# trnKhanh/medical-image-analysis

Measured on AMD Instinct MI355X. Metric: training images/sec (whole node), UNet 512x512 1ch bs=32/GPU, higher is better.
Workload: dtype bf16; 1 GPU; UNet-2D channels [64, 128, 256, 512, 1024] 512x512 1ch, batch 32/GPU, instance norm, dropout 0.1, Dice+CE, Adam(wd 5e-4), clip 10 (cfg3); global_batch=32, parallelism=dp1

## Files before the change

include/mia_hip.h:

```cpp
#ifndef MIA_HIP_H
#define MIA_HIP_H
#include <stdint.h>
#ifdef __cplusplus
extern "C" {
#endif

#define MIA_F32 0
#define MIA_BF16 1

int mia_version(void);
const char* mia_last_error(void);

int mia_pack_weight(const float* src, void* dst, int dtype, int d0, int d1, int taps, int npad, int kpad,
                    int n_from_d0, void* stream);
int mia_pack_desc_bytes(void);
int mia_pack_weight_batch(const void* descs_dev, int count, int total_bricks, int max_taps, int dtype, void* stream);
int mia_relayout(const void* src, int src_dtype, void* dst, int dst_dtype, int n, int c, int64_t hw,
                 int64_t ssn, int64_t ssc, int64_t ssp, int64_t dsn, int64_t dsc, int64_t dsp, void* stream);
int mia_add(const void* a, const void* b, void* out, int dtype, int64_t n, void* stream);
int mia_dropout_mask(float* out, int64_t n, float keep, uint64_t seed, uint64_t offset, void* stream);
int mia_dropout_mask_dyn(float* out, int64_t n, float keep, const uint64_t* seed_base, uint64_t rel_offset, void* stream);
int mia_zero(void* p, int64_t bytes, void* stream);
int mia_gather_f32(const float* src, int64_t stride, float* dst, int n, void* stream);
int mia_colsum_workspace(int64_t p, int c);
int mia_colsum(const void* x, int dtype, int64_t p, int c, float* workspace, float* out, int accumulate, void* stream);

#define MIA_CONV_G3S1 0
#define MIA_CONV_G3S2 1
#define MIA_CONV_G2S2 2
#define MIA_CONV_T3S2 3
#define MIA_CONV_T2S2 4
#define MIA_CONV_G1 5
int mia_set_option(const char* name, int value);
int mia_get_option(const char* name, int* value);
int mia_conv_mma_tiles(int mode, int hout, int wout, int* tiles_y, int* tiles_x, int* tile_h);
int mia_conv_mma(int mode, int dtype, const void* in1, int c1, const void* in2, int c2, const void* wpack, int npad,
                 int kpad, int flip_taps, const float* bias, void* out1, int o1, void* out2, int o2,
                 float* stat_partials, int n, int hin, int win, int hout, int wout, const void* amax_in1, const void* amax_in2,
                 const void* amax_w, const void* wpack_split, void* amax_out1, void* amax_out2, void* stream);
int mia_split_desc_bytes(void);
int mia_split_f16_batch(const void* descs_dev, int count, void* stream);
int mia_amax(const float* x, int64_t n, void* slot, int reset, void* stream);
int mia_widen_u8_i64(const void* src, void* dst, int64_t n, void* stream);
int mia_host_narrow_labels(const int64_t* src, uint8_t* dst, int64_t n, int threads);
int mia_host_copy(void* dst, const void* src, int64_t bytes, int threads);
int mia_amax_desc_bytes(void);
int mia_amax_batch(const void* descs_dev, int count, void* slots, void* stream);

int mia_conv_nl_supported(int mode, int dtype, int c1, int nout, int hout, int wout);
int mia_conv_mma_nl(int mode, int dtype, const void* y_in, int c1, const float* in_scale, const float* in_shift, float slope,
                    const void* wpack, int npad, int kpad, const float* bias, void* out, int nout, float* stat_partials,
                    int n, int hin, int win, int hout, int wout, void* stream);

int mia_conv_acc_supported(int mode, int dtype, int c1, int nout);
int mia_conv_mma_acc(int mode, int dtype, const void* in1, int c1, const void* wpack, int npad, int kpad, int flip_taps,
                     void* out_inout, int nout, int n, int hin, int win, int hout, int wout, const void* amax_in, const void* amax_w,
                     const void* wpack_split, void* stream);


int mia_stem_slabs(void);
int mia_stem_wgrad_workspace(int c0);
int mia_stem_fwd(const void* x, int x_dtype, const float* w, const float* bias, void* y, int dtype, float* stat_partials, int n,
                 int h, int wd, int c0, void* stream);
int mia_stem_wgrad(const void* x, int x_dtype, const void* dy, int dtype, float* workspace, float* grad, int n, int h, int wd,
                   int c0, int accumulate, void* stream);
int mia_stem_wgrad_fused(const void* x, int x_dtype, const void* dz, const void* y, int dtype, const float* scale,
                         const float* shift, const float* xa, const float* xb, const float* c1, const float* c2, float slope,
                         float* workspace, float* grad, int n, int h, int wd, int c0, int accumulate, void* stream);

#define MIA_WGRAD_3S1 0
#define MIA_WGRAD_3S2 1
#define MIA_WGRAD_2S2 2
int mia_wgrad_target_blocks(int mode, int dtype);
int mia_wgrad_geometry(int mode, int dtype, int hy, int wy, int* tiles_y, int* tiles_x);
int mia_wgrad_plan(int mode, int dtype, int c1, int c2, int cdy, int npad, int hy, int* column_blocks, int* target_blocks, int* tile_h);
int mia_conv_wgrad(int mode, int dtype, const void* x1, int c1, const void* x2, int c2, const void* dy, int cdy,
                   float* slabs, int ksplit, int npad, int kpad, int n, int hx, int wx, int hy, int wy, const void* amax_x1,
                   const void* amax_x2, const void* amax_dy, void* stream);
int mia_wgrad_nl_supported(int mode, int dtype, int c1, int cdy);
int mia_conv_wgrad_nl(int mode, int dtype, const void* y_in, int c1, const float* in_scale, const float* in_shift, float slope,
                      const void* dy, int cdy, float* slabs, int ksplit, int npad, int kpad, int n, int hx, int wx, int hy,
                      int wy, void* stream);
int mia_wgrad_reduce(const float* slabs, int ksplit, int taps, int npad, int kpad, float* grad, int nn, int kk,
                     int accumulate, void* stream);

#define MIA_NORM_INSTANCE 0
#define MIA_NORM_BATCH 1
int mia_norm_finalize(const float* partials, int n, int tiles, int c, int64_t hw, int mode, int training,
                      const float* drop_scale, const float* gamma, const float* beta, float eps, float momentum,
                      float* running_mean, float* running_var, long long* num_batches, float* xa, float* xb,
                      float* scale, float* shift, float* ysum, void* stream);
int mia_norm_stats(const void* y, int dtype, int n, int64_t hw, int c, int slabs, float* partials, void* stream);
int mia_norm_act_fwd(const void* y, void* z, int dtype, const float* scale, const float* shift, int n, int64_t hw, int c,
                     float slope, void* amax_out, void* stream);
int mia_norm_two_piece_ok(int dtype, int c);
int mia_norm_act_bwd(const void* dz, const void* dz2, const void* y, void* dy, int dtype, const float* scale, const float* shift,
                     const float* xa, const float* xb, const float* ysum, int n, int64_t hw, int c, int mode,
                     int fixed_stats, float slope, int slabs, float* partials, float* c1, float* c2, float* dgamma,
                     float* dbeta, float* dbias, int accumulate, void* amax_out, void* stream);
int mia_norm_bwd_sums(const void* dz, const void* dz2, const void* y, int dtype, const float* scale, const float* shift,
                      const float* xa, const float* xb, const float* ysum, int n, int64_t hw, int c, int mode,
                      int fixed_stats, float slope, int slabs, float* partials, float* c1, float* c2, float* dgamma,
                      float* dbeta, float* dbias, int accumulate, void* stream);

int mia_bn_sync_local_stats(const float* partials, int n, int tiles, int c, int64_t hw, const float* drop_scale, float* xa,
                            float* xb, float* local, void* stream);
int mia_norm_finalize_sync(const float* gathered, int world, int n, int c, int64_t hw, const float* drop_scale,
                           const float* gamma, const float* beta, float eps, float momentum, float* running_mean,
                           float* running_var, long long* num_batches, float* xa, float* xb, float* scale, float* shift,
                           float* ysum, void* stream);
int mia_norm_act_bwd_reduce(const void* dz, const void* dz2, const void* y, int dtype, const float* scale, const float* shift, const float* xa,
                            const float* xb, int n, int64_t hw, int c, float slope, int slabs, float* partials, float* c1,
                            float* c2, float* tot, void* stream);
int mia_norm_act_bwd_apply_sync(const void* dz, const void* dz2, const void* y, void* dy, int dtype, const float* scale, const float* shift,
                                const float* xa, const float* xb, const float* ysum, int n, int64_t hw, int c, float slope,
                                float* c1, float* c2, const float* group_tot, float* dgamma, float* dbeta, float* dbias,
                                int accumulate, void* amax_out, void* stream);

int mia_head_fwd(const void* x, int dtype, const float* w, const float* b, float* logits, int n, int64_t hw, int c0, int k1,
                 int64_t osn, int64_t osk, int64_t osp, void* stream);
int mia_head_bwd_workspace(int c0, int k1);
int mia_head_bwd(const float* dlogits, const void* x, int dtype, const float* w, void* dx, float* dw, float* db,
                 float* workspace, int n, int64_t hw, int c0, int k1, int64_t gsn, int64_t gsk, int64_t gsp, int accumulate,
                 void* stream);
#define MIA_LOSS_SOFTMAX 1
#define MIA_LOSS_DO_BG 2
#define MIA_LOSS_BATCH 4
#define MIA_LOSS_SQUARED 8
#define MIA_LOSS_DENSE 16
int mia_dice_ce_workspace(int nb, int k1, int slabs);
int mia_dice_ce_fwd(const float* logits, const long long* labels, int nb, int64_t hw, int k1, int64_t sn, int64_t sk,
                    int64_t sp, int flags, float smooth, float dice_w, float ce_w, int slabs, float* workspace, float* sums,
                    float* coef, float* out, int* bad_label, void* stream);
int mia_dice_ce_bwd(const float* logits, const long long* labels, const float* coef, const float* grad_out, float* dlogits,
                    int nb, int64_t hw, int k1, int64_t sn, int64_t sk, int64_t sp, int64_t gsn, int64_t gsk, int64_t gsp,
                    int flags, float dice_w, float ce_w, void* stream);

int mia_ds_loss_workspace(int nb, int k1, int slabs);
int mia_ds_loss_fwd(const float* z, const long long* labels, int nb, int h, int w, int factor, int k1, int64_t sn, int64_t sk,
                    int64_t sp, int flags, float smooth, float dice_w, float ce_w, int slabs, float* workspace, float* sums,
                    float* coef, float* out, int* bad_label, void* stream);
int mia_ds_loss_bwd(const float* z, const long long* labels, const float* coef, const float* grad_out, float* dz, int nb, int h,
                    int w, int factor, int k1, int64_t sn, int64_t sk, int64_t sp, int64_t gsn, int64_t gsk, int64_t gsp, int flags,
                    float dice_w, float ce_w, void* stream);

int mia_head_norm_eligible(int dtype, int n, int64_t hw, int c0, int k1);
int mia_head_norm_fwd(const void* y, int dtype, const float* scale, const float* shift, float slope, const float* w,
                      const float* b, float* logits, int n, int64_t hw, int c0, int k1, int64_t osn, int64_t osk, int64_t osp,
                      void* stream);
int mia_head_norm_wgrad(const float* dlogits, const void* y, int dtype, const float* scale, const float* shift, float slope,
                        float* dw, float* db, float* workspace, int n, int64_t hw, int c0, int k1, int64_t gsn, int64_t gsk,
                        int64_t gsp, int accumulate, void* stream);
int mia_norm_act_bwd_head(const float* dlogits, const float* w, int k1, int64_t gsn, int64_t gsk, int64_t gsp, const void* y,
                          void* dy, int dtype, const float* scale, const float* shift, const float* xa, const float* xb,
                          const float* ysum, int n, int64_t hw, int c, int mode, int fixed_stats, float slope, int slabs,
                          float* partials, float* c1, float* c2, float* dgamma, float* dbeta, float* dbias, int accumulate,
                          void* amax_out, void* stream);
int mia_head_w_supported(int dtype, int c, int k1);
int mia_norm_act_bwd_head_w(const float* dlogits, const float* w, int k1, int64_t gsn, int64_t gsk, int64_t gsp,
                            const void* y, void* dy, int dtype, const float* scale, const float* shift, const float* xa,
                            const float* xb, const float* ysum, int n, int64_t hw, int c, int mode, int fixed_stats,
                            float slope, int slabs, float* partials, float* c1, float* c2, float* dgamma, float* dbeta,
                            float* dbias, int accumulate, float* head_workspace, float* dw_head, float* db_head,
                            int accumulate_head, void* amax_out, void* stream);

#define MIA_SEGLOSS_SOFTMAX 1
#define MIA_SEGLOSS_DO_BG 2
#define MIA_SEGLOSS_BATCH 4
#define MIA_SEGLOSS_LABEL_U8 8
#define MIA_SEGLOSS_IGNORE 16
int mia_seg_loss_workspace(int nb, int k1, int slabs);
int mia_seg_loss_fwd(const float* logits, const void* labels, const float* class_w, int nb, int64_t hw, int k1, int64_t sn,
                     int64_t sk, int64_t sp, int flags, int64_t ignore_label, float smooth, float dice_w, float ce_w, int slabs,
                     float* workspace, float* coef, float* out, int64_t* counts, int* bad_label, void* stream);
int mia_seg_loss_bwd(const float* logits, const void* labels, const float* class_w, const float* coef, const float* grad_out,
                     float* dlogits, int nb, int64_t hw, int k1, int64_t sn, int64_t sk, int64_t sp, int64_t gsn, int64_t gsk,
                     int64_t gsp, int flags, int64_t ignore_label, void* stream);
int mia_topk_ce_workspace(int64_t n_pixels);
int mia_topk_ce_fwd(const float* logits, const void* labels, const float* class_w, int nb, int64_t hw, int k1, int64_t sn,
                    int64_t sk, int64_t sp, int flags, int64_t ignore_label, int64_t n_top, float* workspace, float* out,
                    int* bad_label, void* stream);
int mia_topk_ce_bwd(const float* logits, const void* labels, const float* class_w, const float* workspace, const float* grad_out,
                    float* dlogits, int nb, int64_t hw, int k1, int64_t sn, int64_t sk, int64_t sp, int64_t gsn, int64_t gsk,
                    int64_t gsp, int flags, int64_t ignore_label, void* stream);
#define MIA_REGLOSS_DO_BG 1
#define MIA_REGLOSS_BATCH 2
#define MIA_REGLOSS_IGNORE 4
#define MIA_REGLOSS_INDEX 8
#define MIA_REGLOSS_TARGET_U8 16
int mia_region_loss_workspace(int nb, int c, int slabs);
int mia_region_loss_fwd(const float* logits, const void* target, const unsigned* region_bits, int n_labels, const float* pos_weight,
                        int nb, int64_t hw, int c, int64_t sn, int64_t sk, int64_t sp, int flags, int64_t ignore_label, float smooth,
                        float dice_w, float ce_w, int slabs, float* workspace, float* coef, float* out, int64_t* counts,
                        int* bad_label, void* stream);
int mia_region_loss_bwd(const float* logits, const void* target, const unsigned* region_bits, int n_labels, const float* pos_weight,
                        const float* coef, const float* grad_out, float* dlogits, int nb, int64_t hw, int c, int64_t sn, int64_t sk,
                        int64_t sp, int64_t gsn, int64_t gsk, int64_t gsp, int flags, int64_t ignore_label, void* stream);

#define MIA_OPT_ADAM 0
#define MIA_OPT_ADAMW 1
#define MIA_OPT_SGD 2
int mia_grad_norm_workspace(void);
int mia_grad_norm(const float* grad, int64_t n, float max_norm, float grad_scale, float* workspace, float* out, void* stream);
int mia_scale_by_clip(float* x, int64_t n, const float* clip, void* stream);
int mia_optim_step(float* param, const float* grad, float* m, float* v, int64_t n, int kind, float lr, float beta1,
                   float beta2, float eps, float weight_decay, float bias_corr1, float bias_corr2, int first_step,
                   const float* clip, float grad_scale, void* stream);
int mia_step_dyn_set(void* dyn32, float lr, float bias_corr1, float bias_corr2, int first_step, uint64_t seed, uint64_t offset, void* stream);
int mia_optim_step_dyn(float* param, const float* grad, float* m, float* v, int64_t n, int kind, float beta1, float beta2, float eps,
                       float weight_decay, const float* dyn, const float* clip, float grad_scale, void* stream);

int mia_affine_nearest(const float* img_in, float* img_out, const long long* lab_in, long long* lab_out, int nb, int c, int h,
                       int w, const float* mats, const int* apply, void* stream);
int mia_elastic_warp(const float* img_in, float* img_out, const long long* lab_in, long long* lab_out, int nb, int c, int h,
                     int w, const float* disp, int gh, int gw, const int* apply, void* stream);
int mia_rot90_flip(const void* in, void* out, int elem_bytes, int nb, int c, int h, int w, int k, int flip_h, int flip_w,
                   void* stream);
int mia_crop(const void* in, void* out, int elem_bytes, int nb, int c, int h, int w, int oh, int ow, const int* top,
             const int* left, void* stream);
int mia_gaussian_blur(const float* in, float* out, int nb, int c, int h, int w, const float* sigma, const int* ksize,
                      int max_ksize, const int* apply, void* stream);
int mia_sample_stats_workspace(int nb);
int mia_sample_stats(const float* in, int nb, int c, int64_t hw, int gray, float* workspace, float* mean_std, void* stream);
int mia_sample_stats_sel(const float* in, int nb, int c, int64_t hw, int gray, float* workspace, float* mean_std,
                         const int* apply, void* stream);
int mia_copy_selected(const void* in, void* out, int64_t bytes_per_sample, int nb, const int* apply, void* stream);
#define MIA_EW_GAMMA 0
#define MIA_EW_CONTRAST 1
#define MIA_EW_NOISE 2
#define MIA_EW_ZSCORE 3
int mia_elementwise(const float* in, float* out, int64_t per_sample, int nb, int op, const float* p0, const float* mean_std,
                    const float* aux, const int* apply, void* stream);
int mia_noise_clip(const float* in, float* out, int64_t per_sample, int nb, const float* sigma, uint64_t seed, uint64_t offset,
                   const int* apply, void* stream);
int mia_resize_bilinear(const float* in, float* out, int nb, int c, int h, int w, int oh, int ow, const int* lowres_hw,
                        const int* apply, void* stream);
int mia_resize_bilinear_bwd(const float* dout, float* din_zeroed, int nb, int c, int h, int w, int oh, int ow, void* stream);
int mia_resize_bilinear_aa(const float* in, float* tmp, float* out, int nb, int c, int h, int w, int oh, int ow, void* stream);
int mia_resize_nearest(const void* in, void* out, int elem_bytes, int64_t planes, int h, int w, int oh, int ow, void* stream);

int mia_argmax_dice_workspace(int nb, int k1, int slabs);
int mia_argmax_dice(const float* logits, const long long* labels, long long* pred, int nb, int64_t hw, int k1, int64_t sn, int64_t sk,
                    int64_t sp, int slabs, float* workspace, float* counts, float* dice, void* stream);
int mia_selector_scores_workspace(int nb, int slabs);
int mia_selector_scores(const float* logits, int nb, int64_t hw, int k1, int64_t sn, int64_t sk, int64_t sp, float smooth, int slabs,
                        float* workspace, float* scores, void* stream);
int mia_badge_embed_workspace(int nb, int64_t hw, int k1, int c0, int dtype, int* slabs);
int mia_badge_embed(const float* logits, const void* feat, int dtype, int nb, int64_t hw, int k1, int c0, int64_t sn, int64_t sk,
                    int64_t sp, float smooth, int do_bg, int squared, float* workspace, float* embed, float* loss, void* stream);
int mia_surface_distance_workspace(int nvol, int d, int h, int w, int k1);
int mia_surface_distance(const long long* pred, const long long* labels, int nvol, int ndim, int d, int h, int w, int k1,
                         float sd, float sh, float sw, float* workspace, float* hd, float* asd, void* stream);
int mia_surface_metrics_workspace(int nvol, int d, int h, int w, int k1);
int mia_surface_metrics(const long long* pred, const long long* labels, int nvol, int ndim, int d, int h, int w, int k1,
                        float sd, float sh, float sw, double percentile, const float* tolerance, float* workspace, float* hd,
                        float* asd, float* hd_pct, float* assd, float* nsd, void* stream);
int mia_sdm_workspace(int nb, int h, int w, int k1, int class_mask);
int mia_signed_distance_map(const void* labels, int label_u8, int nb, int h, int w, int k1, int class_mask, float sh, float sw,
                            float* workspace, float* phi, void* stream);
int mia_boundary_loss_workspace(int nb, int slabs);
int mia_boundary_loss_fwd(const float* logits, const void* labels, int label_u8, const float* phi, const float* weight_dev, int nb,
                          int64_t hw, int k1, int class_mask, int64_t sn, int64_t sk, int64_t sp, int slabs, float* workspace,
                          float* coef, float* out, int* bad_label, void* stream);
int mia_boundary_loss_bwd(const float* logits, const float* phi, const float* coef, const float* weight_dev, const float* grad_out,
                          float* dlogits, int nb, int64_t hw, int k1, int class_mask, int64_t sn, int64_t sk, int64_t sp,
                          int64_t gsn, int64_t gsk, int64_t gsp, void* stream);
int mia_consistency_workspace(int nb, int slabs);
int mia_consistency_fwd(const float* zs, const float* zt, const float* prob_mean, const float* dyn_dev, int nb, int64_t hw, int k1,
                        int64_t sn, int64_t sk, int64_t sp, int64_t tsn, int64_t tsk, int64_t tsp, float den_scale, int slabs,
                        float* workspace, unsigned char* keep, float* coef, float* out, long long* n_keep, void* stream);
int mia_consistency_bwd(const float* zs, const float* zt, const unsigned char* keep, const float* coef, const float* dyn_dev,
                        const float* grad_out, float* dzs, int nb, int64_t hw, int k1, int64_t sn, int64_t sk, int64_t sp,
                        int64_t tsn, int64_t tsk, int64_t tsp, int64_t gsn, int64_t gsk, int64_t gsp, void* stream);
int mia_ema_update(float* teacher, const float* student, int64_t n, float alpha, const float* alpha_dev, void* stream);
int mia_urpc_workspace(int nb, int ns, int slabs);
int mia_urpc_fwd(const float* const* z, const int* factors, const int64_t* strides, int ns, int nb, int H, int W, int k1,
                 const float* dyn_dev, int slabs, float* workspace, float* sums, float* terms, float* out, void* stream);
int mia_urpc_bwd(const float* const* z, const int* factors, const int64_t* strides, float* const* dz, const int64_t* gstrides, int ns,
                 int nb, int H, int W, int k1, const float* sums, const float* dyn_dev, const float* grad_out, void* stream);
int mia_cps_workspace(int nb, int slabs);
int mia_cps_fwd(const float* za, const float* zb, const float* dyn_dev, int nb, int64_t hw, int k1, int64_t asn, int64_t ask,
                int64_t asp, int64_t bsn, int64_t bsk, int64_t bsp, int slabs, float* workspace, unsigned char* code, float* out,
                long long* counts, void* stream);
int mia_cps_bwd(const float* za, const float* zb, const unsigned char* code, const float* dyn_dev, const float* grad_out, float* dza,
                float* dzb, int nb, int64_t hw, int k1, int64_t asn, int64_t ask, int64_t asp, int64_t bsn, int64_t bsk, int64_t bsp,
                int64_t gasn, int64_t gask, int64_t gasp, int64_t gbsn, int64_t gbsk, int64_t gbsp, void* stream);

int mia_softmax_accum(const float* logits, float* prob_sum, long long* pred, int nb, int64_t hw, int k1, int64_t sn, int64_t sk,
                      int64_t sp, float weight, int first, void* stream);
int mia_sigmoid_accum(const float* logits, float* prob_sum, long long* pred, const long long* class_order, int nb, int64_t hw, int c,
                      int64_t sn, int64_t sk, int64_t sp, float weight, float threshold, int first, void* stream);
int mia_window_accum(const float* logits, float* canvas, const float* gy, const float* gx, int nb, int k1, int ph, int pw, int h,
                     int w, int y0, int x0, int64_t sn, int64_t sk, int64_t sp, float weight, int flip_h, int flip_w, void* stream);
int mia_window_finalize(float* canvas, long long* pred, const float* ry, const float* rx, int nb, int k1, int h, int w, float scale,
                        int normalise, void* stream);
int mia_mask_denoise_supported(int h, int w, int dilate, int erode, int smooth_k);
int mia_mask_denoise(const long long* in, long long* out, int nb, int h, int w, int dilate, int erode, int smooth_k, void* stream);
int mia_cc_label(const long long* labels, int* roots, int nvol, int ndim, int d, int h, int w, int connectivity, int n_classes,
                 int foreground, int* status, void* stream);
int mia_cc_workspace(int nvol, int ndim, int d, int h, int w, int n_classes);
int mia_cc_filter(const long long* labels, long long* out, int nvol, int ndim, int d, int h, int w, int connectivity, int n_classes,
                  int foreground, int keep_largest, int min_size, const unsigned char* class_mask, int64_t fill, float* workspace,
                  int* status, void* stream);

#ifdef __cplusplus
}
#endif
#endif
```

include/mia_hip_experiments.h:

```cpp
#pragma once
#include <stdint.h>
#ifdef __cplusplus
extern "C" {
#endif
int mia_conv_cr_supported(int mode, int dtype, int c1, int nout, int hout, int wout);
int mia_conv_mma_cr(int mode, int dtype, const void* in1, int c1, const void* wpack, int npad, int kpad, int flip_taps,
                    void* out, int nout, const void* y_prod, const float* scale, const float* shift, const float* xa,
                    const float* xb, float slope, float* partials, int n, int hin, int win, int hout, int wout, void* stream);
int mia_norm_act_bwd_pre(const void* dz, const void* y, void* dy, int dtype, const float* scale, const float* shift,
                         const float* xa, const float* xb, const float* ysum, int n, int64_t hw, int c, int mode,
                         int fixed_stats, float slope, int parts, const float* partials, float* c1, float* c2,
                         float* dgamma, float* dbeta, float* dbias, int accumulate, void* amax_out, void* stream);
#ifdef __cplusplus
}
#endif
```

medical-image-analysis_amd/csrc/common.h:

```cpp
#pragma once
#include <hip/hip_runtime.h>
#include <stdint.h>
#include <stdio.h>
#include <string.h>

#define MIA_F32 0
#define MIA_BF16 1

#define MIA_OK 0
#define MIA_EARG (-1)
#define MIA_EUNSUPPORTED (-2)

extern "C" const char* mia_last_error(void);
void mia_set_error(const char* fmt, ...);

#define MIA_CHECK_ARG(cond, ...)            \
  do {                                      \
    if (!(cond)) {                          \
      mia_set_error(__VA_ARGS__);           \
      return MIA_EARG;                      \
    }                                       \
  } while (0)

#define MIA_LAUNCH_CHECK()                                                  \
  do {                                                                      \
    hipError_t _e = hipGetLastError();                                      \
    if (_e != hipSuccess) {                                                 \
      mia_set_error("%s:%d: %s", __FILE__, __LINE__, hipGetErrorString(_e)); \
      return (int)_e;                                                       \
    }                                                                       \
  } while (0)

typedef unsigned short bf16_t;

typedef __attribute__((ext_vector_type(4))) float f32x4;
typedef __attribute__((ext_vector_type(8))) __bf16 bf16x8;
typedef __attribute__((ext_vector_type(4))) short s16x4;
typedef __attribute__((ext_vector_type(4))) unsigned int u32x4;
typedef __attribute__((ext_vector_type(2))) unsigned int u32x2;
typedef __attribute__((ext_vector_type(16))) float f32x16;

__device__ __forceinline__ float bf2f(bf16_t v) { return __builtin_bit_cast(float, ((unsigned)v) << 16); }
__device__ __forceinline__ bf16_t f2bf(float f) {
  __bf16 b = (__bf16)f;
  return __builtin_bit_cast(bf16_t, b);
}

typedef float f32x2_t __attribute__((ext_vector_type(2)));
typedef __bf16 bf16x2_t __attribute__((ext_vector_type(2)));
__device__ __forceinline__ unsigned pack_bf16x2(float a, float b) {
  return __builtin_bit_cast(unsigned, __builtin_convertvector(f32x2_t{a, b}, bf16x2_t));
}

__device__ __forceinline__ float row16_sum(float v) {
  int iv;
  iv = __builtin_bit_cast(int, v); v += __builtin_bit_cast(float, __builtin_amdgcn_update_dpp(iv, iv, 0xB1, 0xF, 0xF, false));
  iv = __builtin_bit_cast(int, v); v += __builtin_bit_cast(float, __builtin_amdgcn_update_dpp(iv, iv, 0x4E, 0xF, 0xF, false));
  iv = __builtin_bit_cast(int, v); v += __builtin_bit_cast(float, __builtin_amdgcn_update_dpp(iv, iv, 0x141, 0xF, 0xF, false));
  iv = __builtin_bit_cast(int, v); v += __builtin_bit_cast(float, __builtin_amdgcn_update_dpp(iv, iv, 0x140, 0xF, 0xF, false));
  return v;
}

template <typename T> struct Elem;
template <> struct Elem<float> {
  static constexpr int EPU = 4;
  static constexpr int DT = MIA_F32;
  __device__ static __forceinline__ float ld(const float* p) { return *p; }
  __device__ static __forceinline__ void st(float* p, float v) { *p = v; }
  __device__ static __forceinline__ float cvt(float v) { return v; }
};
template <> struct Elem<bf16_t> {
  static constexpr int EPU = 8;
  static constexpr int DT = MIA_BF16;
  __device__ static __forceinline__ float ld(const bf16_t* p) { return bf2f(*p); }
  __device__ static __forceinline__ void st(bf16_t* p, float v) { *p = f2bf(v); }
  __device__ static __forceinline__ bf16_t cvt(float v) { return f2bf(v); }
};

struct SplitF16 {
  typedef __attribute__((ext_vector_type(2))) float f2;
  typedef __attribute__((ext_vector_type(2))) _Float16 h2;
  typedef __attribute__((ext_vector_type(8))) _Float16 f16x8;
  static __device__ __forceinline__ int exp_of(unsigned amax_bits) {
    const int e = 141 - (int)((amax_bits >> 23) & 0xFFu);
    return e > 120 ? 120 : e;
  }
  static __device__ __forceinline__ float pow2(int e) { return __builtin_bit_cast(float, (unsigned)(127 + e) << 23); }
  static __device__ __forceinline__ u32x4 unit(const u32x4& raw, float s) {
    const f32x4 x = __builtin_bit_cast(f32x4, raw) * s;
    u32x4 o;
#pragma unroll
    for (int p = 0; p < 2; ++p) {
      const f2 v = {x[2 * p], x[2 * p + 1]};
      const h2 hh = __builtin_convertvector(v, h2);
      const h2 ll = __builtin_convertvector(v - __builtin_convertvector(hh, f2), h2);
      const unsigned hp = __builtin_bit_cast(unsigned, hh), lp = __builtin_bit_cast(unsigned, ll);
      o[2 * p] = __builtin_amdgcn_perm(lp, hp, 0x05040100u);
      o[2 * p + 1] = __builtin_amdgcn_perm(lp, hp, 0x07060302u);
    }
    return o;
  }
  static __device__ __forceinline__ void unit_planar(const u32x4& raw, float s, u32x2& hp, u32x2& lp) {
    const f32x4 x = __builtin_bit_cast(f32x4, raw) * s;
#pragma unroll
    for (int p = 0; p < 2; ++p) {
      const f2 v = {x[2 * p], x[2 * p + 1]};
      const h2 hh = __builtin_convertvector(v, h2);
      const h2 ll = __builtin_convertvector(v - __builtin_convertvector(hh, f2), h2);
      hp[p] = __builtin_bit_cast(unsigned, hh); lp[p] = __builtin_bit_cast(unsigned, ll);
    }
  }
  static __device__ __forceinline__ void planes_of(const u32x4& w, u32x2& hp, u32x2& lp) {
#pragma unroll
    for (int p = 0; p < 2; ++p) {
      hp[p] = __builtin_amdgcn_perm(w[2 * p + 1], w[2 * p], 0x05040100u);
      lp[p] = __builtin_amdgcn_perm(w[2 * p + 1], w[2 * p], 0x07060302u);
    }
  }
  static __device__ __forceinline__ f32x16 mfma32(const u32x4& a, const u32x4& b, f32x16 c) {
    return __builtin_amdgcn_mfma_f32_32x32x16_f16(__builtin_bit_cast(f16x8, a), __builtin_bit_cast(f16x8, b), c, 0, 0, 0);
  }
  static __device__ __forceinline__ u32x4 dup_hi(const u32x4& w) {
    u32x4 o;
#pragma unroll
    for (int d = 0; d < 4; ++d) o[d] = __builtin_amdgcn_perm(w[d], w[d], 0x01000100u);
    return o;
  }
  static __device__ __forceinline__ u32x4 dup_lo(const u32x4& w) {
    u32x4 o;
#pragma unroll
    for (int d = 0; d < 4; ++d) o[d] = __builtin_amdgcn_perm(w[d], w[d], 0x03020302u);
    return o;
  }
  static __device__ __forceinline__ u32x4 swap_hl(const u32x4& w) {
    u32x4 o;
#pragma unroll
    for (int d = 0; d < 4; ++d) o[d] = __builtin_amdgcn_alignbit(w[d], w[d], 16);
    return o;
  }
  static __device__ __forceinline__ f32x4 mfma(const u32x4& a, const u32x4& b, f32x4 c) {
    return __builtin_amdgcn_mfma_f32_16x16x32_f16(__builtin_bit_cast(f16x8, a), __builtin_bit_cast(f16x8, b), c, 0, 0, 0);
  }
  static __device__ __forceinline__ f32x4 mma(const u32x4& a, const u32x4& bh, const u32x4& bl, f32x4 c) { return mfma(a, bl, mfma(a, bh, c)); }
  static __device__ __forceinline__ f32x4 mma_a(const u32x4& ah, const u32x4& al, const u32x4& b, f32x4 c) { return mfma(al, b, mfma(ah, b, c)); }
  static __device__ __forceinline__ float unscale(float acc, int eo) { return __builtin_ldexpf(acc, eo); }
};

__device__ __forceinline__ float norm_bwd_dy(float g, float yv, float sc, float sf, float ka, float kb, float slope) {
  if (!(__builtin_fmaf(sc, yv, sf) > 0.f)) g *= slope;
  return __builtin_fmaf(sc, g, __builtin_fmaf(ka, yv, kb));
}

__device__ __forceinline__ void store_data_fence() { __builtin_amdgcn_sched_barrier(0x3AC); }
__device__ __forceinline__ void store_data_pad() {
  __builtin_amdgcn_sched_barrier(0x3AC);
  asm volatile("s_nop 1" ::: "memory");
  __builtin_amdgcn_sched_barrier(0x3AC);
}

__device__ __forceinline__ float wave_sum(float v) {
#pragma unroll
  for (int o = 32; o > 0; o >>= 1) v += __shfl_xor(v, o, 64);
  return v;
}

__device__ __forceinline__ double wave_sum_d(double v) {
#pragma unroll
  for (int o = 32; o > 0; o >>= 1) v += __shfl_xor(v, o, 64);
  return v;
}

__device__ __forceinline__ int wave_sum_i(int v) {
#pragma unroll
  for (int o = 32; o > 0; o >>= 1) v += __shfl_xor(v, o, 64);
  return v;
}

__device__ __forceinline__ float block_sum(float v, float* red ) {
  v = wave_sum(v);
  const int w = threadIdx.x >> 6, l = threadIdx.x & 63, nw = (blockDim.x + 63) >> 6;
  __syncthreads();
  if (l == 0) red[w] = v;
  __syncthreads();
  float r = 0.f;
  if (threadIdx.x < 64) {
    r = (l < nw) ? red[l] : 0.f;
    r = wave_sum(r);
  }
  return r;
}

static inline int ceil_div(int a, int b) { return (a + b - 1) / b; }
static inline int64_t ceil_div64(int64_t a, int64_t b) { return (a + b - 1) / b; }
```

medical-image-analysis_amd/csrc/conv64.hip:

```cpp
#include "conv_common.h"
#include "lds_dma.h"
#include <stdlib.h>
#include <type_traits>

namespace {

constexpr int C = 64;
constexpr int TH = 16, TW = 16;
constexpr int IH = TH + 2, IW = TW + 2, PITCH = IW;
constexpr int A_IT = (IH * IW + 63) / 64;
constexpr int NPA = ((A_IT * 64 + 13) / 16) * 16 + 2;
constexpr int LDS_BYTES = 8 * NPA * 16;

struct Tile { int img, ty, tx; };

__device__ __forceinline__ void stat_acc(float& s1, float& s2, float v) {
  asm volatile("v_add_f32 %0, %2, %0\n\tv_fmac_f32 %1, %2, %2" : "+v"(s1), "+v"(s2) : "v"(v));
}

}

#ifdef CONV64_STAMPS
__device__ unsigned long long conv64_dbg[512 * 4 * 8];
#define STAMP(var)                                                                          \
  do {                                                                                      \
    __builtin_amdgcn_sched_barrier(0);                                                      \
    asm volatile("s_memtime %0\n\ts_waitcnt lgkmcnt(0)" : "=s"(var)::"memory");             \
    __builtin_amdgcn_sched_barrier(0);                                                      \
  } while (0)
extern "C" int mia_conv64_debug_read(unsigned long long* host_out) {
  return (int)hipMemcpyFromSymbol(host_out, HIP_SYMBOL(conv64_dbg), sizeof(conv64_dbg));
}
#else
#define STAMP(var) do { } while (0)
#endif

template <bool NL, bool CR>
__global__ __launch_bounds__(256, 2) void conv64_persist_kernel(const ConvArgs a, int total_tiles, int tiles_per_img, int run, int n_base) {
  __shared__ __attribute__((aligned(16))) unsigned char smem[LDS_BYTES + (NL ? 2 * C * 4 : 0)];
  u32x4* ldsA = reinterpret_cast<u32x4*>(smem);
  float* cf = reinterpret_cast<float*>(smem + LDS_BYTES);

  const int tid = threadIdx.x, lane = tid & 63;
  const int wave = __builtin_amdgcn_readfirstlane(tid >> 6);
  const int q = lane >> 4, c16 = lane & 15;
  const int pr = pi16(c16);
  const int g = tid & 3, p4 = tid >> 2;

  const rsrc_t rsw = make_rsrc(a.wp, (unsigned)(9 * a.npad * C * 2));
  u32x4 wf[2][3][3];
#pragma unroll
  for (int c = 0; c < 2; ++c)
#pragma unroll
    for (int ta = 0; ta < 3; ++ta)
#pragma unroll
      for (int tb = 0; tb < 3; ++tb) {
        const int t = ta * 3 + tb;
        const int tw = a.flip ? 8 - t : t;
        wf[c][ta][tb] = __builtin_amdgcn_raw_buffer_load_b128(rsw, ((n_base + 16 * wave + c16) * C + 32 * c + 8 * q) * 2, tw * a.npad * C * 2, 0);
      }
  f32x4 bv;
#pragma unroll
  for (int r = 0; r < 4; ++r) bv[r] = a.bias ? a.bias[n_base + 16 * wave + 4 * q + r] : 0.f;

  const int nblk = gridDim.x, b = blockIdx.x;
  const int first = (b & 7) * run + (b >> 3);
  const int stride = 8 * run;
  auto decode = [&](int t) -> Tile {
    Tile r;
    r.img = t / tiles_per_img;
    const int rem = t - r.img * tiles_per_img;
    r.ty = rem / a.tiles_x;
    r.tx = rem - r.ty * a.tiles_x;
    return r;
  };
  const Tile dstep = decode(stride);
  auto advance = [&](Tile r) -> Tile {
    r.tx += dstep.tx;
    if (r.tx >= a.tiles_x) { r.tx -= a.tiles_x; r.ty += 1; }
    r.ty += dstep.ty;
    if (r.ty >= a.tiles_y) { r.ty -= a.tiles_y; r.img += 1; }
    r.img += dstep.img;
    return r;
  };

  const size_t ipix = (size_t)a.Hin * a.Win;
  const unsigned img_bytes = (unsigned)(ipix * C * 2);
  const bf16_t* in = static_cast<const bf16_t*>(a.in1);
  bf16_t* out = static_cast<bf16_t*>(n_base ? a.out2 : a.out1);

  u32x4 pf[2 * A_IT];
  float cpf = 0.f;
  auto fetch = [&](const Tile& t) {
    const rsrc_t rs = make_rsrc(in + (size_t)t.img * ipix * C, img_bytes);
    const int iy0 = t.ty * TH - 1, ix0 = t.tx * TW - 1;
    int p4v = p4;
    asm volatile("" : "+v"(p4v));
    const bool interior = iy0 >= 0 && ix0 >= 0 && iy0 + IH <= a.Hin && ix0 + IW <= a.Win;
    const int tile_off = (iy0 * a.Win + ix0) * (C * 2) + g * 16;
    if constexpr (NL) {
      if (wave < 2) cpf = (wave == 0 ? a.nl_scale : a.nl_shift)[(size_t)t.img * C + lane];
    }
#pragma unroll
    for (int i = 0; i < A_IT; ++i) {
      const int pix = p4v + 64 * i, iy = pix / IW, ix = pix - iy * IW;
      unsigned voff;
      if (interior) {
        voff = (unsigned)(tile_off + (iy * a.Win + ix) * (C * 2));
        if (i == A_IT - 1) voff = (pix < IH * IW) ? voff : SENT;
      } else {
        const int gy = iy0 + iy, gx = ix0 + ix;
        const int okm = -(int)(((unsigned)gy < (unsigned)a.Hin) & ((unsigned)gx < (unsigned)a.Win) & (pix < IH * IW));
        const unsigned off = (unsigned)((gy * a.Win + gx) * (C * 2) + g * 16);
        voff = (off & (unsigned)okm) | (SENT & ~(unsigned)okm);
      }
      pf[2 * i] = __builtin_amdgcn_raw_buffer_load_b128(rs, (int)voff, 0, 0);
      pf[2 * i + 1] = __builtin_amdgcn_raw_buffer_load_b128(rs, (int)voff, 64, 0);
    }
  };
  auto xform = [&](const u32x4& raw, const f32x4& sa, const f32x4& sb, const f32x4& ha, const f32x4& hb, auto mask_tag, unsigned keep) -> u32x4 {
    constexpr bool MASK = decltype(mask_tag)::value;
    u32x4 o;
    const f32x2_t sl2 = {a.nl_slope, a.nl_slope};
#pragma unroll
    for (int d = 0; d < 4; ++d) {
      const unsigned w = raw[d];
      const f32x2_t sc = d == 0 ? f32x2_t{sa[0], sa[1]} : d == 1 ? f32x2_t{sa[2], sa[3]} : d == 2 ? f32x2_t{sb[0], sb[1]} : f32x2_t{sb[2], sb[3]};
      const f32x2_t sh = d == 0 ? f32x2_t{ha[0], ha[1]} : d == 1 ? f32x2_t{ha[2], ha[3]} : d == 2 ? f32x2_t{hb[0], hb[1]} : f32x2_t{hb[2], hb[3]};
      const f32x2_t x = {__builtin_bit_cast(float, w << 16), __builtin_bit_cast(float, w & 0xFFFF0000u)};
      const f32x2_t v = __builtin_elementwise_fma(sc, x, sh);
      const f32x2_t m = v * sl2;
      const unsigned r = pack_bf16x2(__builtin_fmaxf(v[0], m[0]), __builtin_fmaxf(v[1], m[1]));
      o[d] = MASK ? (r & keep) : r;
    }
    return o;
  };
  auto commit = [&](const Tile& t) {
    if constexpr (NL) {
      const f32x4* cf4 = reinterpret_cast<const f32x4*>(cf);
      const int iy0 = t.ty * TH - 1, ix0 = t.tx * TW - 1;
      const bool interior = iy0 >= 0 && ix0 >= 0 && iy0 + IH <= a.Hin && ix0 + IW <= a.Win;
#pragma unroll
      for (int h = 0; h < 2; ++h) {
        const f32x4 sa = cf4[8 * h + 2 * g], sb = cf4[8 * h + 2 * g + 1], ha = cf4[16 + 8 * h + 2 * g], hb = cf4[17 + 8 * h + 2 * g];
#pragma unroll
        for (int i = 0; i < A_IT; ++i) pf[2 * i + h] = xform(pf[2 * i + h], sa, sb, ha, hb, std::false_type{}, 0u);
        __builtin_amdgcn_sched_barrier(0);
      }
      if (!interior) {
        int p4v = p4;
        asm volatile("" : "+v"(p4v));
#pragma unroll
        for (int i = 0; i < A_IT; ++i) {
          const int pix = p4v + 64 * i, iy = pix / IW, ix = pix - iy * IW;
          const unsigned keep = 0u - (unsigned)(((unsigned)(iy0 + iy) < (unsigned)a.Hin) & ((unsigned)(ix0 + ix) < (unsigned)a.Win));
#pragma unroll
          for (int d = 0; d < 4; ++d) { pf[2 * i][d] &= keep; pf[2 * i + 1][d] &= keep; }
        }
      }
    }
#pragma unroll
    for (int i = 0; i < A_IT; ++i) {
      ldsA[g * NPA + p4 + 64 * i] = pf[2 * i];
      ldsA[(4 + g) * NPA + p4 + 64 * i] = pf[2 * i + 1];
    }
  };

  int t = first;
  if (t >= total_tiles) return;
  Tile cur = decode(t);
  fetch(cur);
  if constexpr (NL) {
    if (tid < 2 * C) cf[tid] = cpf;
    __syncthreads();
  }
  commit(cur);
  __syncthreads();

#ifdef CONV64_STAMPS
  unsigned long long ts0 = 0, ts1 = 0, ts2 = 0, ts3 = 0, ts4 = 0, ts5 = 0, acc_f = 0, acc_m = 0, acc_e = 0, acc_b = 0, acc_c = 0, ntl = 0;
#endif
  while (true) {
    STAMP(ts0);
    const int tn = t + stride;
    const bool more = tn < total_tiles;
    Tile nxt = cur;
    if (more) { nxt = advance(cur); fetch(nxt); }

    STAMP(ts1);
    f32x4 acc[TH];
    constexpr int GROUPS = 6, RPG = 3;
    u32x4 fr[2][RPG];
    auto load_group = [&](int gi, u32x4* f) {
      const int ph = gi / GROUPS, c = ph / 3, tb = ph % 3, r0 = (gi % GROUPS) * RPG;
#pragma unroll
      for (int j = 0; j < RPG; ++j) f[j] = ldsA[(4 * c + q) * NPA + (r0 + j) * PITCH + tb + pr];
    };
    load_group(0, fr[0]);
#pragma unroll
    for (int gi = 0; gi < 6 * GROUPS; ++gi) {
      const int ph = gi / GROUPS, c = ph / 3, tb = ph % 3, r0 = (gi % GROUPS) * RPG;
      if (gi + 1 < 6 * GROUPS) load_group(gi + 1, fr[(gi + 1) & 1]);
      __builtin_amdgcn_sched_barrier(0);
#pragma unroll
      for (int j = 0; j < RPG; ++j) {
        const int r = r0 + j;
#pragma unroll
        for (int ta = 0; ta < 3; ++ta) {
          const int m = r - ta;
          if (m >= 0 && m < TH) {
            const bool first_touch = (ph == 0 && ta == 0);
            acc[m] = __builtin_amdgcn_mfma_f32_16x16x32_bf16(__builtin_bit_cast(bf16x8, wf[c][ta][tb]),
                                                             __builtin_bit_cast(bf16x8, fr[gi & 1][j]), first_touch ? bv : acc[m], 0, 0, 0);
          }
        }
      }
    }

    STAMP(ts2);
    const int oy0 = cur.ty * TH, ox0 = cur.tx * TW;
    const bool full = (oy0 + TH <= a.Hout) && (ox0 + TW <= a.Wout);
    const bool colok = ox0 + pr < a.Wout;
    const rsrc_t rso = make_rsrc(out + (size_t)cur.img * ipix * C, img_bytes);
    const int qodd = q & 1;
    const unsigned obase = (unsigned)((((oy0 + qodd) * a.Wout) + ox0 + pr) * (C * 2) + (16 * wave + 8 * (q >> 1)) * 2);
    const int row_bytes = a.Wout * (C * 2);
    const bool want_stats = a.stats != nullptr;
    float s1[4] = {0.f, 0.f, 0.f, 0.f}, s2[4] = {0.f, 0.f, 0.f, 0.f};
    f32x4 csc, csf, cxa, cxb;
    u32x2 yv[TH];
    const unsigned ybase = (unsigned)(((oy0 * a.Wout) + ox0 + pr) * (C * 2) + (16 * wave + 4 * q) * 2);
    rsrc_t rsy;
    constexpr int YB = 2;
    auto load_y = [&](int m0, bool full_t) {
#pragma unroll
      for (int mm = m0; mm < m0 + YB; ++mm) {
        const bool ok = full_t || (colok && oy0 + mm < a.Hout);
        yv[mm] = __builtin_bit_cast(u32x2, __builtin_amdgcn_raw_buffer_load_b64(rsy, (int)(ok ? ybase + (unsigned)(mm * row_bytes) : SENT), 0, 0));
      }
    };
    if constexpr (CR) {
      const unsigned cbytes = (unsigned)(a.N * C * 4);
      const int co = (cur.img * C + 16 * wave + 4 * q) * 4;
      csc = __builtin_bit_cast(f32x4, __builtin_amdgcn_raw_buffer_load_b128(make_rsrc(a.cr_scale, cbytes), co, 0, 0));
      csf = __builtin_bit_cast(f32x4, __builtin_amdgcn_raw_buffer_load_b128(make_rsrc(a.cr_shift, cbytes), co, 0, 0));
      cxa = __builtin_bit_cast(f32x4, __builtin_amdgcn_raw_buffer_load_b128(make_rsrc(a.cr_xa, cbytes), co, 0, 0));
      cxb = __builtin_bit_cast(f32x4, __builtin_amdgcn_raw_buffer_load_b128(make_rsrc(a.cr_xb, cbytes), co, 0, 0));
      rsy = make_rsrc(static_cast<const bf16_t*>(a.cr_y) + (size_t)cur.img * ipix * C, img_bytes);
      load_y(0, full);
      load_y(YB, full);
    }
    auto cr_row = [&](unsigned p01, unsigned p23, const u32x2& yr, float wgt) {
      const unsigned dzw[2] = {p01, p23}, yw[2] = {yr[0], yr[1]};
#pragma unroll
      for (int h = 0; h < 2; ++h) {
#pragma unroll
        for (int e = 0; e < 2; ++e) {
          const int r = 2 * h + e;
          const float dzv = __builtin_bit_cast(float, e ? (dzw[h] & 0xFFFF0000u) : (dzw[h] << 16));
          const float y = __builtin_bit_cast(float, e ? (yw[h] & 0xFFFF0000u) : (yw[h] << 16));
          float g = dzv * wgt;
          if (!(__builtin_fmaf(csc[r], y, csf[r]) > 0.f)) g *= a.cr_slope;
          s1[r] += g;
          s2[r] = __builtin_fmaf(g, __builtin_fmaf(cxa[r], y, cxb[r]), s2[r]);
        }
      }
    };
    auto store_rows = [&](auto full_tag) {
      constexpr bool FULL = decltype(full_tag)::value;
      if constexpr (FULL) asm volatile("s_nop 7\n\ts_nop 7" ::: "memory");
#pragma unroll
      for (int m = 0; m < TH; m += 2) {
        if constexpr (CR) {
          if (m % YB == 0 && m + 2 * YB < TH) load_y(m + 2 * YB, FULL);
        }
        if (want_stats && !CR) {
#pragma unroll
          for (int mm = m; mm < m + 2; ++mm) {
            const float w = (FULL || (colok && oy0 + mm < a.Hout)) ? 1.f : 0.f;
#pragma unroll
            for (int r = 0; r < 4; ++r) {
              const float v = acc[mm][r];
              if constexpr (FULL) stat_acc(s1[r], s2[r], v);
              else { const float vm = v * w; s1[r] += vm; s2[r] += vm * v; }
            }
          }
        }
        const unsigned x0 = pack_bf16x2(acc[m][0], acc[m][1]), x1 = pack_bf16x2(acc[m][2], acc[m][3]);
        const unsigned y0 = pack_bf16x2(acc[m + 1][0], acc[m + 1][1]), y1 = pack_bf16x2(acc[m + 1][2], acc[m + 1][3]);
        if constexpr (CR) {
          cr_row(x0, x1, yv[m], (FULL || (colok && oy0 + m < a.Hout)) ? 1.f : 0.f);
          cr_row(y0, y1, yv[m + 1], (FULL || (colok && oy0 + m + 1 < a.Hout)) ? 1.f : 0.f);
        }
        const auto r0 = __builtin_amdgcn_permlane16_swap(x0, y0, false, false);
        const auto r1 = __builtin_amdgcn_permlane16_swap(x1, y1, false, false);
        const u32x4 d = {r0[0], r1[0], r0[1], r1[1]};
        if constexpr (FULL) {
          __builtin_amdgcn_raw_buffer_store_b128(d, rso, (int)obase, m * row_bytes, 0);
        } else {
          const bool ok = colok && (oy0 + m + qodd < a.Hout);
          const unsigned voff = ok ? obase + (unsigned)(m * row_bytes) : SENT;
          __builtin_amdgcn_raw_buffer_store_b128(d, rso, (int)voff, 0, 0);
        }
        if constexpr (CR) {
          __builtin_amdgcn_sched_barrier(0);
#ifndef CR_PAD
#define CR_PAD 16
#endif
#if CR_PAD >= 16
          asm volatile("s_nop 7\n\ts_nop 7" ::: "memory");
#elif CR_PAD >= 8
          asm volatile("s_nop 7" ::: "memory");
#elif CR_PAD >= 4
          asm volatile("s_nop 3" ::: "memory");
#elif CR_PAD >= 2
          asm volatile("s_nop 1" ::: "memory");
#endif
          __builtin_amdgcn_sched_barrier(0);
        }
      }
    };
    if (full) store_rows(std::true_type{});
    else store_rows(std::false_type{});
    if (want_stats) {
#pragma unroll
      for (int r = 0; r < 4; ++r) { s1[r] = row16_sum(s1[r]); s2[r] = row16_sum(s2[r]); }
      if (c16 == 0) {
        const size_t tile = (size_t)cur.img * tiles_per_img + (size_t)cur.ty * a.tiles_x + cur.tx;
        typedef __attribute__((address_space(1))) f32x4 gf32x4;
        gf32x4* dst = (gf32x4*)(a.stats + (tile * (size_t)(a.o1 + a.o2) + n_base + 16 * wave + 4 * q) * 2);
        dst[0] = f32x4{s1[0], s2[0], s1[1], s2[1]};
        __builtin_amdgcn_sched_barrier(0);
        asm volatile("s_nop 1" ::: "memory");
        __builtin_amdgcn_sched_barrier(0);
        dst[1] = f32x4{s1[2], s2[2], s1[3], s2[3]};
        __builtin_amdgcn_sched_barrier(0);
        asm volatile("s_nop 1" ::: "memory");
        __builtin_amdgcn_sched_barrier(0);
      }
    }
    STAMP(ts3);
#ifdef CONV64_STAMPS
    acc_f += ts1 - ts0; acc_m += ts2 - ts1; acc_e += ts3 - ts2; ntl += 1;
#endif
    if (!more) break;
    if constexpr (NL) {
      if (tid < 2 * C) cf[tid] = cpf;
    }
    __syncthreads();
    STAMP(ts4);
    commit(nxt);
    __syncthreads();
    STAMP(ts5);
#ifdef CONV64_STAMPS
    acc_b += ts4 - ts3; acc_c += ts5 - ts4;
#endif
    t = tn;
    cur = nxt;
  }
#ifdef CONV64_STAMPS
  if (lane == 0) {
    unsigned long long* d = conv64_dbg + ((size_t)blockIdx.x * 4 + wave) * 8;
    d[0] = acc_f; d[1] = acc_m; d[2] = acc_e; d[3] = acc_b; d[4] = acc_c; d[5] = ntl;
  }
#endif
}

bool conv64_eligible(int mode, int dtype, const ConvArgs& a) {
  if (mode != MODE_G3S1 || dtype != MIA_BF16) return false;
  if (a.nl_scale != nullptr && (a.o2 != 0 || a.nl_shift == nullptr || !(a.nl_slope >= 0.f && a.nl_slope <= 1.f))) return false;
  if (a.cr_y != nullptr && (a.o2 != 0 || a.nl_scale != nullptr || a.stats == nullptr || !a.cr_scale || !a.cr_shift || !a.cr_xa || !a.cr_xb)) return false;
  if (a.c1 != C || a.c2 != 0 || a.o1 != C || (a.o2 != 0 && a.o2 != C) || a.npad != a.o1 + a.o2 || a.kpad != C) return false;
  if (!a.vec_in || !a.vec_out) return false;
  if ((size_t)a.Hin * a.Win * C * 2 >= ((size_t)1 << 31)) return false;
  if (a.Hout <= 8) return false;
  return true;
}

int conv64_launch(const ConvArgs& a, int blocks_override, int reserve, hipStream_t st) {
  const int tiles_per_img = a.tiles_x * a.tiles_y;
  const int total = a.N * tiles_per_img;
  const int cap = 2 * persistent_cus(256, reserve);
  int nblk = total < cap ? ((total + 7) / 8) * 8 : cap;
  if (blocks_override >= 8 && blocks_override % 8 == 0 && blocks_override <= nblk) nblk = blocks_override;
  const int run = nblk / 8;
  if (a.nl_scale != nullptr) {
    hipLaunchKernelGGL((conv64_persist_kernel<true, false>), dim3(nblk), dim3(256), 0, st, a, total, tiles_per_img, run, 0);
    return MIA_OK;
  }
#ifdef MIA_EXPERIMENTS
  if (a.cr_y != nullptr) {
    hipLaunchKernelGGL((conv64_persist_kernel<false, true>), dim3(nblk), dim3(256), 0, st, a, total, tiles_per_img, run, 0);
    return MIA_OK;
  }
#else
  if (a.cr_y != nullptr) { mia_set_error("column-reduce epilogue: experiment build only (-DMIA_EXPERIMENTS)"); return MIA_EUNSUPPORTED; }
#endif
  hipLaunchKernelGGL((conv64_persist_kernel<false, false>), dim3(nblk), dim3(256), 0, st, a, total, tiles_per_img, run, 0);
  if (a.o2 == C)
    hipLaunchKernelGGL((conv64_persist_kernel<false, false>), dim3(nblk), dim3(256), 0, st, a, total, tiles_per_img, run, C);
  return MIA_OK;
}
```

medical-image-analysis_amd/csrc/conv_mma.hip:

```cpp
#include <stdlib.h>

#include "conv_common.h"
#include "options.h"

template <typename T, int MODE, int MT, int NT>
__global__ __launch_bounds__(256, 2) void conv_mma_kernel(const ConvArgs a) {
  using G = Geo<MODE, MT>;
  constexpr int TH = G::TH, BN = 16 * NT, EPU = Elem<T>::EPU, KB = 4 * EPU;
  constexpr int NPA = G::NPA, NPB = BN + 2, PITCH = G::PITCH, S = G::S, IW = G::IW, IH = G::IH;
  constexpr int OSTR = BN + EPU;
  constexpr int A_UNITS = 4 * NPA, B_UNITS = G::MAXTAPS * 4 * NPB;
  constexpr int STAGE_BYTES = (A_UNITS + B_UNITS) * 16;
  constexpr int OUT_BYTES = TH * 16 * OSTR * (int)sizeof(T);
  constexpr int LDS_BYTES = STAGE_BYTES > OUT_BYTES ? STAGE_BYTES : OUT_BYTES;
  __shared__ __attribute__((aligned(16))) unsigned char smem[LDS_BYTES + 2 * 4 * BN * 4];
  u32x4* ldsA = reinterpret_cast<u32x4*>(smem);
  u32x4* ldsB = ldsA + A_UNITS;
  T* ldsO = reinterpret_cast<T*>(smem);
  float* ldsR = reinterpret_cast<float*>(smem + LDS_BYTES);

  const int tid = threadIdx.x, lane = tid & 63, wave = tid >> 6;
  const int q = lane >> 4, r16 = lane & 15;
  const int pr = pi16(r16);

// ... 20 lines not shown
    return 0;
  };
  auto tap_off = [&](int ta, int tb) -> int {
    if (MODE == MODE_G3S1) return ta * PITCH + tb;
    if (MODE == MODE_G3S2 || MODE == MODE_G2S2) return ta * PITCH + (tb & 1) * G::IWH + (tb >> 1);
    if (MODE == MODE_T3S2) { const int dh = ph ? (ta == 0 ? 1 : 0) : 0; const int dw = pw ? (tb == 0 ? 1 : 0) : 0; return dh * PITCH + dw; }
    return 0;
  };

  const int ctot = a.c1 + a.c2;
  f32x4 acc[MT][NT];
#pragma unroll
  for (int m = 0; m < MT; ++m)
#pragma unroll
    for (int n = 0; n < NT; ++n) acc[m][n] = f32x4{0.f, 0.f, 0.f, 0.f};

  const T* in1 = static_cast<const T*>(a.in1);
  const T* in2 = static_cast<const T*>(a.in2);
  const T* wp = static_cast<const T*>(a.wp);

  constexpr int A_N = IH * IW * 4, A_IT = (A_N + 255) / 256;
  constexpr int B_NMAX = G::MAXTAPS * 4 * BN, B_IT = (B_NMAX + 255) / 256;
  const int ntaps = nth * ntw;
  const int b_n = ntaps * 4 * BN;
  constexpr unsigned OOB = 0xFFFFFFFFu;
  unsigned a_pix[A_IT];
#pragma unroll
  for (int i = 0; i < A_IT; ++i) {
    const int u = tid + i * 256;
    a_pix[i] = OOB;
    if (u < A_N) {
      const int pix = u >> 2;
      const int iy = pix / IW, ix = pix - iy * IW;
      const int gy = iy0 + iy, gx = ix0 + ix;
      if (gy >= 0 && gy < a.Hin && gx >= 0 && gx < a.Win) a_pix[i] = (unsigned)(((int64_t)img * a.Hin + gy) * a.Win + gx);
    }
  }
  auto b_src = [&](int u) -> size_t {
    const int g = u & 3, n = (u >> 2) % BN, tl = u / (4 * BN);
    const int ta = tl / ntw, tb = tl - ta * ntw;
    return ((size_t)tap_w(ta, tb) * a.npad + n0 + n) * a.kpad + g * EPU;
  };
  u32x4 pa[A_IT], pb[B_IT];
  auto fetch = [&](int c0) {
#pragma unroll
    for (int i = 0; i < A_IT; ++i) {
      const int g = (tid + i * 256) & 3;
      const int c = c0 + g * EPU;
      u32x4 v = u32x4{0u, 0u, 0u, 0u};
      if (a_pix[i] != OOB && c < ctot) {
        const size_t p = a_pix[i];
        if (a.vec_in) {
          const T* src = (c < a.c1) ? in1 + p * a.c1 + c : in2 + p * a.c2 + (c - a.c1);
          v = *reinterpret_cast<const u32x4*>(src);
        } else {
          alignas(16) T tmp[EPU];
#pragma unroll
          for (int e = 0; e < EPU; ++e) {
            const int ce = c + e;
            T val = (T)0;
            if (ce < a.c1) val = in1[p * a.c1 + ce];
            else if (ce < ctot) val = in2[p * a.c2 + (ce - a.c1)];
            tmp[e] = val;
          }
          v = *reinterpret_cast<const u32x4*>(tmp);
        }
      }
      pa[i] = v;
    }
#pragma unroll
    for (int i = 0; i < B_IT; ++i)
      if (tid + i * 256 < b_n) pb[i] = *reinterpret_cast<const u32x4*>(wp + b_src(tid + i * 256) + c0);
  };
  auto commit = [&]() {
#pragma unroll
    for (int i = 0; i < A_IT; ++i) {
      const int u = tid + i * 256;
      if (u < A_N) {
        const int pix = u >> 2;
        const int iy = pix / IW, ix = pix - iy * IW;
        const int lidx = (S == 2) ? iy * PITCH + (ix & 1) * G::IWH + (ix >> 1) : iy * PITCH + ix;
        ldsA[(u & 3) * NPA + lidx] = pa[i];
      }
    }
#pragma unroll
    for (int i = 0; i < B_IT; ++i) {
      const int u = tid + i * 256;
      if (u < b_n) ldsB[((u / (4 * BN)) * 4 + (u & 3)) * NPB + ((u >> 2) % BN)] = pb[i];
    }
  };

  fetch(0);
  for (int c0 = 0; c0 < ctot; c0 += KB) {
    commit();
    __syncthreads();
    if (c0 + KB < ctot) fetch(c0 + KB);

    for (int ta = 0; ta < nth; ++ta) {
      for (int tb = 0; tb < ntw; ++tb) {
        const int tl = ta * ntw + tb;
        const int toff = tap_off(ta, tb);
        u32x4 bf[NT], af[MT];
#pragma unroll
        for (int n = 0; n < NT; ++n) bf[n] = ldsB[(tl * 4 + q) * NPB + n * 16 + pr];
#pragma unroll
        for (int m = 0; m < MT; ++m) af[m] = ldsA[q * NPA + S * (wave * MT + m) * PITCH + toff + pr];
#pragma unroll
        for (int m = 0; m < MT; ++m)
#pragma unroll
          for (int n = 0; n < NT; ++n) acc[m][n] = Mma<T>::run(af[m], bf[n], acc[m][n]);
      }
    }
    __syncthreads();
  }

  const bool tmode = (MODE == MODE_T3S2 || MODE == MODE_T2S2);
  const int hd = tmode ? (a.Hout - ph + 1) / 2 : a.Hout;
  const int wd = tmode ? (a.Wout - pw + 1) / 2 : a.Wout;
  const int nout = a.o1 + a.o2;
  float s1[NT], s2[NT];
#pragma unroll
  for (int n = 0; n < NT; ++n) { s1[n] = 0.f; s2[n] = 0.f; }
#pragma unroll
  for (int n = 0; n < NT; ++n) {
    const int nn = n * 16 + pr;
    const float b = (a.bias != nullptr && n0 + nn < nout) ? a.bias[n0 + nn] : 0.f;
#pragma unroll
    for (int m = 0; m < MT; ++m) {
      const int y = wave * MT + m;
#pragma unroll
      for (int r = 0; r < 4; ++r) {
        const int px = pi16(4 * q + r);
        const float v = acc[m][n][r] + b;
        if (oy0 + y < hd && ox0 + px < wd) { s1[n] += v; s2[n] += v * v; }
        ldsO[(y * 16 + px) * OSTR + nn] = Elem<T>::cvt(v);
      }
    }
  }
  if (a.stats != nullptr) {
#pragma unroll
    for (int n = 0; n < NT; ++n) {
      float t1 = s1[n], t2 = s2[n];
      t1 += __shfl_xor(t1, 16, 64); t1 += __shfl_xor(t1, 32, 64);
      t2 += __shfl_xor(t2, 16, 64); t2 += __shfl_xor(t2, 32, 64);
      if (q == 0) { ldsR[(0 * 4 + wave) * BN + n * 16 + pr] = t1; ldsR[(1 * 4 + wave) * BN + n * 16 + pr] = t2; }
    }
  }
  __syncthreads();
  if (a.stats != nullptr && tid < BN && n0 + tid < nout) {
    const float t1 = ldsR[0 * BN + tid] + ldsR[1 * BN + tid] + ldsR[2 * BN + tid] + ldsR[3 * BN + tid];
    const float t2 = ldsR[4 * BN + tid] + ldsR[5 * BN + tid] + ldsR[6 * BN + tid] + ldsR[7 * BN + tid];
    const size_t tile = (size_t)img * (a.tiles_x * a.tiles_y) + ty * a.tiles_x + tx;
    float* dst = a.stats + (tile * nout + n0 + tid) * 2;
    dst[0] = t1; dst[1] = t2;
  }
  T* out1 = static_cast<T*>(a.out1);
  T* out2 = static_cast<T*>(a.out2);
  constexpr int UPP = BN / EPU;
  for (int u = tid; u < TH * 16 * UPP; u += 256) {
    const int cu = u % UPP, pl = u / UPP;
    const int y = pl >> 4, px = pl & 15;
    if (oy0 + y >= hd || ox0 + px >= wd) continue;
    const int oy = tmode ? 2 * (oy0 + y) + ph : oy0 + y;
    const int ox = tmode ? 2 * (ox0 + px) + pw : ox0 + px;
    const size_t p = ((size_t)img * a.Hout + oy) * a.Wout + ox;
    const int n = n0 + cu * EPU;
    if (n >= nout) continue;
    const T* srow = ldsO + pl * OSTR + cu * EPU;
    if (a.vec_out) {
      T* dst = (n < a.o1) ? out1 + p * a.o1 + n : out2 + p * a.o2 + (n - a.o1);
      *reinterpret_cast<u32x4*>(dst) = *reinterpret_cast<const u32x4*>(srow);
    } else {
#pragma unroll
      for (int e = 0; e < EPU; ++e) {
        const int ne = n + e;
        if (ne < a.o1) out1[p * a.o1 + ne] = srow[e];
        else if (ne < nout) out2[p * a.o2 + (ne - a.o1)] = srow[e];
      }
    }
  }
}

template <typename T, int MODE, int MT, int NT>
static void launch(const ConvArgs& a, int grid_y, hipStream_t st) {
  const int grid_x = a.N * a.tiles_x * a.tiles_y * a.nblk_n;
  hipLaunchKernelGGL((conv_mma_kernel<T, MODE, MT, NT>), dim3(grid_x, grid_y), dim3(256), 0, st, a);
}

template <typename T, int MODE, int MT>
static void launch_nt(const ConvArgs& a, int nt, int grid_y, hipStream_t st) {
  if (nt == 4) launch<T, MODE, MT, 4>(a, grid_y, st);
  else if (nt == 2) launch<T, MODE, MT, 2>(a, grid_y, st);
  else launch<T, MODE, MT, 1>(a, grid_y, st);
}

template <typename T, int MODE>
static void launch_mt(const ConvArgs& a, int mt, int nt, int grid_y, hipStream_t st) {
  if constexpr (MODE == MODE_G3S2 || MODE == MODE_G2S2) {
    launch_nt<T, MODE, 2>(a, nt, grid_y, st);
  } else {
    if (mt >= 4) launch_nt<T, MODE, 4>(a, nt, grid_y, st);
    else launch_nt<T, MODE, 2>(a, nt, grid_y, st);
  }
}

template <typename T>
static int dispatch(int mode, const ConvArgs& a, int mt, int nt, int grid_y, hipStream_t st) {
  switch (mode) {
    case MODE_G3S1: launch_mt<T, MODE_G3S1>(a, mt, nt, grid_y, st); break;
    case MODE_G3S2: launch_mt<T, MODE_G3S2>(a, mt, nt, grid_y, st); break;
    case MODE_G2S2: launch_mt<T, MODE_G2S2>(a, mt, nt, grid_y, st); break;
    case MODE_T3S2: launch_mt<T, MODE_T3S2>(a, mt, nt, grid_y, st); break;
    case MODE_T2S2: launch_mt<T, MODE_T2S2>(a, mt, nt, grid_y, st); break;
    case MODE_G1: launch_mt<T, MODE_G1>(a, mt, nt, grid_y, st); break;
    default: return MIA_EARG;
  }
  return MIA_OK;
}

extern "C" int mia_amax(const float* x, int64_t n, void* slot, int reset, void* stream);

static void conv_tiles(const MiaOptions& opt, int mode, int hout, int wout, int* tiles_y, int* tiles_x, int* tile_h) {
  const bool tmode = (mode == MODE_T3S2 || mode == MODE_T2S2);
  const int hd = tmode ? (hout + 1) / 2 : hout, wd = tmode ? (wout + 1) / 2 : wout;
  int mt = (mode == MODE_G3S2 || mode == MODE_G2S2) ? 2 : (hd > 8 ? 4 : 2);
  const int th = 4 * mt;
  if (tiles_y) *tiles_y = ceil_div(hd, th);
  if (tiles_x) *tiles_x = ceil_div(wd, 16);
  if (tile_h) *tile_h = th;
}

extern "C" int mia_conv_mma_tiles(int mode, int hout, int wout, int* tiles_y, int* tiles_x, int* tile_h) {
  const MiaOptions opt = mia_options();
  conv_tiles(opt, mode, hout, wout, tiles_y, tiles_x, tile_h);
  return MIA_OK;
}

static int conv_mma_run(int mode, int dtype, const void* in1, int c1, const void* in2, int c2, const void* wpack,
                        int npad, int kpad, int flip_taps, const float* bias, void* out1, int o1, void* out2,
                        int o2, float* stat_partials, int n, int hin, int win, int hout, int wout, void* stream,
                        const float* nl_scale, const float* nl_shift, float nl_slope, const void* cr_y = nullptr,
                        const float* const* cr_coef = nullptr, float cr_slope = 0.f, int acc_out = 0, const void* amax_in1 = nullptr,
                        const void* amax_in2 = nullptr, const void* amax_w = nullptr, void* amax_out1 = nullptr, void* amax_out2 = nullptr,
                        const void* wpack_split = nullptr) {
  MIA_CHECK_ARG(mode >= 0 && mode <= MODE_G1, "mia_conv_mma: bad mode %d", mode);
  MIA_CHECK_ARG(dtype == MIA_F32 || dtype == MIA_BF16, "mia_conv_mma: bad dtype %d", dtype);
  MIA_CHECK_ARG(in1 && wpack && out1 && c1 > 0 && o1 > 0 && c2 >= 0 && o2 >= 0, "mia_conv_mma: null/empty operand");
  MIA_CHECK_ARG((c2 == 0) == (in2 == nullptr) && (o2 == 0) == (out2 == nullptr), "mia_conv_mma: split operand mismatch");
  MIA_CHECK_ARG(n > 0 && hin > 0 && win > 0 && hout > 0 && wout > 0, "mia_conv_mma: bad shape");
  const int epu = dtype == MIA_BF16 ? 8 : 4, kb = 4 * epu;
  MIA_CHECK_ARG(npad % 64 == 0 && npad >= o1 + o2, "mia_conv_mma: npad=%d must be a multiple of 64 >= %d", npad, o1 + o2);
  MIA_CHECK_ARG(kpad % kb == 0 && kpad >= c1 + c2, "mia_conv_mma: kpad=%d must be a multiple of %d >= %d", kpad, kb, c1 + c2);
  bool ok = true;
  switch (mode) {
    case MODE_G3S1: case MODE_G1: ok = (hout == hin && wout == win); break;
    case MODE_G3S2: ok = (hout == (hin + 1) / 2 && wout == (win + 1) / 2); break;
    case MODE_G2S2: ok = (hin == 2 * hout && win == 2 * wout); break;
    case MODE_T3S2: ok = (hin == (hout + 1) / 2 && win == (wout + 1) / 2); break;
    case MODE_T2S2: ok = (hout == 2 * hin && wout == 2 * win); break;
  }
  MIA_CHECK_ARG(ok, "mia_conv_mma: mode %d shape mismatch in %dx%d out %dx%d", mode, hin, win, hout, wout);
  const MiaOptions opt = mia_options();
  ConvArgs a;
  a.in1 = in1; a.in2 = in2; a.c1 = c1; a.c2 = c2; a.wp = wpack; a.bias = bias;
  a.out1 = out1; a.out2 = out2; a.o1 = o1; a.o2 = o2; a.stats = stat_partials;
  a.N = n; a.Hin = hin; a.Win = win; a.Hout = hout; a.Wout = wout;
  a.npad = npad; a.kpad = kpad; a.flip = flip_taps;
  a.nl_scale = nl_scale; a.nl_shift = nl_shift; a.nl_slope = nl_slope;
  a.acc_out = acc_out;
  a.split = (dtype == MIA_F32 && opt.f32_split && amax_in1 != nullptr && amax_w != nullptr && (c2 == 0 || amax_in2 != nullptr)) ? opt.f32_split : 0;
  a.amax_in1 = static_cast<const unsigned*>(amax_in1); a.amax_in2 = static_cast<const unsigned*>(amax_in2);
  a.amax_w = static_cast<const unsigned*>(amax_w);
  if (dtype != MIA_F32) amax_out1 = amax_out2 = nullptr;
  if (cr_y != nullptr) {
    a.cr_y = cr_y; a.cr_scale = cr_coef[0]; a.cr_shift = cr_coef[1]; a.cr_xa = cr_coef[2]; a.cr_xb = cr_coef[3]; a.cr_slope = cr_slope;
  }
  int th;
  conv_tiles(opt, mode, hout, wout, &a.tiles_y, &a.tiles_x, &th);
  int mt = th / 4;
  const int nout = o1 + o2;
  const int nt = nout > 32 ? 4 : (nout > 16 ? 2 : 1);
  a.nblk_n = ceil_div(nout, 16 * nt);
  a.st_tiles_y = a.tiles_y;
  auto al16 = [](const void* p) { return (reinterpret_cast<uintptr_t>(p) & 15) == 0; };
  a.vec_in = (c1 % epu == 0) && (c2 % epu == 0) && al16(in1) && (in2 == nullptr || al16(in2));
  a.vec_out = (o1 % epu == 0) && (o2 % epu == 0) && al16(out1) && (out2 == nullptr || al16(out2));
  const bool tmode = (mode == MODE_T3S2 || mode == MODE_T2S2);
  a.xcd = opt.conv_xcd;
  const int grid_y = tmode ? 4 : 1;
  hipStream_t st = static_cast<hipStream_t>(stream);
  int rc;
  const bool fast = conv_mma_fast_eligible(dtype, a, nt);
  if (opt.conv_s2_wide && fast && mode == MODE_G3S2 && dtype == MIA_BF16 && nout % 128 == 0 && o1 % 128 == 0 && hout > 8 &&
      (c1 + c2 >= 128 || opt.conv_s2_wide >= 2)) {
    mt = 4;
    a.tiles_y = ceil_div(hout, 16);
    a.nblk_n = nout / 128;
  }
  if (acc_out) {
    if (!fast) { mia_set_error("mia_conv_mma_acc: shape outside the accumulating kernel's contract"); return MIA_EUNSUPPORTED; }
    if (a.split && wpack_split != nullptr) { a.wp = wpack_split; a.wsplit = 1; }
    rc = conv_mma_fast_launch(mode, dtype, a, mt, nt, grid_y, st);
  }
#ifdef MIA_EXPERIMENTS
  else if (cr_y != nullptr) {
    if (!(mt == 4 && conv64_eligible(mode, dtype, a))) {
      mia_set_error("mia_conv_mma_cr: shape outside the column-reduce kernel's contract (ask mia_conv_cr_supported first)");
      return MIA_EUNSUPPORTED;
    }
    rc = conv64_launch(a, 0, opt.reserve_cus, st);
  }
#endif
  else if (nl_scale != nullptr) {
    if (!(mt == 4 && conv64_eligible(mode, dtype, a))) {
      mia_set_error("mia_conv_mma_nl: shape outside the normalise-on-load kernel's contract (ask mia_conv_nl_supported first)");
      return MIA_EUNSUPPORTED;
    }
    rc = conv64_launch(a, 0, opt.reserve_cus, st);
  }
  else if (opt.conv64 && opt.conv64_dma && (opt.conv64_dma >= 2 || a.o2 != 0) && mt == 4 && conv64_dma_eligible(mode, dtype, a)) rc = conv64_dma_launch(a, opt.reserve_cus, st);
  else if (opt.conv64 && mt == 4 && conv64_eligible(mode, dtype, a)) rc = conv64_launch(a, 0, opt.reserve_cus, st);
  else if (opt.conv_bt && mt == 4 && conv_bt_eligible(mode, dtype, a)) rc = conv_bt_launch(a, opt.conv_bt_order, opt.reserve_cus, st);
  else if (opt.conv_pw && (mode != MODE_G3S2 || opt.conv_pw_s2 >= 2 || (opt.conv_pw_s2 == 1 && c1 <= 256)) && conv_pw_eligible(mode, dtype, a))
    rc = conv_pw_launch(mode, a, opt.reserve_cus, st);
  else if (fast) {
    if (a.split && wpack_split != nullptr) { a.wp = wpack_split; a.wsplit = 1; }
    if (dtype == MIA_F32) { a.amax_out1 = static_cast<unsigned*>(amax_out1); a.amax_out2 = static_cast<unsigned*>(amax_out2); amax_out1 = amax_out2 = nullptr; }
    rc = conv_mma_fast_launch(mode, dtype, a, mt, nt, grid_y, st);
  }
  else rc = dtype == MIA_BF16 ? dispatch<bf16_t>(mode, a, mt, nt, grid_y, st) : dispatch<float>(mode, a, mt, nt, grid_y, st);
  if (rc != MIA_OK) return rc;
  MIA_LAUNCH_CHECK();
  if (amax_out1 != nullptr) { rc = mia_amax(static_cast<const float*>(out1), (int64_t)n * hout * wout * o1, amax_out1, 0, stream); if (rc) return rc; }
  if (amax_out2 != nullptr && out2 != nullptr) { rc = mia_amax(static_cast<const float*>(out2), (int64_t)n * hout * wout * o2, amax_out2, 0, stream); if (rc) return rc; }
  return MIA_OK;
}

extern "C" int mia_conv_mma(int mode, int dtype, const void* in1, int c1, const void* in2, int c2, const void* wpack,
                            int npad, int kpad, int flip_taps, const float* bias, void* out1, int o1, void* out2,
                            int o2, float* stat_partials, int n, int hin, int win, int hout, int wout, const void* amax_in1,
                            const void* amax_in2, const void* amax_w, const void* wpack_split, void* amax_out1, void* amax_out2,
                            void* stream) {
  return conv_mma_run(mode, dtype, in1, c1, in2, c2, wpack, npad, kpad, flip_taps, bias, out1, o1, out2, o2, stat_partials, n, hin,
                      win, hout, wout, stream, nullptr, nullptr, 0.f, nullptr, nullptr, 0.f, 0, amax_in1, amax_in2, amax_w, amax_out1,
                      amax_out2, wpack_split);
}

extern "C" int mia_conv_nl_supported(int mode, int dtype, int c1, int nout, int hout, int wout) {
  if (mode != MODE_G3S1) return 0;
  return (dtype == MIA_BF16 && c1 == 64 && nout == 64 && hout > 8) ? 1 : 0;
}

extern "C" int mia_conv_mma_nl(int mode, int dtype, const void* y_in, int c1, const float* in_scale, const float* in_shift,
                               float slope, const void* wpack, int npad, int kpad, const float* bias, void* out, int nout,
                               float* stat_partials, int n, int hin, int win, int hout, int wout, void* stream) {
  MIA_CHECK_ARG(in_scale != nullptr && in_shift != nullptr, "mia_conv_mma_nl: null coefficient arrays");
  MIA_CHECK_ARG(slope >= 0.f && slope <= 1.f, "mia_conv_mma_nl: slope %g outside [0, 1]", (double)slope);
  MIA_CHECK_ARG(mia_conv_nl_supported(mode, dtype, c1, nout, hout, wout), "mia_conv_mma_nl: unsupported shape (mode %d dtype %d %d -> %d)",
                mode, dtype, c1, nout);
  return conv_mma_run(mode, dtype, y_in, c1, nullptr, 0, wpack, npad, kpad, 0, bias, out, nout, nullptr, 0, stat_partials, n, hin, win,
                      hout, wout, stream, in_scale, in_shift, slope);
}

#ifdef MIA_EXPERIMENTS
extern "C" int mia_conv_cr_supported(int mode, int dtype, int c1, int nout, int hout, int wout) {
  (void)wout;
  return (mode == MODE_G3S1 && dtype == MIA_BF16 && c1 == 64 && nout == 64 && hout > 8) ? 1 : 0;
}

extern "C" int mia_conv_mma_cr(int mode, int dtype, const void* in1, int c1, const void* wpack, int npad, int kpad, int flip_taps,
                               void* out, int nout, const void* y_prod, const float* scale, const float* shift, const float* xa,
                               const float* xb, float slope, float* partials, int n, int hin, int win, int hout, int wout,
                               void* stream) {
  MIA_CHECK_ARG(y_prod && scale && shift && xa && xb && partials, "mia_conv_mma_cr: null pointer");
  MIA_CHECK_ARG(mia_conv_cr_supported(mode, dtype, c1, nout, hout, wout), "mia_conv_mma_cr: unsupported shape (mode %d dtype %d %d -> %d)",
                mode, dtype, c1, nout);
  MIA_CHECK_ARG((reinterpret_cast<uintptr_t>(y_prod) & 15) == 0 && (reinterpret_cast<uintptr_t>(scale) & 15) == 0 &&
                (reinterpret_cast<uintptr_t>(shift) & 15) == 0 && (reinterpret_cast<uintptr_t>(xa) & 15) == 0 &&
                (reinterpret_cast<uintptr_t>(xb) & 15) == 0, "mia_conv_mma_cr: 16-byte aligned tensors / coefficient rows required");
  const float* coef[4] = {scale, shift, xa, xb};
  return conv_mma_run(mode, dtype, in1, c1, nullptr, 0, wpack, npad, kpad, flip_taps, nullptr, out, nout, nullptr, 0, partials, n, hin,
                      win, hout, wout, stream, nullptr, nullptr, 0.f, y_prod, coef, slope);
}

#endif

extern "C" int mia_conv_acc_supported(int mode, int dtype, int c1, int nout) {
  const int epu = dtype == MIA_BF16 ? 8 : 4;
  return ((mode == MODE_T3S2 || mode == MODE_G3S1) && (dtype == MIA_BF16 || dtype == MIA_F32) && c1 % (4 * epu) == 0 && nout % epu == 0) ? 1 : 0;
}

extern "C" int mia_conv_mma_acc(int mode, int dtype, const void* in1, int c1, const void* wpack, int npad, int kpad, int flip_taps,
                                void* out_inout, int nout, int n, int hin, int win, int hout, int wout, const void* amax_in,
                                const void* amax_w, const void* wpack_split, void* stream) {
  MIA_CHECK_ARG(mode == MODE_T3S2 || mode == MODE_G3S1, "mia_conv_mma_acc: mode %d not served", mode);
  return conv_mma_run(mode, dtype, in1, c1, nullptr, 0, wpack, npad, kpad, flip_taps, nullptr, out_inout, nout, nullptr, 0, nullptr, n, hin,
                      win, hout, wout, stream, nullptr, nullptr, 0.f, nullptr, nullptr, 0.f, 1, amax_in, nullptr, amax_w, nullptr, nullptr, wpack_split);
}
```

medical-image-analysis_amd/csrc/lds_dma.h:

```cpp
#pragma once
#include "common.h"

typedef int i32x4 __attribute__((ext_vector_type(4)));
typedef __amdgpu_buffer_rsrc_t rsrc_t;
constexpr unsigned SENT = 0xFFFFFFF0u;

__device__ __forceinline__ rsrc_t make_rsrc(const void* p, unsigned bytes) {
  return __builtin_amdgcn_make_buffer_rsrc(const_cast<void*>(p), 0, (int)bytes, 0x00020000);
}
__device__ __forceinline__ i32x4 rsrc_words(const void* p, unsigned bytes) {
  const unsigned long long addr = (unsigned long long)p;
  i32x4 r;
  r.x = __builtin_amdgcn_readfirstlane((int)(unsigned)addr);
  r.y = __builtin_amdgcn_readfirstlane((int)(unsigned)(addr >> 32));
  r.z = __builtin_amdgcn_readfirstlane((int)bytes);
  r.w = 0x00020000;
  return r;
}

template <int NOP>
__device__ __forceinline__ void dma16(i32x4 rsrc, unsigned voff, unsigned soff, unsigned lds_dst) {
  asm volatile("s_mov_b32 m0, %3\n\ts_nop %4\n\tbuffer_load_dwordx4 %0, %1, %2 offen lds" : : "v"(voff), "s"(rsrc), "s"(soff), "s"(lds_dst), "n"(NOP) : "memory", "m0");
}
template <int NOP>
__device__ __forceinline__ void dma16(i32x4 rsrc, unsigned voff, unsigned lds_dst) {
  asm volatile("s_mov_b32 m0, %2\n\ts_nop %3\n\tbuffer_load_dwordx4 %0, %1, 0 offen lds" : : "v"(voff), "s"(rsrc), "s"(lds_dst), "n"(NOP) : "memory", "m0");
}

template <int N> __device__ __forceinline__ void wait_vm() { asm volatile("s_waitcnt vmcnt(%0)" ::"n"(N) : "memory"); }
```

medical-image-analysis_amd/csrc/norm.hip:

```cpp
#include "common.h"
#include "options.h"
#include <stdlib.h>

#define NORM_INSTANCE 0
#define NORM_BATCH 1

template <bool INST>
__global__ __launch_bounds__(1024) void norm_fwd_sum_kernel(const float* __restrict__ part, int tiles, int c, float* __restrict__ xa, float* __restrict__ xb,
                                    int64_t hw, const float* __restrict__ drop, const float* __restrict__ gamma,
                                    const float* __restrict__ beta, float eps, float* __restrict__ scale, float* __restrict__ shift,
                                    float* __restrict__ ysum) {
  __shared__ double sh1[16][17], sh2[16][17];
  const int cl = threadIdx.x & 15, tl = threadIdx.x >> 4;
  const int n = blockIdx.x, ch = blockIdx.y * 16 + cl;
  double s1 = 0.0, s2 = 0.0;
  if (ch < c) {
    typedef float f2_t __attribute__((ext_vector_type(2)));
    const f2_t* p = reinterpret_cast<const f2_t*>(part) + (size_t)n * tiles * c + ch;
    int t = tl;
    for (; t + 192 < tiles; t += 256) {
      const f2_t v0 = p[(size_t)t * c], v1 = p[(size_t)(t + 64) * c], v2 = p[(size_t)(t + 128) * c], v3 = p[(size_t)(t + 192) * c];
      s1 += (double)v0.x + (double)v1.x + (double)v2.x + (double)v3.x;
      s2 += (double)v0.y + (double)v1.y + (double)v2.y + (double)v3.y;
    }
// ... 441 lines not shown
template <typename T, bool VEC>
__global__ void norm_act_fwd_kernel(const T* __restrict__ y, T* __restrict__ z, const float* __restrict__ scale,
                                    const float* __restrict__ shift, int64_t hw, int c, int64_t total_units, float slope) {
  constexpr int EPU = VEC ? Elem<T>::EPU : 1;
  const int upp = c / EPU;
  for (int64_t u = (int64_t)blockIdx.x * blockDim.x + threadIdx.x; u < total_units; u += (int64_t)gridDim.x * blockDim.x) {
    const int64_t pix = u / upp;
    const int ch = (int)(u - pix * upp) * EPU;
    const int n = (int)(pix / hw);
    const float* sc = scale + (size_t)n * c + ch;
    const float* sf = shift + (size_t)n * c + ch;
    if constexpr (VEC) {
      const u32x4 raw = *reinterpret_cast<const u32x4*>(y + u * EPU);
      alignas(16) T in[EPU]; alignas(16) T out[EPU];
      *reinterpret_cast<u32x4*>(in) = raw;
#pragma unroll
      for (int e = 0; e < EPU; ++e) {
        const float v = sc[e] * Elem<T>::ld(in + e) + sf[e];
        out[e] = Elem<T>::cvt(v > 0.f ? v : v * slope);
      }
      *reinterpret_cast<u32x4*>(z + u * EPU) = *reinterpret_cast<const u32x4*>(out);
    } else {
      const float v = sc[0] * Elem<T>::ld(y + u) + sf[0];
      Elem<T>::st(z + u, v > 0.f ? v : v * slope);
    }
  }
}

extern "C" int mia_norm_act_fwd(const void* y, void* z, int dtype, const float* scale, const float* shift, int n, int64_t hw,
                                int c, float slope, void* amax_out, void* stream) {
  MIA_CHECK_ARG(y && z && scale && shift && n > 0 && hw > 0 && c > 0, "mia_norm_act_fwd: bad arguments");
  if (dtype != MIA_F32) amax_out = nullptr;
  const int epu = dtype == MIA_BF16 ? 8 : 4;
  const bool vec = (c % epu == 0) && ((reinterpret_cast<uintptr_t>(y) | reinterpret_cast<uintptr_t>(z)) & 15) == 0;
  const int64_t units = (int64_t)n * hw * (vec ? c / epu : c);
  const int blocks = (int)((units + 255) / 256 < 16384 ? (units + 255) / 256 : 16384);
  hipStream_t st = static_cast<hipStream_t>(stream);
  if (vec && (dtype == MIA_BF16 || dtype == MIA_F32)) {
    int sl, upb, gy;
    stream_geometry(n, hw, c, epu, &sl, &upb, &gy);
    if (dtype == MIA_BF16)
      hipLaunchKernelGGL(norm_act_fwd_stream_kernel<bf16_t>, dim3(n * sl, gy), dim3(256), 0, st, static_cast<const bf16_t*>(y), static_cast<bf16_t*>(z), scale, shift, hw, c, sl, upb, slope, (unsigned*)nullptr);
    else
      hipLaunchKernelGGL(norm_act_fwd_stream_kernel<float>, dim3(n * sl, gy), dim3(256), 0, st, static_cast<const float*>(y), static_cast<float*>(z), scale, shift, hw, c, sl, upb, slope, static_cast<unsigned*>(amax_out));
    MIA_LAUNCH_CHECK();
    return MIA_OK;
  }
#define NA(T, V) hipLaunchKernelGGL((norm_act_fwd_kernel<T, V>), dim3(blocks), dim3(256), 0, st, static_cast<const T*>(y), \
                                    static_cast<T*>(z), scale, shift, hw, c, units, slope)
  if (dtype == MIA_BF16) { if (vec) NA(bf16_t, true); else NA(bf16_t, false); }
  else if (dtype == MIA_F32) { if (vec) NA(float, true); else NA(float, false); }
  else { mia_set_error("mia_norm_act_fwd: bad dtype"); return MIA_EARG; }
#undef NA
  MIA_LAUNCH_CHECK();
  if (amax_out) return mia_amax(static_cast<const float*>(z), (int64_t)n * hw * c, amax_out, 0, stream);
  return MIA_OK;
}

template <typename T>
__global__ void norm_act_bwd_reduce_kernel(const T* __restrict__ dz, const T* __restrict__ y, const float* __restrict__ scale,
                                           const float* __restrict__ shift, const float* __restrict__ xa,
                                           const float* __restrict__ xb, int64_t hw, int c, int slabs, float slope,
                                           float* __restrict__ part) {
  extern __shared__ float sh[];
  const int n = blockIdx.x / slabs, s = blockIdx.x % slabs;
  const int cw = blockDim.x >= c ? c : blockDim.x, rows_par = blockDim.x / cw;
  const int tc = threadIdx.x % cw, tr = threadIdx.x / cw;
  const int64_t per = (hw + slabs - 1) / slabs, r0 = s * per, r1 = r0 + per < hw ? r0 + per : hw;
  const size_t base = (size_t)n * hw * c;
  for (int cb = blockIdx.y * cw; cb < c; cb += gridDim.y * cw) {
    const int ch = cb + tc;
    float s1 = 0.f, s2 = 0.f;
    if (ch < c && tr < rows_par) {
      const float sc = scale[(size_t)n * c + ch], sf = shift[(size_t)n * c + ch];
      const float a = xa[(size_t)n * c + ch], b = xb[(size_t)n * c + ch];
      for (int64_t r = r0 + tr; r < r1; r += rows_par) {
        const float yv = Elem<T>::ld(y + base + r * c + ch);
        float g = Elem<T>::ld(dz + base + r * c + ch);
        if (!(sc * yv + sf > 0.f)) g *= slope;
        s1 += g; s2 += g * (a * yv + b);
      }
    }
    sh[threadIdx.x] = s1; sh[blockDim.x + threadIdx.x] = s2;
    __syncthreads();
    if (tr == 0 && ch < c) {
      float t1 = 0.f, t2 = 0.f;
      for (int j = 0; j < rows_par; ++j) { t1 += sh[j * cw + tc]; t2 += sh[blockDim.x + j * cw + tc]; }
      float* dst = part + (((size_t)n * slabs + s) * c + ch) * 2;
      dst[0] = t1; dst[1] = t2;
    }
    __syncthreads();
  }
}

__global__ void norm_bwd_sum_kernel(const float* __restrict__ part, int slabs, int c, float* __restrict__ c1,
                                    float* __restrict__ c2) {
  __shared__ double sh1[16][17], sh2[16][17];
  const int cl = threadIdx.x & 15, tl = threadIdx.x >> 4;
  const int n = blockIdx.x, ch = blockIdx.y * 16 + cl;
  double s1 = 0.0, s2 = 0.0;
  if (ch < c)
    for (int s = tl; s < slabs; s += 16) {
      const float* p = part + (((size_t)n * slabs + s) * c + ch) * 2;
      s1 += p[0]; s2 += p[1];
    }
  sh1[tl][cl] = s1; sh2[tl][cl] = s2;
  __syncthreads();
  if (tl == 0 && ch < c) {
    s1 = 0.0; s2 = 0.0;
    for (int j = 0; j < 16; ++j) { s1 += sh1[j][cl]; s2 += sh2[j][cl]; }
    c1[(size_t)n * c + ch] = (float)s1; c2[(size_t)n * c + ch] = (float)s2;
  }
}

__global__ void norm_bwd_finalize_kernel(int n_img, int c, int64_t hw, int mode, int fixed_stats, const float* __restrict__ scale,
                                         const float* __restrict__ xa, const float* __restrict__ xb, const float* __restrict__ ysum,
                                         float* __restrict__ c1, float* __restrict__ c2, float* __restrict__ dgamma,
                                         float* __restrict__ dbeta, float* __restrict__ dbias, int accumulate,
                                         const float* __restrict__ group_tot, const float* __restrict__ part, int slabs) {
  __shared__ double sh1[16][17], sh2[16][17], sh3[16][17];
  const int cl = threadIdx.x & 15, tl = threadIdx.x >> 4;
  const int ch = blockIdx.x * 16 + cl;
  const double M = (double)hw;
  if (part != nullptr && ch < c) {
    for (int n = tl; n < n_img; n += 16) {
      double s1 = 0.0, s2 = 0.0;
      for (int t = 0; t < slabs; ++t) {
        const float* p = part + (((size_t)n * slabs + t) * c + ch) * 2;
        s1 += p[0]; s2 += p[1];
      }
      c1[(size_t)n * c + ch] = (float)s1; c2[(size_t)n * c + ch] = (float)s2;
    }
  }
  double tg = 0.0, tgx = 0.0;
  if (ch < c)
    for (int n = tl; n < n_img; n += 16) { tg += c1[(size_t)n * c + ch]; tgx += c2[(size_t)n * c + ch]; }
  sh1[tl][cl] = tg; sh2[tl][cl] = tgx;
  __syncthreads();
  tg = 0.0; tgx = 0.0;
  for (int j = 0; j < 16; ++j) { tg += sh1[j][cl]; tgx += sh2[j][cl]; }
  __syncthreads();
  const double cnt = (double)n_img * M;
  double tb = 0.0;
  if (ch < c)
    for (int n = tl; n < n_img; n += 16) {
      const size_t idx = (size_t)n * c + ch;
      const double sg = c1[idx], sgx = c2[idx];
      double m1 = 0.0, m2 = 0.0;
      if (!fixed_stats) {
        if (mode == NORM_INSTANCE) { m1 = sg / M; m2 = sgx / M; }
        else if (group_tot) { const double gc = group_tot[2 * c + ch]; m1 = (double)group_tot[ch] / gc; m2 = (double)group_tot[c + ch] / gc; }
        else { m1 = tg / cnt; m2 = tgx / cnt; }
      }
      c1[idx] = (float)m1; c2[idx] = (float)m2;
      if (dbias) {
        const double sxh = ysum ? (double)xa[idx] * ysum[idx] + M * xb[idx] : 0.0;
        tb += (double)scale[idx] * (sg - M * m1 - m2 * sxh);
      }
    }
  sh3[tl][cl] = tb;
  __syncthreads();
  if (tl == 0 && ch < c) {
    tb = 0.0;
    for (int j = 0; j < 16; ++j) tb += sh3[j][cl];
    dgamma[ch] = accumulate ? dgamma[ch] + (float)tgx : (float)tgx;
    dbeta[ch] = accumulate ? dbeta[ch] + (float)tg : (float)tg;
    if (dbias) dbias[ch] = accumulate ? dbias[ch] + (float)tb : (float)tb;
  }
}

template <typename T, bool VEC>
__global__ void norm_act_bwd_apply_kernel(const T* __restrict__ dz, const T* __restrict__ y, T* __restrict__ dy,
                                          const float* __restrict__ scale, const float* __restrict__ shift,
                                          const float* __restrict__ xa, const float* __restrict__ xb,
                                          const float* __restrict__ c1, const float* __restrict__ c2, int64_t hw, int c,
                                          int64_t total_units, float slope) {
  constexpr int EPU = VEC ? Elem<T>::EPU : 1;
  const int upp = c / EPU;
  for (int64_t u = (int64_t)blockIdx.x * blockDim.x + threadIdx.x; u < total_units; u += (int64_t)gridDim.x * blockDim.x) {
    const int64_t pix = u / upp;
    const int ch = (int)(u - pix * upp) * EPU;
    const size_t o = (size_t)(pix / hw) * c + ch;
    alignas(16) T gin[EPU]; alignas(16) T yin[EPU]; alignas(16) T out[EPU];
    if constexpr (VEC) {
      *reinterpret_cast<u32x4*>(gin) = *reinterpret_cast<const u32x4*>(dz + u * EPU);
      *reinterpret_cast<u32x4*>(yin) = *reinterpret_cast<const u32x4*>(y + u * EPU);
    } else { gin[0] = dz[u]; yin[0] = y[u]; }
#pragma unroll
    for (int e = 0; e < EPU; ++e) {
      const float yv = Elem<T>::ld(yin + e);
      float g = Elem<T>::ld(gin + e);
      if (!(scale[o + e] * yv + shift[o + e] > 0.f)) g *= slope;
      const float xh = xa[o + e] * yv + xb[o + e];
      out[e] = Elem<T>::cvt(scale[o + e] * (g - c1[o + e] - xh * c2[o + e]));
    }
    if constexpr (VEC) *reinterpret_cast<u32x4*>(dy + u * EPU) = *reinterpret_cast<const u32x4*>(out);
    else dy[u] = out[0];
  }
}

static bool bwd_vec_ok(const void* dz, const void* y, const void* dy, int dtype, int c) {
  const int epu = dtype == MIA_BF16 ? 8 : 4;
  return (c % epu == 0) &&
         ((reinterpret_cast<uintptr_t>(y) | reinterpret_cast<uintptr_t>(dz) | reinterpret_cast<uintptr_t>(dy)) & 15) == 0;
}

struct NormBwd {
  const void *dz, *dz2, *y; void* dy; int dtype;
  const float *scale, *shift, *xa, *xb, *ysum;
  int n; int64_t hw; int c, mode, fixed_stats; float slope; int slabs;
  float *partials, *c1, *c2, *dgamma, *dbeta, *dbias; int accumulate;
  void* amax_out; hipStream_t st;
};

extern "C" int mia_norm_two_piece_ok(int dtype, int c) { return (dtype == MIA_BF16 || dtype == MIA_F32) && c % 32 == 0; }

static int bwd_check(const char* who, const NormBwd& p, bool tensors, bool need_partials, bool need_grads) {
  MIA_CHECK_ARG(tensors && p.scale && p.shift && p.xa && p.xb && p.c1 && p.c2 && (!need_partials || p.partials) &&
                (!need_grads || (p.dgamma && p.dbeta)), "%s: null pointer", who);
  MIA_CHECK_ARG(p.n > 0 && p.hw > 0 && p.c > 0 && (!need_partials || p.slabs > 0), "%s: bad shape", who);
  MIA_CHECK_ARG(p.dtype == MIA_BF16 || p.dtype == MIA_F32, "%s: bad dtype", who);
  MIA_CHECK_ARG(p.dz2 == nullptr || (p.c % 32 == 0 && bwd_vec_ok(p.dz, p.y, p.dy, p.dtype, p.c) && (reinterpret_cast<uintptr_t>(p.dz2) & 15) == 0),
                "%s: two-piece gradient needs c %% 32 == 0 and aligned tensors", who);
  return MIA_OK;
}

static void bwd_reduce_launch(const NormBwd& p) {
  const int n = p.n, c = p.c, slabs = p.slabs;
  const int64_t hw = p.hw; float* partials = p.partials; hipStream_t st = p.st;
  const bool vec = bwd_vec_ok(p.dz, p.y, nullptr, p.dtype, c);
#define RD(T) hipLaunchKernelGGL(norm_act_bwd_reduce_kernel<T>, dim3(n * slabs, ceil_div(c, 256)), dim3(256), 512 * sizeof(float), st,   \
                                 static_cast<const T*>(p.dz), static_cast<const T*>(p.y), p.scale, p.shift, p.xa, p.xb, hw, c, slabs, \
                                 p.slope, partials)
#define RDV(T) CRV(T, true, static_cast<const T*>(p.dz), static_cast<const T*>(p.y), static_cast<const T*>(p.dz2), p.scale, p.shift, p.xa, p.xb, p.slope)
  if (vec && c % 32 == 0) { if (p.dtype == MIA_BF16) RDV(bf16_t); else RDV(float); }
  else if (p.dtype == MIA_BF16) RD(bf16_t); else RD(float);
#undef RDV
#undef RD
}

static void bwd_finalize_launch(const NormBwd& p, bool producer_parts = false, const float* group_tot = nullptr) {
  const bool own = !producer_parts && group_tot == nullptr;
  const bool inline_sums = own && (int64_t)p.n * p.slabs <= 1024;
  if (group_tot == nullptr && !inline_sums)
    hipLaunchKernelGGL(norm_bwd_sum_kernel, dim3(p.n, ceil_div(p.c, 16)), dim3(256), 0, p.st, p.partials, p.slabs, p.c, p.c1, p.c2);
  hipLaunchKernelGGL(norm_bwd_finalize_kernel, dim3(ceil_div(p.c, 16)), dim3(256), 0, p.st, p.n, p.c, p.hw, p.mode, p.fixed_stats,
                     p.scale, p.xa, p.xb, p.ysum, p.c1, p.c2, p.dgamma, p.dbeta, p.dbias, p.accumulate, group_tot,
                     inline_sums ? p.partials : nullptr, own ? p.slabs : 0);
}

static void bwd_apply_launch(const NormBwd& p) {
  void* amax_out = p.dtype == MIA_F32 ? p.amax_out : nullptr;
  const int epu = p.dtype == MIA_BF16 ? 8 : 4;
  const bool vec = bwd_vec_ok(p.dz, p.y, p.dy, p.dtype, p.c);
  const int64_t units = (int64_t)p.n * p.hw * (vec ? p.c / epu : p.c);
  const int blocks = (int)((units + 255) / 256 < 16384 ? (units + 255) / 256 : 16384);
#define AP(T, V) hipLaunchKernelGGL((norm_act_bwd_apply_kernel<T, V>), dim3(blocks), dim3(256), 0, p.st,                   \
                                    static_cast<const T*>(p.dz), static_cast<const T*>(p.y), static_cast<T*>(p.dy), p.scale, p.shift, \
                                    p.xa, p.xb, p.c1, p.c2, p.hw, p.c, units, p.slope)
  if (vec) {
    int sl, upb, gy;
    stream_geometry(p.n, p.hw, p.c, epu, &sl, &upb, &gy);
#define BS(T, TWOF) hipLaunchKernelGGL((norm_act_bwd_stream_kernel<T, TWOF>), dim3(p.n * sl, gy), dim3(256), 0, p.st, static_cast<const T*>(p.dz), \
                                       static_cast<const T*>(p.dz2), static_cast<const T*>(p.y), static_cast<T*>(p.dy), p.scale, p.shift, p.xa, p.xb, \
                                       p.c1, p.c2, p.hw, p.c, sl, upb, p.slope, static_cast<unsigned*>(amax_out))
    if (p.dtype == MIA_BF16) { if (p.dz2) BS(bf16_t, true); else BS(bf16_t, false); }
    else { if (p.dz2) BS(float, true); else BS(float, false); }
#undef BS
  } else {
    if (p.dtype == MIA_BF16) AP(bf16_t, false);
    else AP(float, false);
    if (amax_out) (void)mia_amax(static_cast<const float*>(p.dy), (int64_t)p.n * p.hw * p.c, amax_out, 0, p.st);
  }
#undef AP
}

extern "C" int mia_norm_act_bwd(const void* dz, const void* dz2, const void* y, void* dy, int dtype, const float* scale, const float* shift,
                                const float* xa, const float* xb, const float* ysum, int n, int64_t hw, int c, int mode,
                                int fixed_stats, float slope, int slabs, float* partials, float* c1, float* c2, float* dgamma,
                                float* dbeta, float* dbias, int accumulate, void* amax_out, void* stream) {
  const NormBwd p{dz, dz2, y, dy, dtype, scale, shift, xa, xb, ysum, n, hw, c, mode, fixed_stats, slope, slabs, partials, c1, c2,
                  dgamma, dbeta, dbias, accumulate, amax_out, static_cast<hipStream_t>(stream)};
  if (int e = bwd_check("mia_norm_act_bwd", p, dz && y && dy, true, true)) return e;
  bwd_reduce_launch(p);
  bwd_finalize_launch(p);
  bwd_apply_launch(p);
  MIA_LAUNCH_CHECK();
  return MIA_OK;
}

extern "C" int mia_norm_bwd_sums(const void* dz, const void* dz2, const void* y, int dtype, const float* scale, const float* shift,
                                 const float* xa, const float* xb, const float* ysum, int n, int64_t hw, int c, int mode,
                                 int fixed_stats, float slope, int slabs, float* partials, float* c1, float* c2, float* dgamma,
                                 float* dbeta, float* dbias, int accumulate, void* stream) {
  const NormBwd p{dz, dz2, y, nullptr, dtype, scale, shift, xa, xb, ysum, n, hw, c, mode, fixed_stats, slope, slabs, partials, c1, c2,
                  dgamma, dbeta, dbias, accumulate, nullptr, static_cast<hipStream_t>(stream)};
  if (int e = bwd_check("mia_norm_bwd_sums", p, dz && y, true, true)) return e;
  bwd_reduce_launch(p);
  bwd_finalize_launch(p);
  MIA_LAUNCH_CHECK();
  return MIA_OK;
}

#ifdef MIA_EXPERIMENTS
extern "C" int mia_norm_act_bwd_pre(const void* dz, const void* y, void* dy, int dtype, const float* scale, const float* shift,
                                    const float* xa, const float* xb, const float* ysum, int n, int64_t hw, int c, int mode,
                                    int fixed_stats, float slope, int parts, const float* partials, float* c1, float* c2,
                                    float* dgamma, float* dbeta, float* dbias, int accumulate, void* amax_out, void* stream) {
  const NormBwd p{dz, nullptr, y, dy, dtype, scale, shift, xa, xb, ysum, n, hw, c, mode, fixed_stats, slope, parts,
                  const_cast<float*>(partials), c1, c2, dgamma, dbeta, dbias, accumulate, amax_out, static_cast<hipStream_t>(stream)};
  if (int e = bwd_check("mia_norm_act_bwd_pre", p, true, true, true)) return e;
  MIA_CHECK_ARG(dy == nullptr || (dz && y), "mia_norm_act_bwd_pre: the apply pass needs dz and y");
  bwd_finalize_launch(p, true);
  if (dy != nullptr) bwd_apply_launch(p);
  MIA_LAUNCH_CHECK();
  return MIA_OK;
}

#endif

__global__ void bn_bwd_local_tot_kernel(int n_img, int c, int64_t hw, const float* __restrict__ c1, const float* __restrict__ c2,
                                        float* __restrict__ tot) {
  __shared__ double sh1[16][17], sh2[16][17];
  const int cl = threadIdx.x & 15, tl = threadIdx.x >> 4;
  const int ch = blockIdx.x * 16 + cl;
  double tg = 0.0, tgx = 0.0;
  if (ch < c)
    for (int n = tl; n < n_img; n += 16) { tg += c1[(size_t)n * c + ch]; tgx += c2[(size_t)n * c + ch]; }
  sh1[tl][cl] = tg; sh2[tl][cl] = tgx;
  __syncthreads();
  if (tl == 0 && ch < c) {
    tg = 0.0; tgx = 0.0;
    for (int j = 0; j < 16; ++j) { tg += sh1[j][cl]; tgx += sh2[j][cl]; }
    tot[ch] = (float)tg; tot[c + ch] = (float)tgx; tot[2 * c + ch] = (float)((double)n_img * (double)hw);
  }
}

extern "C" int mia_norm_act_bwd_reduce(const void* dz, const void* dz2, const void* y, int dtype, const float* scale, const float* shift,
                                       const float* xa, const float* xb, int n, int64_t hw, int c, float slope, int slabs,
                                       float* partials, float* c1, float* c2, float* tot, void* stream) {
  const NormBwd p{dz, dz2, y, nullptr, dtype, scale, shift, xa, xb, nullptr, n, hw, c, NORM_BATCH, 0, slope, slabs, partials, c1, c2,
                  nullptr, nullptr, nullptr, 0, nullptr, static_cast<hipStream_t>(stream)};
  if (int e = bwd_check("mia_norm_act_bwd_reduce", p, dz && y && tot, true, false)) return e;
  bwd_reduce_launch(p);
  hipLaunchKernelGGL(norm_bwd_sum_kernel, dim3(n, ceil_div(c, 16)), dim3(256), 0, p.st, partials, slabs, c, c1, c2);
  hipLaunchKernelGGL(bn_bwd_local_tot_kernel, dim3(ceil_div(c, 16)), dim3(256), 0, p.st, n, c, hw, c1, c2, tot);
  MIA_LAUNCH_CHECK();
  return MIA_OK;
}

extern "C" int mia_norm_act_bwd_apply_sync(const void* dz, const void* dz2, const void* y, void* dy, int dtype, const float* scale,
                                           const float* shift, const float* xa, const float* xb, const float* ysum, int n,
                                           int64_t hw, int c, float slope, float* c1, float* c2, const float* group_tot,
                                           float* dgamma, float* dbeta, float* dbias, int accumulate, void* amax_out, void* stream) {
  const NormBwd p{dz, dz2, y, dy, dtype, scale, shift, xa, xb, ysum, n, hw, c, NORM_BATCH, 0, slope, 0, nullptr, c1, c2,
                  dgamma, dbeta, dbias, accumulate, amax_out, static_cast<hipStream_t>(stream)};
  if (int e = bwd_check("mia_norm_act_bwd_apply_sync", p, dz && y && dy && group_tot, false, true)) return e;
  bwd_finalize_launch(p, false, group_tot);
  bwd_apply_launch(p);
  MIA_LAUNCH_CHECK();
  return MIA_OK;
}

template <typename T, int K1, int CG, bool HWG = false>
__global__ __launch_bounds__(256) void colreduce_head_kernel(const float* __restrict__ dl, const float* __restrict__ w,
                                                             const T* __restrict__ y, const float* __restrict__ scale,
                                                             const float* __restrict__ shift, const float* __restrict__ xa,
                                                             const float* __restrict__ xb, int hw, int c, int slabs, float slope,
                                                             int64_t gsn, int64_t gsp, int64_t gsk, float* __restrict__ part, float* __restrict__ wpart) {
  constexpr int EPU = Elem<T>::EPU, UPB = CG / EPU, LANES = 256 / UPB;
  __shared__ float sh[2][LANES][CG + 1];
  const int n = blockIdx.x / slabs, s = blockIdx.x % slabs;
  const int u = threadIdx.x % UPB, pl = threadIdx.x / UPB;
  const int ch0 = blockIdx.y * CG + u * EPU;
  const int per = (hw + slabs - 1) / slabs, r0 = s * per, r1 = r0 + per < hw ? r0 + per : hw;
  float s1[EPU], s2[EPU], sc[EPU], sf[EPU], ka[EPU], kb[EPU], wr[K1][EPU];
  float wacc[HWG ? K1 : 1][EPU], bacc[HWG ? K1 : 1];
#pragma unroll
  for (int k = 0; k < (HWG ? K1 : 1); ++k) {
    bacc[k] = 0.f;
#pragma unroll
    for (int e = 0; e < EPU; ++e) wacc[k][e] = 0.f;
  }
#pragma unroll
  for (int e = 0; e < EPU; ++e) {
    s1[e] = 0.f; s2[e] = 0.f;
    const size_t o = (size_t)n * c + ch0 + e;
    sc[e] = scale[o]; sf[e] = shift[o]; ka[e] = xa[o]; kb[e] = xb[o];
#pragma unroll
    for (int k = 0; k < K1; ++k) wr[k][e] = w[k * c + ch0 + e];
  }
  const T* yb = y + (size_t)n * hw * c + ch0;
  const float* gb = dl + (int64_t)n * gsn;
  auto body = [&](const u32x4& raw, const float (&gv)[K1]) {
    alignas(16) T v[EPU];
    *reinterpret_cast<u32x4*>(v) = raw;
    if constexpr (HWG) {
#pragma unroll
      for (int k = 0; k < K1; ++k) bacc[k] += gv[k];
    }
#pragma unroll
    for (int e = 0; e < EPU; ++e) {
      const float yv = Elem<T>::ld(v + e);
      float g = 0.f;
#pragma unroll
      for (int k = 0; k < K1; ++k) g += gv[k] * wr[k][e];
      const float uv = sc[e] * yv + sf[e];
      if (!(uv > 0.f)) g *= slope;
      s1[e] += g; s2[e] += g * (ka[e] * yv + kb[e]);
      if constexpr (HWG) {
        const float xv = uv > 0.f ? uv : uv * slope;
#pragma unroll
        for (int k = 0; k < K1; ++k) wacc[k][e] += gv[k] * xv;
      }
    }
  };
  int r = r0 + pl;
  for (; r + 3 * LANES < r1; r += 4 * LANES) {
    u32x4 raw[4];
    float gv[4][K1];
#pragma unroll
    for (int j = 0; j < 4; ++j) raw[j] = *reinterpret_cast<const u32x4*>(yb + (size_t)(r + j * LANES) * c);
#pragma unroll
    for (int j = 0; j < 4; ++j)
#pragma unroll
      for (int k = 0; k < K1; ++k) gv[j][k] = gb[(int64_t)(r + j * LANES) * gsp + k * gsk];
#pragma unroll
    for (int j = 0; j < 4; ++j) body(raw[j], gv[j]);
  }
  for (; r < r1; r += LANES) {
    float gv[K1];
#pragma unroll
    for (int k = 0; k < K1; ++k) gv[k] = gb[(int64_t)r * gsp + k * gsk];
    body(*reinterpret_cast<const u32x4*>(yb + (size_t)r * c), gv);
  }
#pragma unroll
  for (int e = 0; e < EPU; ++e) { sh[0][pl][u * EPU + e] = s1[e]; sh[1][pl][u * EPU + e] = s2[e]; }
  __syncthreads();
  if (threadIdx.x < 2 * CG) {
    const int k = threadIdx.x / CG, chl = threadIdx.x % CG;
    float t = 0.f;
#pragma unroll 8
    for (int j = 0; j < LANES; ++j) t += sh[k][j][chl];
    part[(((size_t)n * slabs + s) * c + blockIdx.y * CG + chl) * 2 + k] = t;
  }
  if constexpr (HWG) {
#pragma unroll
    for (int k = 0; k < K1; ++k) {
      __syncthreads();
#pragma unroll
      for (int e = 0; e < EPU; ++e) sh[0][pl][u * EPU + e] = wacc[k][e];
      if (u == 0) sh[0][pl][CG] = bacc[k];
      __syncthreads();
      if (threadIdx.x <= CG) {
        float t = 0.f;
#pragma unroll 8
        for (int j = 0; j < LANES; ++j) t += sh[0][j][threadIdx.x];
        wpart[((size_t)blockIdx.x * K1 + k) * (CG + 1) + threadIdx.x] = t;
      }
    }
  }
}

__global__ void head_w_final_kernel(const float* __restrict__ part, int nblk, int k1, int c0, float* __restrict__ dw, float* __restrict__ db,
                                    int accumulate) {
  __shared__ float sh[16][17];
  const int cl = threadIdx.x & 15, tl = threadIdx.x >> 4;
  const int i = blockIdx.x * 16 + cl, tot = k1 * (c0 + 1);
  float sm = 0.f;
  if (i < tot)
    for (int b = tl; b < nblk; b += 16) sm += part[(size_t)b * tot + i];
  sh[tl][cl] = sm;
  __syncthreads();
  if (tl == 0 && i < tot) {
    float t = 0.f;
    for (int j = 0; j < 16; ++j) t += sh[j][cl];
    const int kk = i / (c0 + 1), ch = i % (c0 + 1);
    if (ch < c0) dw[kk * c0 + ch] = accumulate ? dw[kk * c0 + ch] + t : t;
    else db[kk] = accumulate ? db[kk] + t : t;
  }
}



template <typename T, int K1>
__global__ __launch_bounds__(256) void norm_act_bwd_stream_head_kernel(const float* __restrict__ dl, const float* __restrict__ w,
                                                                       const T* __restrict__ y, T* __restrict__ dy,
                                                                       const float* __restrict__ scale, const float* __restrict__ shift,
                                                                       const float* __restrict__ xa, const float* __restrict__ xb,
                                                                       const float* __restrict__ c1, const float* __restrict__ c2,
                                                                       int hw, int c, int slabs, int upb, float slope, int64_t gsn,
                                                                       int64_t gsp, int64_t gsk, unsigned* __restrict__ amax) {
  constexpr int EPU = Elem<T>::EPU;
  const int n = blockIdx.x / slabs, s = blockIdx.x % slabs;
  const int lanes = 256 / upb;
  const int u = blockIdx.y * upb + threadIdx.x % upb, pl = threadIdx.x / upb;
  const bool live = u * EPU < c;
  if (!live && (sizeof(T) != 4 || amax == nullptr)) return;
  const int per = (hw + slabs - 1) / slabs, r0 = s * per, r1 = live ? (r0 + per < hw ? r0 + per : hw) : r0;
  float sc[EPU], sf[EPU], ka[EPU], kb[EPU], wr[K1][EPU];
  unsigned am = 0;
#pragma unroll
  for (int e = 0; e < EPU; ++e) {
    const size_t o = live ? (size_t)n * c + u * EPU + e : 0;
    sc[e] = scale[o]; sf[e] = shift[o];
    ka[e] = -sc[e] * c2[o] * xa[o];
    kb[e] = -sc[e] * (c1[o] + c2[o] * xb[o]);
#pragma unroll
    for (int k = 0; k < K1; ++k) wr[k][e] = live ? w[k * c + u * EPU + e] : 0.f;
  }
  const size_t base = (size_t)n * hw * c + (size_t)u * EPU;
  const float* gb = dl + (int64_t)n * gsn;
  auto body = [&](const u32x4& raw, const float (&gv)[K1], int r) {
    alignas(16) T yin[EPU]; alignas(16) T out[EPU];
    *reinterpret_cast<u32x4*>(yin) = raw;
#pragma unroll
    for (int e = 0; e < EPU; ++e) {
      const float yv = Elem<T>::ld(yin + e);
      float g = 0.f;
#pragma unroll
      for (int k = 0; k < K1; ++k) g += gv[k] * wr[k][e];
      if (!(sc[e] * yv + sf[e] > 0.f)) g *= slope;
      out[e] = Elem<T>::cvt(sc[e] * g + ka[e] * yv + kb[e]);
    }
    amax_fold<T>(am, out);
    store_data_fence();
    *reinterpret_cast<u32x4*>(dy + base + (size_t)r * c) = *reinterpret_cast<const u32x4*>(out);
    store_data_pad();
  };
  int r = r0 + pl;
  for (; r + 3 * lanes < r1; r += 4 * lanes) {
    u32x4 raw[4];
    float gv[4][K1];
#pragma unroll
    for (int j = 0; j < 4; ++j) raw[j] = *reinterpret_cast<const u32x4*>(y + base + (size_t)(r + j * lanes) * c);
#pragma unroll
    for (int j = 0; j < 4; ++j)
#pragma unroll
      for (int k = 0; k < K1; ++k) gv[j][k] = gb[(int64_t)(r + j * lanes) * gsp + k * gsk];
#pragma unroll
    for (int j = 0; j < 4; ++j) body(raw[j], gv[j], r + j * lanes);
  }
  for (; r < r1; r += lanes) {
    float gv[K1];
#pragma unroll
    for (int k = 0; k < K1; ++k) gv[k] = gb[(int64_t)r * gsp + k * gsk];
    body(*reinterpret_cast<const u32x4*>(y + base + (size_t)r * c), gv, r);
  }
  if constexpr (sizeof(T) == 4) { if (amax != nullptr) amax_publish(am, amax); }
}

static int norm_act_bwd_head_run(const char* who, const float* dlogits, const float* w, int k1, int64_t gsn, int64_t gsk, int64_t gsp,
                                 const NormBwd& p, float* wpart, float* dwh, float* dbh, int acc_head) {
  if (int e = bwd_check(who, p, dlogits && w && p.y && p.dy, true, true)) return e;
  MIA_CHECK_ARG(p.hw < ((int64_t)1 << 31) && k1 >= 2 && k1 <= 4 && p.c % 32 == 0, "%s: bad shape (c=%d k1=%d)", who, p.c, k1);
  MIA_CHECK_ARG(((reinterpret_cast<uintptr_t>(p.y) | reinterpret_cast<uintptr_t>(p.dy)) & 15) == 0, "%s: unaligned", who);
  const int n = p.n, c = p.c, slabs = p.slabs, dtype = p.dtype, epu = dtype == MIA_BF16 ? 8 : 4;
  const int64_t hw = p.hw; hipStream_t st = p.st;
#define CRH(T, K, CGW, HG) hipLaunchKernelGGL((colreduce_head_kernel<T, K, CGW, HG>), dim3(n * slabs, c / CGW), dim3(256), 0, st, dlogits, w, \
                                              static_cast<const T*>(p.y), p.scale, p.shift, p.xa, p.xb, (int)hw, c, slabs, p.slope, gsn, gsp, gsk, p.partials, wpart)
#define CRHK(T, CGW, HG) do { if (k1 == 2) CRH(T, 2, CGW, HG); else if (k1 == 3) CRH(T, 3, CGW, HG); else CRH(T, 4, CGW, HG); } while (0)
  if (wpart != nullptr) {
    if (dtype == MIA_BF16) CRHK(bf16_t, 64, true); else CRHK(float, 64, true);
    hipLaunchKernelGGL(head_w_final_kernel, dim3(ceil_div(k1 * (c + 1), 16)), dim3(256), 0, st, wpart, n * slabs, k1, c, dwh, dbh, acc_head);
  }
  else if (c % 64 == 0) { if (dtype == MIA_BF16) CRHK(bf16_t, 64, false); else CRHK(float, 64, false); }
  else { if (dtype == MIA_BF16) CRHK(bf16_t, 32, false); else CRHK(float, 32, false); }
#undef CRHK
#undef CRH
  bwd_finalize_launch(p);
  int sl, upb, gy;
  stream_geometry(n, hw, c, epu, &sl, &upb, &gy);
  void* amax_out = dtype == MIA_F32 ? p.amax_out : nullptr;
#define BSH(T, K) hipLaunchKernelGGL((norm_act_bwd_stream_head_kernel<T, K>), dim3(n * sl, gy), dim3(256), 0, st, dlogits, w, \
                                     static_cast<const T*>(p.y), static_cast<T*>(p.dy), p.scale, p.shift, p.xa, p.xb, p.c1, p.c2, (int)hw, c, sl, upb, \
                                     p.slope, gsn, gsp, gsk, static_cast<unsigned*>(amax_out))
#define BSHK(T) do { if (k1 == 2) BSH(T, 2); else if (k1 == 3) BSH(T, 3); else BSH(T, 4); } while (0)
  if (dtype == MIA_BF16) BSHK(bf16_t); else BSHK(float);
#undef BSHK
#undef BSH
  MIA_LAUNCH_CHECK();
  return MIA_OK;
}

extern "C" int mia_norm_act_bwd_head(const float* dlogits, const float* w, int k1, int64_t gsn, int64_t gsk, int64_t gsp,
                                     const void* y, void* dy, int dtype, const float* scale, const float* shift, const float* xa,
                                     const float* xb, const float* ysum, int n, int64_t hw, int c, int mode, int fixed_stats,
                                     float slope, int slabs, float* partials, float* c1, float* c2, float* dgamma, float* dbeta,
                                     float* dbias, int accumulate, void* amax_out, void* stream) {
  const NormBwd p{nullptr, nullptr, y, dy, dtype, scale, shift, xa, xb, ysum, n, hw, c, mode, fixed_stats, slope, slabs, partials, c1, c2,
                  dgamma, dbeta, dbias, accumulate, amax_out, static_cast<hipStream_t>(stream)};
  return norm_act_bwd_head_run("mia_norm_act_bwd_head", dlogits, w, k1, gsn, gsk, gsp, p, nullptr, nullptr, nullptr, 0);
}

extern "C" int mia_head_w_supported(int dtype, int c, int k1) {
  return ((dtype == MIA_BF16 || dtype == MIA_F32) && c == 64 && k1 >= 2 && k1 <= 4) ? 1 : 0;
}
extern "C" int mia_norm_act_bwd_head_w(const float* dlogits, const float* w, int k1, int64_t gsn, int64_t gsk, int64_t gsp,
                                       const void* y, void* dy, int dtype, const float* scale, const float* shift, const float* xa,
                                       const float* xb, const float* ysum, int n, int64_t hw, int c, int mode, int fixed_stats,
                                       float slope, int slabs, float* partials, float* c1, float* c2, float* dgamma, float* dbeta,
                                       float* dbias, int accumulate, float* head_workspace, float* dw_head, float* db_head,
                                       int accumulate_head, void* amax_out, void* stream) {
  MIA_CHECK_ARG(head_workspace && dw_head && db_head, "mia_norm_act_bwd_head_w: null head-gradient pointer");
  MIA_CHECK_ARG(mia_head_w_supported(dtype, c, k1), "mia_norm_act_bwd_head_w: unsupported shape (c=%d k1=%d)", c, k1);
  const NormBwd p{nullptr, nullptr, y, dy, dtype, scale, shift, xa, xb, ysum, n, hw, c, mode, fixed_stats, slope, slabs, partials, c1, c2,
                  dgamma, dbeta, dbias, accumulate, amax_out, static_cast<hipStream_t>(stream)};
  return norm_act_bwd_head_run("mia_norm_act_bwd_head_w", dlogits, w, k1, gsn, gsk, gsp, p, head_workspace, dw_head, db_head,
                               accumulate_head);
}
```

medical-image-analysis_amd/mia_hip/__init__.py:

```python
from __future__ import annotations

import ctypes
import os
import re
from typing import Dict, List, Tuple

HERE = os.path.dirname(os.path.abspath(__file__))
ROOT = os.path.dirname(os.path.dirname(HERE))
HEADER = os.path.join(ROOT, "include", "mia_hip.h")
LIB_PATH = os.environ.get("MIA_HIP_LIB") or os.path.join(HERE, "libmia_hip.so")

F32, BF16 = 0, 1
CONV_G3S1, CONV_G3S2, CONV_G2S2, CONV_T3S2, CONV_T2S2, CONV_G1 = range(6)
WGRAD_3S1, WGRAD_3S2, WGRAD_2S2 = range(3)
NORM_INSTANCE, NORM_BATCH = 0, 1
LOSS_SOFTMAX, LOSS_DO_BG, LOSS_BATCH, LOSS_SQUARED, LOSS_DENSE = 1, 2, 4, 8, 16
SEGLOSS_SOFTMAX, SEGLOSS_DO_BG, SEGLOSS_BATCH, SEGLOSS_LABEL_U8, SEGLOSS_IGNORE = 1, 2, 4, 8, 16
REGLOSS_DO_BG, REGLOSS_BATCH, REGLOSS_IGNORE, REGLOSS_INDEX, REGLOSS_TARGET_U8 = 1, 2, 4, 8, 16
OPT_ADAM, OPT_ADAMW, OPT_SGD = 0, 1, 2


class MiaError(RuntimeError):
    pass


_CTYPES = {
    "int": ctypes.c_int, "int64_t": ctypes.c_int64, "uint64_t": ctypes.c_uint64, "float": ctypes.c_float, "double": ctypes.c_double,
}


def parse_defines(path: str = HEADER) -> Dict[str, int]:
    out = {}
    with open(path) as fh:
        src = fh.read()
    for m in re.finditer(r"^#define\s+(MIA_\w+)\s+(-?\d+)\b", src, flags=re.M):
        out[m.group(1)] = int(m.group(2))
    return out


def parse_header(path: str = HEADER) -> Dict[str, Tuple[object, List[object]]]:
    with open(path) as fh:
        txt = fh.read()
    txt = re.sub(r"/\*.*?\*/", "", txt, flags=re.S)
    txt = "\n".join(l for l in txt.splitlines() if not l.strip().startswith("#"))
    protos = {}
    for m in re.finditer(r"(const char\*|int)\s+(mia_\w+)\s*\(([^)]*)\)\s*;", txt):
        ret, name, args = m.group(1), m.group(2), m.group(3).strip()
        argtypes = []
        if args and args != "void":
            for a in args.split(","):
                a = a.strip()
                if "*" in a:
                    argtypes.append(ctypes.c_void_p)
                else:
                    argtypes.append(_CTYPES[a.split()[-2] if len(a.split()) > 1 else a])
        protos[name] = (ctypes.c_char_p if ret.startswith("const char") else ctypes.c_int, argtypes)
    return protos


_lib = None


def lib() -> ctypes.CDLL:
    global _lib
    if _lib is None:
        if not os.path.exists(LIB_PATH):
            raise MiaError(f"{LIB_PATH} not built; run `python -c 'import __graft_entry__ as g; g.build()'` "
                           "(there is no CPU fallback)")
        import torch
        tl = os.path.join(os.path.dirname(torch.__file__), "lib", "libamdhip64.so")
        if os.path.exists(tl):
            ctypes.CDLL(tl, mode=ctypes.RTLD_GLOBAL)
        l = ctypes.CDLL(LIB_PATH)
        for name, (ret, args) in parse_header().items():
            fn = getattr(l, name)
            fn.restype = ret
            fn.argtypes = args
        exp = os.path.join(os.path.dirname(HEADER), "mia_hip_experiments.h")
        if os.path.exists(exp):
            for name, (ret, args) in parse_header(exp).items():
                if hasattr(l, name):
                    fn = getattr(l, name)
                    fn.restype = ret
                    fn.argtypes = args
        for item in filter(None, os.environ.get("MIA_OPTIONS", "").split(",")):
            key, _, val = item.partition("=")
            if l.mia_set_option(key.strip().encode(), int(val or 1)) != 0:
                raise MiaError(f"MIA_OPTIONS: unknown option {key!r}")
        _lib = l
    return _lib


def set_option(name: str, value: int) -> None:
    check(lib().mia_set_option(name.encode(), int(value)), "mia_set_option")


def get_option(name: str) -> int:
    v = ctypes.c_int(0)
    check(lib().mia_get_option(name.encode(), ctypes.byref(v)), "mia_get_option")
    return v.value


def check(rc: int, what: str = "") -> None:
    if rc != 0:
        msg = lib().mia_last_error()
        raise MiaError(f"{what} failed (rc={rc}): {msg.decode() if msg else ''}")


def call(name: str, *args) -> None:
    check(getattr(lib(), name)(*args), name)
```

medical-image-analysis_amd/mia_hip/build.py:

```python
from __future__ import annotations

import os
import subprocess
import sys
from concurrent.futures import ThreadPoolExecutor

HERE = os.path.dirname(os.path.abspath(__file__))
CSRC = os.path.join(os.path.dirname(HERE), "csrc")
LIB = os.path.join(HERE, "libmia_hip.so")
OBJ = os.path.join(HERE, "_obj")
FLAGS = ["--offload-arch=gfx950", "-O3", "-fPIC", "-std=c++17", "-fno-gpu-rdc"]
COUNTED_VMCNT = {"conv_bt.hip": ("conv_bt_kernel",), "conv_pw.hip": ("conv_pw_kernel",), "conv64_dma.hip": ("conv64_dma_kernel",), "wgrad_ring.hip": ("wgrad_bf16_dma_kernel", "wgrad_bf16_dma96_kernel"), "wgrad_bt.hip": ("wgrad_bf16_bt_kernel", "wgrad_bf16_bt_s2_kernel", "wgrad_bf16_bt_t2_kernel")}


def sources():
    return sorted(os.path.join(CSRC, f) for f in os.listdir(CSRC) if f.endswith(".hip"))


def _stale(target, deps):
    if not os.path.exists(target):
        return True
    t = os.path.getmtime(target)
    return any(os.path.getmtime(d) > t for d in deps)


def check_no_scratch(src, remarks, kernels, obj):
    name, seen = None, set()
    for line in remarks.splitlines():
        if "Function Name:" in line:
            name = line.split("Function Name:")[1].split()[0]
        elif "ScratchSize" in line and name and any(k in name for k in kernels):
            seen.add(name)
            size = int(line.split("ScratchSize [bytes/lane]:")[1].split()[0])
            if size != 0:
                if os.path.exists(obj):
                    os.remove(obj)
                raise RuntimeError(f"{os.path.basename(src)}: {name} spills {size} bytes/lane to scratch; its hand-counted "
                                   f"vmcnt pipeline would be wrong")
    if not seen:
        raise RuntimeError(f"{os.path.basename(src)}: no resource-usage remark found for {kernels}")


def build(force: bool = False, verbose: bool = False) -> str:
    hipcc = os.environ.get("HIPCC", "/opt/rocm/bin/hipcc")
    os.makedirs(OBJ, exist_ok=True)
    headers = [os.path.join(CSRC, f) for f in os.listdir(CSRC) if f.endswith(".h")]
    srcs = sources()
    unknown = set(COUNTED_VMCNT) - {os.path.basename(s) for s in srcs}
    if unknown:
        raise RuntimeError(f"COUNTED_VMCNT names no source file: {sorted(unknown)} (a renamed file would lose its no-scratch guard)")
    jobs = []
    for s in srcs:
        o = os.path.join(OBJ, os.path.basename(s)[:-4] + ".o")
        if force or _stale(o, [s] + headers):
            jobs.append((s, o))

    def cc(job):
        s, o = job
        guarded = COUNTED_VMCNT.get(os.path.basename(s), ())
        cmd = [hipcc] + FLAGS + (["-Rpass-analysis=kernel-resource-usage"] if guarded else []) + ["-c", s, "-o", o]
        if verbose:
            print(" ".join(cmd), flush=True)
        r = subprocess.run(cmd, capture_output=True, text=True)
        if r.returncode != 0:
            raise RuntimeError(f"hipcc failed for {s}:\n{r.stderr}")
        if guarded:
            check_no_scratch(s, r.stderr, guarded, o)
        return o

    if jobs:
        with ThreadPoolExecutor(max_workers=min(4, len(jobs))) as ex:
            list(ex.map(cc, jobs))
    objs = [os.path.join(OBJ, os.path.basename(s)[:-4] + ".o") for s in srcs]
    if force or jobs or _stale(LIB, objs):
        cmd = [hipcc, "--offload-arch=gfx950", "-shared", "-fPIC", "-o", LIB] + objs
        r = subprocess.run(cmd, capture_output=True, text=True)
        if r.returncode != 0:
            raise RuntimeError(f"link failed:\n{r.stderr}")
    return LIB


if __name__ == "__main__":
    print(build(force="--force" in sys.argv, verbose=True))
```

medical-image-analysis_amd/mia_hip/ops.py:

```python
from __future__ import annotations

import ctypes
import math
from typing import Optional, Tuple

import torch

from . import (BF16, CONV_G1, CONV_G2S2, CONV_G3S1, CONV_G3S2, CONV_T2S2, CONV_T3S2, F32, LOSS_BATCH, LOSS_DO_BG,
               LOSS_DENSE, LOSS_SOFTMAX, LOSS_SQUARED, NORM_BATCH, NORM_INSTANCE, REGLOSS_BATCH, REGLOSS_DO_BG, REGLOSS_IGNORE,
               REGLOSS_INDEX, REGLOSS_TARGET_U8, SEGLOSS_BATCH, SEGLOSS_DO_BG, SEGLOSS_IGNORE,
               SEGLOSS_LABEL_U8, SEGLOSS_SOFTMAX, WGRAD_2S2, WGRAD_3S1, WGRAD_3S2, MiaError, call, lib)

LRELU_SLOPE = 0.01
_c_int, _c_float, _c_i64 = ctypes.c_int, ctypes.c_float, ctypes.c_int64


def _p(t: Optional[torch.Tensor]):
    return None if t is None else ctypes.c_void_p(t.data_ptr())


def _stream():
    return ctypes.c_void_p(torch.cuda.current_stream().cuda_stream)


# ... 148 lines not shown
        for w in params:
            c = _caches.get(id(w))
            if c is None or c[0]() is not w or not w.is_cuda or not w.is_contiguous() or w.ndim != 4:
                continue
            for (dt, n_from_d0) in c[1]._store:
                if dt == dtype:
                    ents.append(((id(w), dt, n_from_d0), (w, c[1])))
        if not ents:
            raise MiaError("PackPlan: no packed weights were requested yet (run a step first)")

        class Desc(C.Structure):
            _fields_ = [("src", C.c_void_p), ("dst", C.c_void_p), ("d0", C.c_int), ("d1", C.c_int), ("taps", C.c_int),
                        ("npad", C.c_int), ("kpad", C.c_int), ("n_from_d0", C.c_int), ("brick_begin", C.c_int), ("bricks_x", C.c_int)]

        assert C.sizeof(Desc) == lib().mia_pack_desc_bytes()
        arr = (Desc * len(ents))()
        self.entries, self.dtype, bricks, self.max_taps = [], dtype, 0, 1
        for i, ((_, _, n_from_d0), (w, pc)) in enumerate(ents):
            key = (dtype, n_from_d0)
            _, buf, npad, kpad = pc._store[key]
            d0, d1, taps = w.shape[0], w.shape[1], w.shape[2] * w.shape[3]
            if d0 * d1 * taps * 4 >= 1 << 31:
                raise MiaError("PackPlan: a weight tensor of 2 GiB or more is outside the batched pack kernel's 32-bit offsets")
            pa, pb = (npad, kpad) if n_from_d0 else (kpad, npad)
            ta, tb = (16, 64) if n_from_d0 else (64, 16)
            bx, by = -(-pb // tb), -(-pa // ta)
            arr[i] = Desc(w.data_ptr(), buf.data_ptr(), d0, d1, taps, npad, kpad, int(n_from_d0), bricks, bx)
            bricks += bx * by
            self.max_taps = max(self.max_taps, taps)
            self.entries.append((w, pc, key, buf, npad, kpad, w.data_ptr()))
        self.total_bricks = bricks
        host = torch.frombuffer(bytearray(bytes(arr)), dtype=torch.uint8)
        self.descs = host.to(self.entries[0][0].device)
        self.amax_descs = None
        if dtype == F32:
            class ADesc(C.Structure):
                _fields_ = [("src", C.c_void_p), ("n", C.c_int64)]

            assert C.sizeof(ADesc) == lib().mia_amax_desc_bytes()
            aarr = (ADesc * len(self.entries))()
            for i, (w, *_rest) in enumerate(self.entries):
                aarr[i] = ADesc(w.data_ptr(), w.numel())
            self.amax_descs = torch.frombuffer(bytearray(bytes(aarr)), dtype=torch.uint8).to(self.entries[0][0].device)
            self.amax_slots = torch.zeros(len(self.entries), device=self.entries[0][0].device, dtype=torch.int32)
            self.split_bufs = [getattr(e[3], "_mia_split", None) for e in self.entries]
            for i, e in enumerate(self.entries):
                if self.split_bufs[i] is None:
                    self.split_bufs[i] = torch.empty(e[3].shape, device=e[3].device, dtype=torch.int32)
            self.split_descs = _split_descs([(e[3], self.split_bufs[i], self.amax_slots[i:i + 1]) for i, e in enumerate(self.entries)],
                                            self.entries[0][0].device)

    def valid(self) -> bool:
        return all(w.data_ptr() == ptr for w, _, _, _, _, _, ptr in self.entries)

    def repack(self) -> None:
        call("mia_pack_weight_batch", _p(self.descs), len(self.entries), self.total_bricks, self.max_taps, self.dtype, _stream())
        if self.amax_descs is not None:
            call("mia_amax_batch", _p(self.amax_descs), len(self.entries), _p(self.amax_slots), _stream())
            call("mia_split_f16_batch", _p(self.split_descs), len(self.entries), _stream())
        self.plant()

    def plant(self) -> None:
        for i, (w, pc, key, buf, npad, kpad, _) in enumerate(self.entries):
            pc._store[key] = ((w._version, w.data_ptr(), PARAM_EPOCH), buf, npad, kpad)
            if self.amax_descs is not None:
                buf._mia_amax = (self.amax_slots[i:i + 1], buf._version)
                buf._mia_split = self.split_bufs[i]


_caches = {}


def pack_cache(w: torch.Tensor) -> PackCache:
    c = _caches.get(id(w))
    if c is None or c[0]() is not w:
        import weakref
        pc = PackCache()
        _caches[id(w)] = (weakref.ref(w, lambda _r, k=id(w): _caches.pop(k, None)), pc)
        return pc
    return c[1]


def to_nhwc(x: torch.Tensor, dtype: torch.dtype) -> torch.Tensor:
    _need_dev(x)
    n, c, h, w = x.shape
    if x.dtype not in (torch.float32, torch.bfloat16):
        x = x.float()
    sn, sc, sh, sw = x.stride()
    if x.dtype == dtype:
        if c == 1 and sw == 1 and (h == 1 or sh == w) and (n == 1 or sn == h * w):
            return x.reshape(n, h, w, 1)
        if sc == 1 and sw == c and (h == 1 or sh == w * c) and (n == 1 or sn == h * w * c):
            return x.permute(0, 2, 3, 1)
    if h > 1 and sh != w * sw:
        x = x.contiguous()
        sn, sc, sh, sw = x.stride()
    out = torch.empty((n, h, w, c), device=x.device, dtype=dtype)
    call("mia_relayout", _p(x), _dt(x), _p(out), _dt(out), n, c, _c_i64(h * w), _c_i64(sn), _c_i64(sc), _c_i64(sw),
         _c_i64(h * w * c), _c_i64(1), _c_i64(c), _stream())
    return out


def nhwc_as_nchw(x: torch.Tensor) -> torch.Tensor:
    return x.permute(0, 3, 1, 2)


def cast_nhwc(x: torch.Tensor, dtype: torch.dtype) -> torch.Tensor:
    if x.dtype == dtype:
        return x
    n, h, w, c = x.shape
    out = torch.empty_like(x, dtype=dtype)
    call("mia_relayout", _p(x), _dt(x), _p(out), _dt(out), n, c, _c_i64(h * w), _c_i64(h * w * c), _c_i64(1), _c_i64(c),
         _c_i64(h * w * c), _c_i64(1), _c_i64(c), _stream())
    return out


class LaunchProbe:

    def __init__(self, match):
        self.match, self.pairs, self.enabled = match, [], False

    def times_ms(self, tag=None):
        torch.cuda.synchronize()
        return [p[0].elapsed_time(p[1]) for p in self.pairs if tag is None or p[2] == tag]

    def records(self):
        torch.cuda.synchronize()
        return [(p[0].elapsed_time(p[1]), p[2], p[3]) for p in self.pairs]


PROBE: Optional[LaunchProbe] = None


def conv_tiles(mode: int, hout: int, wout: int) -> int:
    ty, tx, th = _c_int(), _c_int(), _c_int()
    call("mia_conv_mma_tiles", mode, hout, wout, ctypes.byref(ty), ctypes.byref(tx), ctypes.byref(th))
    return ty.value * tx.value


def conv_mma(mode: int, x1: torch.Tensor, x2: Optional[torch.Tensor], wpack: torch.Tensor, npad: int, kpad: int,
             flip: bool, bias: Optional[torch.Tensor], nout: int, out_hw: Tuple[int, int], want_stats: bool = False,
             out_split: Optional[int] = None, nl=None, cr=None):
    n, hin, win, c1 = x1.shape
    c2 = 0 if x2 is None else x2.shape[3]
    hout, wout = out_hw
    if out_split is None:
        out1 = torch.empty((n, hout, wout, nout), device=x1.device, dtype=x1.dtype)
        out2, o1, o2 = None, nout, 0
    else:
        o1, o2 = out_split, nout - out_split
        out1 = torch.empty((n, hout, wout, o1), device=x1.device, dtype=x1.dtype)
        out2 = torch.empty((n, hout, wout, o2), device=x1.device, dtype=x1.dtype)
    stats = None
    if want_stats or cr is not None:
        stats = torch.empty((n, conv_tiles(mode, hout, wout), nout, 2), device=x1.device, dtype=torch.float32)
    am1 = am2 = amw = wsp = None
    if cr is None and nl is None and _split_ok(x1, n * hout * wout * nout * (c1 + c2)):
        wh = getattr(wpack, "_mia_amax", None)
        if wh is not None:
            amw, am1 = wh[0], amax_slot(x1)
            am2 = None if x2 is None else amax_slot(x2)
            wsp = getattr(wpack, "_mia_split", None)
    tag = PROBE.match(mode, c1, c2, nout, hin, win, bool(flip)) if (PROBE is not None and PROBE.enabled) else None
    probe = PROBE if tag else None
    if probe is not None:
        e0, e1 = torch.cuda.Event(enable_timing=True), torch.cuda.Event(enable_timing=True)
        e0.record()
    if cr is not None:
        assert x2 is None and out_split is None and nl is None and bias is None
        yp, cf, sl = cr
        call("mia_conv_mma_cr", mode, _dt(x1), _p(x1), c1, _p(wpack), npad, kpad, int(flip), _p(out1), o1, _p(yp), _p(cf[2]), _p(cf[3]),
             _p(cf[0]), _p(cf[1]), _c_float(sl), _p(stats), n, hin, win, hout, wout, _stream())
    elif nl is not None:
        assert x2 is None and out_split is None and not flip
        call("mia_conv_mma_nl", mode, _dt(x1), _p(x1), c1, _p(nl[0][2]), _p(nl[0][3]), _c_float(nl[1]), _p(wpack), npad, kpad,
             _p(bias), _p(out1), o1, _p(stats), n, hin, win, hout, wout, _stream())
    else:
        ao1 = _amax_new(out1) if (mode == CONV_T2S2 and x1.dtype == torch.float32) else None
        ao2 = _amax_new(out2) if (out2 is not None and x1.dtype == torch.float32) else None
        call("mia_conv_mma", mode, _dt(x1), _p(x1), c1, _p(x2), c2, _p(wpack), npad, kpad, int(flip), _p(bias), _p(out1), o1,
             _p(out2), o2, _p(stats), n, hin, win, hout, wout, _p(am1), _p(am2), _p(amw), _p(wsp), _p(ao1), _p(ao2), _stream())
    if probe is not None:
        e1.record()
        probe.pairs.append((e0, e1, tag, (mode, c1 + c2, nout, n, hout, wout)))
    return out1, out2, stats


WGRAD_TARGET_BLOCKS = int(__import__('os').environ.get('MIA_WGRAD_BLOCKS', '0'))


WGRAD_KSPLIT_MODEL = __import__('os').environ.get('MIA_WGRAD_KSPLIT_MODEL', '1') != '0'


def _ksplit_by_cost(base: int, slots: int, ntiles: int, slab_bytes: int, flops: float) -> int:
    t_compute = flops / 1.2e15
    cands = [k for k in range(1, 8) if k <= ntiles] + [k for k in range(8, min(ntiles, 1024) + 1, 8)]
    best, best_t = 1, None
    for k in cands:
        rounds = -(-base * k // slots)
        t = rounds * slots / (base * k) * t_compute + k * 2.0 * slab_bytes / 4.0e12
        if best_t is None or t < best_t * 0.98:
            best, best_t = k, t
    return best


def conv_wgrad(mode: int, x1: torch.Tensor, x2: Optional[torch.Tensor], dy: torch.Tensor, grad_shape, nn: int, kk: int,
               out: Optional[torch.Tensor] = None, nl=None) -> torch.Tensor:
    n, hx, wx, c1 = x1.shape
    c2 = 0 if x2 is None else x2.shape[3]
    _, hy, wy, cdy = dy.shape
    dtype = _dt(x1)
    taps = 4 if mode == WGRAD_2S2 else 9
    npad, kpad = _pad(nn, 64), _pad(kk, 64)
    pb, pt, ph = _c_int(), _c_int(), _c_int()
    call("mia_wgrad_plan", mode, dtype, c1, c2, cdy, npad, hy, ctypes.byref(pb), ctypes.byref(pt), ctypes.byref(ph))
    ntiles = n * -(-hy // ph.value) * -(-wy // 16)
    base = pb.value
    target = WGRAD_TARGET_BLOCKS or pt.value
    ksplit = max(1, min(ntiles, -(-target // base), 1024))
    if 8 <= ksplit < ntiles:
        ksplit -= ksplit % 8
    if dtype == BF16 and WGRAD_KSPLIT_MODEL and base * ksplit != target:
        ksplit = _ksplit_by_cost(base, target, ntiles, taps * npad * kpad * 4, 2.0 * taps * nn * kk * n * hy * wy)
    slabs = torch.empty((ksplit, taps, npad, kpad), device=x1.device, dtype=torch.float32)
    if nl is not None:
        assert x2 is None
        call("mia_conv_wgrad_nl", mode, dtype, _p(x1), c1, _p(nl[0][2]), _p(nl[0][3]), _c_float(nl[1]), _p(dy), cdy, _p(slabs),
             ksplit, npad, kpad, n, hx, wx, hy, wy, _stream())
    else:
        am1 = am2 = amd = None
        if _split_ok(x1, n * hy * wy * cdy * (c1 + c2)) and dy.dtype == torch.float32:
            am1, amd = amax_slot(x1), amax_slot(dy)
            am2 = None if x2 is None else amax_slot(x2)
        call("mia_conv_wgrad", mode, dtype, _p(x1), c1, _p(x2), c2, _p(dy), cdy, _p(slabs), ksplit, npad, kpad, n, hx, wx, hy,
             wy, _p(am1), _p(am2), _p(amd), _stream())
    grad = out if out is not None else torch.empty(grad_shape, device=x1.device, dtype=torch.float32)
    call("mia_wgrad_reduce", _p(slabs), ksplit, taps, npad, kpad, _p(grad), nn, kk, 0, _stream())
    return grad


def colsum(x: torch.Tensor) -> torch.Tensor:
    c = x.shape[-1]
    p = x.numel() // c
    ws = torch.empty(lib().mia_colsum_workspace(_c_i64(p), c), device=x.device, dtype=torch.float32)
    out = torch.empty(c, device=x.device, dtype=torch.float32)
    call("mia_colsum", _p(x), _dt(x), _c_i64(p), c, _p(ws), _p(out), 0, _stream())
    return out


_GRAD_DEST = {}
_GRAD_CLAIMED = set()


def register_grad_dest(param: torch.Tensor, flat: torch.Tensor, offset: int) -> None:
    _GRAD_DEST[id(param)] = (__import__("weakref").ref(param), flat, offset, param.numel(), tuple(param.shape))
    _GRAD_CLAIMED.discard(id(param))


def unregister_grad_dest(param: torch.Tensor) -> None:
    _GRAD_DEST.pop(id(param), None)
    _GRAD_CLAIMED.discard(id(param))


def release_grad_dest(param: torch.Tensor) -> None:
    _GRAD_CLAIMED.discard(id(param))


def grad_dest(param: Optional[torch.Tensor]) -> Optional[torch.Tensor]:
    if param is None:
        return None
    hit = _GRAD_DEST.get(id(param))
    if hit is None:
        return None
    if hit[0]() is not param:
        _GRAD_DEST.pop(id(param), None)
        _GRAD_CLAIMED.discard(id(param))
        return None
    if param.grad is not None:
        return None
    if id(param) in _GRAD_CLAIMED:
        return None
    _GRAD_CLAIMED.add(id(param))
    _, flat, off, n, shape = hit
    return flat[off:off + n].view(shape)


_COLSUM_HINT = {}


def _hint_colsum(t: torch.Tensor, sums: torch.Tensor) -> None:
    if len(_COLSUM_HINT) > 16:
        _COLSUM_HINT.clear()
    _COLSUM_HINT[t.data_ptr()] = (tuple(t.shape), t._version, sums)


def _take_colsum(t: torch.Tensor) -> Optional[torch.Tensor]:
    hit = _COLSUM_HINT.pop(t.data_ptr(), None)
    if hit is not None and hit[0] == tuple(t.shape) and hit[1] == t._version:
        return hit[2]
    return None


_CR_HINT = {}
FUSE_CR = __import__('os').environ.get('MIA_FUSE_CR', '0') != '0'


def _hint_cr(dz: torch.Tensor, partials: torch.Tensor) -> None:
    if len(_CR_HINT) > 64:
        _CR_HINT.clear()
    _CR_HINT[dz.data_ptr()] = (partials, tuple(dz.shape))


def _take_cr(dz: torch.Tensor) -> Optional[torch.Tensor]:
    h = _CR_HINT.pop(dz.data_ptr(), None)
    return h[0] if (h is not None and h[1] == tuple(dz.shape)) else None


_ACC_HINT = {}
FUSE_ACC = __import__('os').environ.get('MIA_FUSE_ACC', '1') != '0'


def _hint_acc(x: torch.Tensor, dx: torch.Tensor) -> None:
    if FUSE_ACC and dx is not None:
        _ACC_HINT[x.data_ptr()] = (dx, tuple(x.shape))


def _take_acc(x: torch.Tensor) -> Optional[torch.Tensor]:
    h = _ACC_HINT.pop(x.data_ptr(), None)
    return h[0] if (h is not None and h[1] == tuple(x.shape) and h[0].dtype == x.dtype) else None


def clear_hints() -> None:
    _COLSUM_HINT.clear()
    _CR_HINT.clear()
    _ACC_HINT.clear()
    _GRAD_CLAIMED.clear()


def cr_supported(dtype, cin: int, cout: int, h: int, w: int) -> bool:
    return (FUSE_CR and dtype == torch.bfloat16 and hasattr(lib(), "mia_conv_mma_cr")
            and bool(lib().mia_conv_cr_supported(CONV_G3S1, BF16, cout, cin, h, w)))


_COL_SLABS = int(__import__('os').environ.get('MIA_COL_SLABS', '64'))


def _slabs_for(hw: int) -> int:
    return max(1, min(_COL_SLABS, hw // 1024))


class StepDyn:

    def __init__(self, device):
        self.dev = torch.zeros(32, dtype=torch.uint8, device=device)
        self.rng_span = 0

    def set(self, lr: float, bc1: float, bc2: float, first: bool, seed: int, base_offset: int) -> None:
        call("mia_step_dyn_set", _p(self.dev), _c_float(lr), _c_float(bc1), _c_float(bc2), int(bool(first)),
             ctypes.c_uint64(seed & (2 ** 64 - 1)), ctypes.c_uint64(base_offset), _stream())

    @property
    def f32_ptr(self):
        return ctypes.c_void_p(self.dev.data_ptr())

    @property
    def u64_ptr(self):
        return ctypes.c_void_p(self.dev.data_ptr() + 16)


_STEP_DYN: Optional[StepDyn] = None


def dropout_mask(numel: int, keep: float, device) -> torch.Tensor:
    dev = torch.device(device)
    if _STEP_DYN is not None:
        out = torch.empty(numel, device=dev, dtype=torch.float32)
        call("mia_dropout_mask_dyn", _p(out), _c_i64(numel), _c_float(keep), _STEP_DYN.u64_ptr, ctypes.c_uint64(_STEP_DYN.rng_span), _stream())
        _STEP_DYN.rng_span += 4 * ((numel + 3) // 4)
        return out
    gen = torch.cuda.default_generators[dev.index if dev.index is not None else torch.cuda.current_device()]
    seed, off = int(gen.initial_seed()), int(gen.get_offset())
    gen.set_offset(off + 4 * ((numel + 3) // 4))
    out = torch.empty(numel, device=dev, dtype=torch.float32)
    call("mia_dropout_mask", _p(out), _c_i64(numel), _c_float(keep), ctypes.c_uint64(seed & (2 ** 64 - 1)), ctypes.c_uint64(off),
         _stream())
    return out


class NormCfg:
    __slots__ = ("mode", "training", "eps", "momentum", "running_mean", "running_var", "num_batches", "drop_scale", "sync")

    def __init__(self, mode, training, eps=1e-5, momentum=0.1, running_mean=None, running_var=None, num_batches=None,
                 drop_scale=None, sync=None):
        self.mode, self.training, self.eps, self.momentum = mode, training, eps, momentum
        self.running_mean, self.running_var, self.num_batches, self.drop_scale = running_mean, running_var, num_batches, drop_scale
        self.sync = sync

    fixed = property(lambda self: self.mode == NORM_BATCH and not self.training)


class BatchSync:

    def __init__(self, process_group=None):
        import torch.distributed as dist
        self.dist, self.pg = dist, process_group
        self.world = dist.get_world_size(process_group)

    def all_gather(self, local: torch.Tensor) -> torch.Tensor:
        out = torch.empty((self.world,) + tuple(local.shape), device=local.device, dtype=local.dtype)
        self.dist.all_gather([out[r] for r in range(self.world)], local, group=self.pg)
        return out

    def all_reduce_sum(self, t: torch.Tensor) -> torch.Tensor:
        self.dist.all_reduce(t, op=self.dist.ReduceOp.SUM, group=self.pg)
        return t


def _norm_finalize(ctx, cfg: NormCfg, stats, gamma, beta, y) -> torch.Tensor:
    n, h, w, cout = y.shape
    hw = h * w
    coefs = torch.empty((5, n, cout), device=y.device, dtype=torch.float32)
    ctx.sync = sync = cfg.sync if (cfg.sync is not None and cfg.mode == NORM_BATCH and cfg.training and cfg.sync.world > 1) else None
    if sync is None:
        call("mia_norm_finalize", _p(stats), n, 0 if stats is None else stats.shape[1], cout, _c_i64(hw), cfg.mode, int(cfg.training),
             _p(cfg.drop_scale), _p(gamma.detach()), _p(beta.detach()), _c_float(cfg.eps), _c_float(cfg.momentum),
             _p(cfg.running_mean), _p(cfg.running_var), _p(cfg.num_batches), _p(coefs[0]), _p(coefs[1]), _p(coefs[2]),
             _p(coefs[3]), _p(coefs[4]), _stream())
        return coefs
    local = torch.empty((3, cout), device=stats.device, dtype=torch.float32)
    call("mia_bn_sync_local_stats", _p(stats), n, stats.shape[1], cout, _c_i64(hw), _p(cfg.drop_scale), _p(coefs[0]),
         _p(coefs[1]), _p(local), _stream())
    gathered = sync.all_gather(local)
    call("mia_norm_finalize_sync", _p(gathered), sync.world, n, cout, _c_i64(hw), _p(cfg.drop_scale), _p(gamma.detach()),
         _p(beta.detach()), _c_float(cfg.eps), _c_float(cfg.momentum), _p(cfg.running_mean), _p(cfg.running_var),
         _p(cfg.num_batches), _p(coefs[0]), _p(coefs[1]), _p(coefs[2]), _p(coefs[3]), _p(coefs[4]), _stream())
    return coefs


def _norm_act_fwd(y, scale, shift, slope) -> torch.Tensor:
    n, h, w, c = y.shape
    z = torch.empty_like(y)
    call("mia_norm_act_fwd", _p(y), _p(z), _dt(y), _p(scale), _p(shift), n, _c_i64(h * w), c, _c_float(slope), _p(_amax_new(z)), _stream())
    return z


class LazyAct:
    __slots__ = ("y", "coefs", "slope")

    def __init__(self, y, coefs, slope):
        self.y, self.coefs, self.slope = y, coefs, slope

    @property
    def shape(self):
        return self.y.shape

    @property
    def dtype(self):
        return self.y.dtype

    @property
    def device(self):
        return self.y.device

    def materialize(self) -> torch.Tensor:
        return LazyMaterializeFn.apply(self.y, self.coefs, self.slope)


class LazyMaterializeFn(torch.autograd.Function):

    @staticmethod
    def forward(ctx, y, coefs, slope):
        return _norm_act_fwd(y, coefs[2], coefs[3], slope)

    @staticmethod
    def backward(ctx, dz):
        return dz, None, None


FUSE_HEAD_W = __import__('os').environ.get('MIA_FUSE_HEAD_W', '1') != '0'
FUSE_STEM_BWD = __import__('os').environ.get('MIA_FUSE_STEM_BWD', '1') != '0'
FUSE_NL = __import__('os').environ.get('MIA_FUSE_NL', '1') != '0'


def nl_supported(dtype, cin: int, cout: int, h: int, w: int, train: bool) -> bool:
    if not FUSE_NL or dtype != torch.bfloat16:
        return False
    if not lib().mia_conv_nl_supported(CONV_G3S1, BF16, cin, cout, h, w):
        return False
    return (not train) or bool(lib().mia_wgrad_nl_supported(WGRAD_3S1, BF16, cin, cout))


class _NormBwd:

    def __init__(self, y, coefs, mode, fixed, slope, dests=None):
        self.y, self.coefs, self.mode, self.fixed, self.slope = y, coefs, mode, fixed, slope
        n, h, w, c = y.shape
        self.dtype, self.n, self.hw, self.c, self.slabs = _dt(y), n, h * w, c, _slabs_for(h * w)
        self.part = torch.empty((n, self.slabs, c, 2), device=y.device, dtype=torch.float32)
        self.cc = torch.empty((2, n, c), device=y.device, dtype=torch.float32)
        dgb = torch.empty((3, c), device=y.device, dtype=torch.float32)
        got = (None,) * 3 if dests is None else [grad_dest(p) for p in dests]
        self.dgamma, self.dbeta, self.dbias = (dgb[i] if g is None else g for i, g in enumerate(got))

    def _run(self, slabs, part):
        k = self.coefs
        return (_p(k[2]), _p(k[3]), _p(k[0]), _p(k[1]), _p(None if self.fixed else k[4]), self.n, _c_i64(self.hw), self.c, self.mode,
                int(self.fixed), _c_float(self.slope), slabs, _p(part), _p(self.cc[0]), _p(self.cc[1]), _p(self.dgamma),
                _p(self.dbeta), _p(self.dbias), 0)

    def plain(self, dz, dz2, dy) -> None:
        call("mia_norm_act_bwd", _p(dz), _p(dz2), _p(self.y), _p(dy), self.dtype, *self._run(self.slabs, self.part),
             _p(_amax_new(dy)), _stream())

    def sums(self, dz, dz2) -> None:
        call("mia_norm_bwd_sums", _p(dz), _p(dz2), _p(self.y), self.dtype, *self._run(self.slabs, self.part), _stream())

    def pre(self, parts, dz, dy) -> None:
        call("mia_norm_act_bwd_pre", _p(None if dy is None else dz), _p(None if dy is None else self.y), _p(dy), self.dtype,
             *self._run(parts.shape[1], parts), _p(None if dy is None else _amax_new(dy)), _stream())

    def synced(self, sync: BatchSync, dz, dz2, dy) -> None:
        k, cc = self.coefs, self.cc
        tot = torch.empty((3, self.c), device=self.y.device, dtype=torch.float32)
        call("mia_norm_act_bwd_reduce", _p(dz), _p(dz2), _p(self.y), self.dtype, _p(k[2]), _p(k[3]), _p(k[0]), _p(k[1]), self.n,
             _c_i64(self.hw), self.c, _c_float(self.slope), self.slabs, _p(self.part), _p(cc[0]), _p(cc[1]), _p(tot), _stream())
        sync.all_reduce_sum(tot)
        call("mia_norm_act_bwd_apply_sync", _p(dz), _p(dz2), _p(self.y), _p(dy), self.dtype, _p(k[2]), _p(k[3]), _p(k[0]), _p(k[1]),
             _p(k[4]), self.n, _c_i64(self.hw), self.c, _c_float(self.slope), _p(cc[0]), _p(cc[1]), _p(tot), _p(self.dgamma),
             _p(self.dbeta), _p(self.dbias), 0, _p(_amax_new(dy)), _stream())

    def run(self, dz, dz2, sync, on_load: bool) -> Optional[torch.Tensor]:
        pre = _take_cr(dz) if (dz2 is None and sync is None) else None
        dy = None if on_load else torch.empty_like(self.y)
        if pre is not None:
            self.pre(pre, dz, dy)
        elif sync is not None:
            self.synced(sync, dz, dz2, dy)
        elif on_load:
            self.sums(dz, dz2)
        else:
            self.plain(dz, dz2, dy)
        return dy

    def head(self, dl, st, w2, dy, entry="mia_norm_act_bwd_head", extra=()) -> None:
        call(entry, _p(dl), _p(w2), w2.shape[0], _c_i64(st[0]), _c_i64(st[1]), _c_i64(st[2]), _p(self.y), _p(dy), self.dtype,
             *self._run(self.slabs, self.part), *extra, _p(_amax_new(dy)), _stream())

    def head_w(self, dl, st, w2, dy, ws, dwh, dbh) -> None:
        self.head(dl, st, w2, dy, "mia_norm_act_bwd_head_w", (_p(ws), _p(dwh), _p(dbh), 0))


def _block_wgrad(nb: _NormBwd, x1, x2, weight, stride: int, nl, dy, stem: bool = False, dz=None, dz2=None) -> torch.Tensor:
    cout, cin = weight.shape[:2]
    y, k = nb.y, nb.coefs
    if not stem:
        dw = conv_wgrad(WGRAD_3S2 if stride == 2 else WGRAD_3S1, x1, x2, dy, weight.shape, cout, cin, out=grad_dest(weight), nl=nl)
    else:
        if dy is None and dz2 is not None:
            dz = dz + dz2
        ws = torch.empty(lib().mia_stem_wgrad_workspace(cout), device=y.device, dtype=torch.float32)
        dw = grad_dest(weight)
        if dw is None:
            dw = torch.empty(weight.shape, device=y.device, dtype=torch.float32)
        if dy is None:
            call("mia_stem_wgrad_fused", _p(x1), _dt(x1), _p(dz), _p(y), nb.dtype, _p(k[2]), _p(k[3]), _p(k[0]), _p(k[1]),
                 _p(nb.cc[0]), _p(nb.cc[1]), _c_float(nb.slope), _p(ws), _p(dw), nb.n, y.shape[1], y.shape[2], cout, 0, _stream())
        else:
            call("mia_stem_wgrad", _p(x1), _dt(x1), _p(dy), nb.dtype, _p(ws), _p(dw), nb.n, y.shape[1], y.shape[2], cout, 0, _stream())
    return dw


def _block_dgrad(x1, x2, weight, dy, stride: int, nl, dup_in: bool, need1: bool, need2: bool):
    dx1 = dx2 = None
    dtype = _dt(dy)
    n, ho, wo, cout = dy.shape
    c1, cin = x1.shape[3], weight.shape[1]
    wb, npad, kpad = pack_cache(weight).get(weight, dtype, n_from_d0=False)
    split = c1 if x2 is not None else None
    other = _take_acc(x1) if (stride == 2 and x2 is None and dup_in) else None
    if other is not None and lib().mia_conv_acc_supported(CONV_T3S2, dtype, cout, cin):
        amw = getattr(wb, "_mia_amax", None) if _split_ok(dy, n * ho * wo * cout * cin) else None
        call("mia_conv_mma_acc", CONV_T3S2, dtype, _p(dy), cout, _p(wb), npad, kpad, 0, _p(other), cin, n, ho, wo,
             x1.shape[1], x1.shape[2], _p(None if amw is None else amax_slot(dy)), _p(None if amw is None else amw[0]),
             _p(None if amw is None else getattr(wb, "_mia_split", None)), _stream())
    elif stride == 2:
        dx1, dx2, _ = conv_mma(CONV_T3S2, dy, None, wb, npad, kpad, False, None, cin, (x1.shape[1], x1.shape[2]), out_split=split)
    elif nl is not None and cr_supported(dy.dtype, cin, cout, ho, wo):
        dx1, _, partials = conv_mma(CONV_G3S1, dy, None, wb, npad, kpad, True, None, cin, (ho, wo), cr=(x1,) + nl)
        _hint_cr(dx1, partials)
    else:
        want = x2 is not None and need2
        dx1, dx2, st = conv_mma(CONV_G3S1, dy, None, wb, npad, kpad, True, None, cin, (ho, wo), want_stats=want, out_split=split)
        if want:
            sums = colsum(st.view(-1, 2 * cin)).view(cin, 2)[c1:, 0]
            _hint_colsum(dx2, sums)
        if x2 is not None and need1 and dup_in:
            _hint_acc(x1, dx1)
    return dx1, dx2


class PlainBlockFn(torch.autograd.Function):

    @staticmethod
    def forward(ctx, x1, x2, weight, bias, gamma, beta, stride: int, cfg: NormCfg, out_dtype=None, slope: float = LRELU_SLOPE,
                dup: bool = False, lazy: bool = False, nl_coefs=None, nl_slope: float = LRELU_SLOPE):
        ctx.dup_in = bool(getattr(x1, "_mia_dup", False))
        ctx.set_materialize_grads(False)
        _need_dev(x1, x2, weight)
        x1 = x1.contiguous()
        x2 = None if x2 is None else x2.contiguous()
        out_dtype = out_dtype or x1.dtype
        cout = weight.shape[0]
        assert not (lazy and dup)
        stem = (weight.shape[1] == 1 and x2 is None and stride == 1 and x1.shape[3] == 1 and not x1.requires_grad
                and cout % (8 if out_dtype == torch.bfloat16 else 4) == 0 and cout <= 256 and nl_coefs is None)
        if stem:
            z = PlainBlockFn._stem_forward(ctx, x1, weight, bias, gamma, beta, cfg, out_dtype, slope, lazy)
            return (z, _dup_view(z)) if dup else z
        if x1.dtype != out_dtype:
            x1 = cast_nhwc(x1, out_dtype)
        if x2 is not None and (x2.shape[:3] != x1.shape[:3] or x2.dtype != x1.dtype):
            raise RuntimeError(f"Sizes of tensors must match except in dimension 1: {tuple(x1.shape)} vs {tuple(x2.shape)} (NHWC)")
        dtype = _dt(x1)
        n, h, w, c1 = x1.shape
        if weight.shape[1] != c1 + (0 if x2 is None else x2.shape[3]):
            raise RuntimeError(f"conv weight expects {weight.shape[1]} input channels, got {c1 + (0 if x2 is None else x2.shape[3])}")
        ho, wo = ((h + 1) // 2, (w + 1) // 2) if stride == 2 else (h, w)
        wp, npad, kpad = pack_cache(weight).get(weight, dtype, n_from_d0=True)
        mode = CONV_G3S2 if stride == 2 else CONV_G3S1
        nl = None if nl_coefs is None else (nl_coefs, float(nl_slope))
        if nl is not None and (x2 is not None or stride != 1):
            raise MiaError("normalise-on-load serves one-source stride-1 blocks only")
        y, _, stats = conv_mma(mode, x1, x2, wp, npad, kpad, False, bias.detach().float(), cout, (ho, wo), want_stats=not cfg.fixed,
                               nl=nl)
        coefs = _norm_finalize(ctx, cfg, stats, gamma, beta, y)
        ctx.stride, ctx.mode, ctx.fixed, ctx.stem, ctx.slope = stride, cfg.mode, cfg.fixed, False, slope
        ctx.small = (bias, beta)
        ctx.nl_slope = float(nl_slope)
        ctx.save_for_backward(x1, x2, y, coefs, weight, gamma, nl_coefs)
        if lazy:
            ctx.mark_non_differentiable(coefs)
            return y, coefs
        z = _norm_act_fwd(y, coefs[2], coefs[3], slope)
        return (z, _dup_view(z)) if dup else z
# ... 967 lines not shown
```

Measured before the change: 778.7 images/sec.

## Enable column-reduce norm-backward epilogue in conv64 by default with LDS-staged operands

Moves the column-reduce epilogue, which fuses the instance-norm backward reductions into the 64-channel 3x3 conv data-grad kernel, out of the experiment-only build and turns it on by default. The y tile and per-channel coefficients are now DMA'd into LDS at tile start, replacing per-row register-prefetched buffer loads, and the LDS A-image is shrunk for CR so two blocks still fit per CU. This removes a separate pass over dz and y for the norm backward sums. In exchange the kernel uses more LDS and adds store fences, and the fused path is now limited to maps of at least 64x64.

Result: no change. 782.2 images/sec (median of 6 runs) (+0.5%).

```diff
diff --git a/include/mia_hip.h b/include/mia_hip.h
--- a/include/mia_hip.h
+++ b/include/mia_hip.h
@@ -52,6 +52,11 @@
                     const void* wpack, int npad, int kpad, const float* bias, void* out, int nout, float* stat_partials,
                     int n, int hin, int win, int hout, int wout, void* stream);
 
+int mia_conv_cr_supported(int mode, int dtype, int c1, int nout, int hout, int wout);
+int mia_conv_mma_cr(int mode, int dtype, const void* in1, int c1, const void* wpack, int npad, int kpad, int flip_taps,
+                    void* out, int nout, const void* y_prod, const float* scale, const float* shift, const float* xa,
+                    const float* xb, float slope, float* partials, int n, int hin, int win, int hout, int wout, void* stream);
+
 int mia_conv_acc_supported(int mode, int dtype, int c1, int nout);
 int mia_conv_mma_acc(int mode, int dtype, const void* in1, int c1, const void* wpack, int npad, int kpad, int flip_taps,
                      void* out_inout, int nout, int n, int hin, int win, int hout, int wout, const void* amax_in, const void* amax_w,
@@ -102,6 +107,10 @@
                       const float* xa, const float* xb, const float* ysum, int n, int64_t hw, int c, int mode,
                       int fixed_stats, float slope, int slabs, float* partials, float* c1, float* c2, float* dgamma,
                       float* dbeta, float* dbias, int accumulate, void* stream);
+int mia_norm_act_bwd_pre(const void* dz, const void* y, void* dy, int dtype, const float* scale, const float* shift,
+                         const float* xa, const float* xb, const float* ysum, int n, int64_t hw, int c, int mode,
+                         int fixed_stats, float slope, int parts, const float* partials, float* c1, float* c2,
+                         float* dgamma, float* dbeta, float* dbias, int accumulate, void* amax_out, void* stream);
 
 int mia_bn_sync_local_stats(const float* partials, int n, int tiles, int c, int64_t hw, const float* drop_scale, float* xa,
                             float* xb, float* local, void* stream);
diff --git a/include/mia_hip_experiments.h b/include/mia_hip_experiments.h
--- a/include/mia_hip_experiments.h
+++ /dev/null
@@ -1,16 +0,0 @@
-#pragma once
-#include <stdint.h>
-#ifdef __cplusplus
-extern "C" {
-#endif
-int mia_conv_cr_supported(int mode, int dtype, int c1, int nout, int hout, int wout);
-int mia_conv_mma_cr(int mode, int dtype, const void* in1, int c1, const void* wpack, int npad, int kpad, int flip_taps,
-                    void* out, int nout, const void* y_prod, const float* scale, const float* shift, const float* xa,
-                    const float* xb, float slope, float* partials, int n, int hin, int win, int hout, int wout, void* stream);
-int mia_norm_act_bwd_pre(const void* dz, const void* y, void* dy, int dtype, const float* scale, const float* shift,
-                         const float* xa, const float* xb, const float* ysum, int n, int64_t hw, int c, int mode,
-                         int fixed_stats, float slope, int parts, const float* partials, float* c1, float* c2,
-                         float* dgamma, float* dbeta, float* dbias, int accumulate, void* amax_out, void* stream);
-#ifdef __cplusplus
-}
-#endif
diff --git a/medical-image-analysis_amd/csrc/common.h b/medical-image-analysis_amd/csrc/common.h
--- a/medical-image-analysis_amd/csrc/common.h
+++ b/medical-image-analysis_amd/csrc/common.h
@@ -146,8 +146,15 @@
   static __device__ __forceinline__ float unscale(float acc, int eo) { return __builtin_ldexpf(acc, eo); }
 };
 
+__device__ __forceinline__ float norm_bwd_g(float dz, float yv, float sc, float sf, float slope) {
+  return (__builtin_fmaf(sc, yv, sf) > 0.f) ? dz : dz * slope;
+}
+__device__ __forceinline__ f32x2_t norm_bwd_g(f32x2_t dz, f32x2_t yv, f32x2_t sc, f32x2_t sf, float slope) {
+  const f32x2_t u = __builtin_elementwise_fma(sc, yv, sf), ds = dz * f32x2_t{slope, slope};
+  return f32x2_t{(u[0] > 0.f) ? dz[0] : ds[0], (u[1] > 0.f) ? dz[1] : ds[1]};
+}
 __device__ __forceinline__ float norm_bwd_dy(float g, float yv, float sc, float sf, float ka, float kb, float slope) {
-  if (!(__builtin_fmaf(sc, yv, sf) > 0.f)) g *= slope;
+  g = norm_bwd_g(g, yv, sc, sf, slope);
   return __builtin_fmaf(sc, g, __builtin_fmaf(ka, yv, kb));
 }
 
diff --git a/medical-image-analysis_amd/csrc/conv64.hip b/medical-image-analysis_amd/csrc/conv64.hip
--- a/medical-image-analysis_amd/csrc/conv64.hip
+++ b/medical-image-analysis_amd/csrc/conv64.hip
@@ -11,6 +11,9 @@
 constexpr int A_IT = (IH * IW + 63) / 64;
 constexpr int NPA = ((A_IT * 64 + 13) / 16) * 16 + 2;
 constexpr int LDS_BYTES = 8 * NPA * 16;
+constexpr int Y_BYTES = TH * TW * C * 2;
+constexpr int NPA_CR = ((IH * IW + 13) / 16) * 16 + 2;
+static_assert(NPA_CR >= IH * IW && NPA_CR % 16 == 2 && 2 * ((8 * NPA_CR * 16 + 1023) / 1024 * 1024 + Y_BYTES + 4096) <= 160 * 1024, "column-reduce LDS image");
 
 struct Tile { int img, ty, tx; };
 
@@ -37,9 +40,11 @@
 
 template <bool NL, bool CR>
 __global__ __launch_bounds__(256, 2) void conv64_persist_kernel(const ConvArgs a, int total_tiles, int tiles_per_img, int run, int n_base) {
-  __shared__ __attribute__((aligned(16))) unsigned char smem[LDS_BYTES + (NL ? 2 * C * 4 : 0)];
+  constexpr int NP = CR ? NPA_CR : NPA;
+  constexpr int Y0 = (8 * NP * 16 + 1023) / 1024 * 1024, CRC0 = Y0 + Y_BYTES;
+  __shared__ __attribute__((aligned(CR ? 1024 : 16))) unsigned char smem[CR ? CRC0 + 4 * 1024 : 8 * NP * 16 + (NL ? 2 * C * 4 : 0)];
   u32x4* ldsA = reinterpret_cast<u32x4*>(smem);
-  float* cf = reinterpret_cast<float*>(smem + LDS_BYTES);
+  float* cf = reinterpret_cast<float*>(smem + 8 * NP * 16);
 
   const int tid = threadIdx.x, lane = tid & 63;
   const int wave = __builtin_amdgcn_readfirstlane(tid >> 6);
@@ -61,7 +66,7 @@
       }
   f32x4 bv;
 #pragma unroll
-  for (int r = 0; r < 4; ++r) bv[r] = a.bias ? a.bias[n_base + 16 * wave + 4 * q + r] : 0.f;
+  for (int r = 0; r < 4; ++r) bv[r] = (!CR && a.bias) ? a.bias[n_base + 16 * wave + 4 * q + r] : 0.f;
 
   const int nblk = gridDim.x, b = blockIdx.x;
   const int first = (b & 7) * run + (b >> 3);
@@ -161,8 +166,9 @@
     }
 #pragma unroll
     for (int i = 0; i < A_IT; ++i) {
-      ldsA[g * NPA + p4 + 64 * i] = pf[2 * i];
-      ldsA[(4 + g) * NPA + p4 + 64 * i] = pf[2 * i + 1];
+      if (CR && 64 * (i + 1) > NP && !(p4 + 64 * i < IH * IW)) continue;
+      ldsA[g * NP + p4 + 64 * i] = pf[2 * i];
+      ldsA[(4 + g) * NP + p4 + 64 * i] = pf[2 * i + 1];
     }
   };
 
@@ -182,6 +188,23 @@
 #endif
   while (true) {
     STAMP(ts0);
+    if constexpr (CR) {
+      const unsigned lds0 = (unsigned)(size_t)(__attribute__((address_space(3))) unsigned char*)smem;
+      const i32x4 rsy = rsrc_words(static_cast<const bf16_t*>(a.cr_y) + (size_t)cur.img * ipix * C, img_bytes);
+      const int oy = cur.ty * TH + (lane >> 5), ox = cur.tx * TW + ((lane >> 1) & 15);
+      const unsigned yo = (unsigned)((oy * a.Wout + ox) * (C * 2) + (16 * wave + 8 * (lane & 1)) * 2);
+#pragma unroll
+      for (int j = 0; j < TH / 2; ++j) {
+        const bool ok = ox < a.Wout && oy + 2 * j < a.Hout;
+        dma16<4>(rsy, ok ? yo + (unsigned)(2 * j * a.Wout * (C * 2)) : SENT, __builtin_amdgcn_readfirstlane(lds0 + Y0 + wave * (Y_BYTES / 4) + j * 1024));
+      }
+      const unsigned cbytes = (unsigned)(a.N * C * 4), co = (unsigned)((cur.img * C + 16 * wave + (lane & 15)) * 4);
+      const unsigned cdst = __builtin_amdgcn_readfirstlane(lds0 + CRC0 + wave * 1024);
+      dma4<4>(rsrc_words(a.cr_scale, cbytes), co, cdst);
+      dma4<4>(rsrc_words(a.cr_shift, cbytes), co, cdst + 256);
+      dma4<4>(rsrc_words(a.cr_xa, cbytes), co, cdst + 512);
+      dma4<4>(rsrc_words(a.cr_xb, cbytes), co, cdst + 768);
+    }
     const int tn = t + stride;
     const bool more = tn < total_tiles;
     Tile nxt = cur;
@@ -194,7 +217,7 @@
     auto load_group = [&](int gi, u32x4* f) {
       const int ph = gi / GROUPS, c = ph / 3, tb = ph % 3, r0 = (gi % GROUPS) * RPG;
 #pragma unroll
-      for (int j = 0; j < RPG; ++j) f[j] = ldsA[(4 * c + q) * NPA + (r0 + j) * PITCH + tb + pr];
+      for (int j = 0; j < RPG; ++j) f[j] = ldsA[(4 * c + q) * NP + (r0 + j) * PITCH + tb + pr];
     };
     load_group(0, fr[0]);
 #pragma unroll
@@ -227,40 +250,19 @@
     const int row_bytes = a.Wout * (C * 2);
     const bool want_stats = a.stats != nullptr;
     float s1[4] = {0.f, 0.f, 0.f, 0.f}, s2[4] = {0.f, 0.f, 0.f, 0.f};
+    const u32x2* yl = reinterpret_cast<const u32x2*>(smem + (CR ? Y0 : 0) + wave * (Y_BYTES / 4) + 32 * pr + 8 * q);
     f32x4 csc, csf, cxa, cxb;
-    u32x2 yv[TH];
-    const unsigned ybase = (unsigned)(((oy0 * a.Wout) + ox0 + pr) * (C * 2) + (16 * wave + 4 * q) * 2);
-    rsrc_t rsy;
-    constexpr int YB = 2;
-    auto load_y = [&](int m0, bool full_t) {
-#pragma unroll
-      for (int mm = m0; mm < m0 + YB; ++mm) {
-        const bool ok = full_t || (colok && oy0 + mm < a.Hout);
-        yv[mm] = __builtin_bit_cast(u32x2, __builtin_amdgcn_raw_buffer_load_b64(rsy, (int)(ok ? ybase + (unsigned)(mm * row_bytes) : SENT), 0, 0));
-      }
-    };
-    if constexpr (CR) {
-      const unsigned cbytes = (unsigned)(a.N * C * 4);
-      const int co = (cur.img * C + 16 * wave + 4 * q) * 4;
-      csc = __builtin_bit_cast(f32x4, __builtin_amdgcn_raw_buffer_load_b128(make_rsrc(a.cr_scale, cbytes), co, 0, 0));
-      csf = __builtin_bit_cast(f32x4, __builtin_amdgcn_raw_buffer_load_b128(make_rsrc(a.cr_shift, cbytes), co, 0, 0));
-      cxa = __builtin_bit_cast(f32x4, __builtin_amdgcn_raw_buffer_load_b128(make_rsrc(a.cr_xa, cbytes), co, 0, 0));
-      cxb = __builtin_bit_cast(f32x4, __builtin_amdgcn_raw_buffer_load_b128(make_rsrc(a.cr_xb, cbytes), co, 0, 0));
-      rsy = make_rsrc(static_cast<const bf16_t*>(a.cr_y) + (size_t)cur.img * ipix * C, img_bytes);
-      load_y(0, full);
-      load_y(YB, full);
-    }
-    auto cr_row = [&](unsigned p01, unsigned p23, const u32x2& yr, float wgt) {
-      const unsigned dzw[2] = {p01, p23}, yw[2] = {yr[0], yr[1]};
+    auto cr_row = [&](unsigned p01, unsigned p23, const u32x2& yr, auto full_tag, bool ok) {
+      const unsigned dzw[2] = {p01, p23};
 #pragma unroll
       for (int h = 0; h < 2; ++h) {
 #pragma unroll
         for (int e = 0; e < 2; ++e) {
           const int r = 2 * h + e;
-          const float dzv = __builtin_bit_cast(float, e ? (dzw[h] & 0xFFFF0000u) : (dzw[h] << 16));
-          const float y = __builtin_bit_cast(float, e ? (yw[h] & 0xFFFF0000u) : (yw[h] << 16));
-          float g = dzv * wgt;
-          if (!(__builtin_fmaf(csc[r], y, csf[r]) > 0.f)) g *= a.cr_slope;
+          float d = __builtin_bit_cast(float, e ? (dzw[h] & 0xFFFF0000u) : (dzw[h] << 16));
+          if constexpr (!decltype(full_tag)::value) d *= ok ? 1.f : 0.f;
+          const float y = __builtin_bit_cast(float, e ? (yr[h] & 0xFFFF0000u) : (yr[h] << 16));
+          const float g = norm_bwd_g(d, y, csc[r], csf[r], a.cr_slope);
           s1[r] += g;
           s2[r] = __builtin_fmaf(g, __builtin_fmaf(cxa[r], y, cxb[r]), s2[r]);
         }
@@ -269,10 +271,19 @@
     auto store_rows = [&](auto full_tag) {
       constexpr bool FULL = decltype(full_tag)::value;
       if constexpr (FULL) asm volatile("s_nop 7\n\ts_nop 7" ::: "memory");
+      u32x2 ya, yb, yan, ybn;
+      if constexpr (CR) {
+        wait_vm<0>();
+        const f32x4* c4 = reinterpret_cast<const f32x4*>(smem + (CR ? CRC0 : 0) + 1024 * wave) + q;
+        csc = c4[0]; csf = c4[16];
+        yan = yl[0]; ybn = yl[64];
+      }
 #pragma unroll
       for (int m = 0; m < TH; m += 2) {
         if constexpr (CR) {
-          if (m % YB == 0 && m + 2 * YB < TH) load_y(m + 2 * YB, FULL);
+          ya = yan; yb = ybn;
+          { const f32x4* c4 = reinterpret_cast<const f32x4*>(smem + (CR ? CRC0 : 0) + 1024 * wave) + q; cxa = c4[32]; cxb = c4[48]; }
+          if (m + 2 < TH) { yan = yl[64 * (m + 2)]; ybn = yl[64 * (m + 3)]; }
         }
         if (want_stats && !CR) {
 #pragma unroll
@@ -289,12 +300,13 @@
         const unsigned x0 = pack_bf16x2(acc[m][0], acc[m][1]), x1 = pack_bf16x2(acc[m][2], acc[m][3]);
         const unsigned y0 = pack_bf16x2(acc[m + 1][0], acc[m + 1][1]), y1 = pack_bf16x2(acc[m + 1][2], acc[m + 1][3]);
         if constexpr (CR) {
-          cr_row(x0, x1, yv[m], (FULL || (colok && oy0 + m < a.Hout)) ? 1.f : 0.f);
-          cr_row(y0, y1, yv[m + 1], (FULL || (colok && oy0 + m + 1 < a.Hout)) ? 1.f : 0.f);
+          cr_row(x0, x1, ya, full_tag, colok && oy0 + m < a.Hout);
+          cr_row(y0, y1, yb, full_tag, colok && oy0 + m + 1 < a.Hout);
         }
         const auto r0 = __builtin_amdgcn_permlane16_swap(x0, y0, false, false);
         const auto r1 = __builtin_amdgcn_permlane16_swap(x1, y1, false, false);
         const u32x4 d = {r0[0], r1[0], r0[1], r1[1]};
+        if constexpr (CR) store_data_fence();
         if constexpr (FULL) {
           __builtin_amdgcn_raw_buffer_store_b128(d, rso, (int)obase, m * row_bytes, 0);
         } else {
@@ -303,19 +315,7 @@
           __builtin_amdgcn_raw_buffer_store_b128(d, rso, (int)voff, 0, 0);
         }
         if constexpr (CR) {
-          __builtin_amdgcn_sched_barrier(0);
-#ifndef CR_PAD
-#define CR_PAD 16
-#endif
-#if CR_PAD >= 16
-          asm volatile("s_nop 7\n\ts_nop 7" ::: "memory");
-#elif CR_PAD >= 8
-          asm volatile("s_nop 7" ::: "memory");
-#elif CR_PAD >= 4
-          asm volatile("s_nop 3" ::: "memory");
-#elif CR_PAD >= 2
-          asm volatile("s_nop 1" ::: "memory");
-#endif
+          store_data_pad();
           __builtin_amdgcn_sched_barrier(0);
         }
       }
@@ -369,7 +369,7 @@
 bool conv64_eligible(int mode, int dtype, const ConvArgs& a) {
   if (mode != MODE_G3S1 || dtype != MIA_BF16) return false;
   if (a.nl_scale != nullptr && (a.o2 != 0 || a.nl_shift == nullptr || !(a.nl_slope >= 0.f && a.nl_slope <= 1.f))) return false;
-  if (a.cr_y != nullptr && (a.o2 != 0 || a.nl_scale != nullptr || a.stats == nullptr || !a.cr_scale || !a.cr_shift || !a.cr_xa || !a.cr_xb)) return false;
+  if (a.cr_y != nullptr && (a.o2 != 0 || a.bias != nullptr || a.nl_scale != nullptr || a.stats == nullptr || !a.cr_scale || !a.cr_shift || !a.cr_xa || !a.cr_xb)) return false;
   if (a.c1 != C || a.c2 != 0 || a.o1 != C || (a.o2 != 0 && a.o2 != C) || a.npad != a.o1 + a.o2 || a.kpad != C) return false;
   if (!a.vec_in || !a.vec_out) return false;
   if ((size_t)a.Hin * a.Win * C * 2 >= ((size_t)1 << 31)) return false;
@@ -388,14 +388,10 @@
     hipLaunchKernelGGL((conv64_persist_kernel<true, false>), dim3(nblk), dim3(256), 0, st, a, total, tiles_per_img, run, 0);
     return MIA_OK;
   }
-#ifdef MIA_EXPERIMENTS
   if (a.cr_y != nullptr) {
     hipLaunchKernelGGL((conv64_persist_kernel<false, true>), dim3(nblk), dim3(256), 0, st, a, total, tiles_per_img, run, 0);
     return MIA_OK;
   }
-#else
-  if (a.cr_y != nullptr) { mia_set_error("column-reduce epilogue: experiment build only (-DMIA_EXPERIMENTS)"); return MIA_EUNSUPPORTED; }
-#endif
   hipLaunchKernelGGL((conv64_persist_kernel<false, false>), dim3(nblk), dim3(256), 0, st, a, total, tiles_per_img, run, 0);
   if (a.o2 == C)
     hipLaunchKernelGGL((conv64_persist_kernel<false, false>), dim3(nblk), dim3(256), 0, st, a, total, tiles_per_img, run, C);
diff --git a/medical-image-analysis_amd/csrc/conv_mma.hip b/medical-image-analysis_amd/csrc/conv_mma.hip
--- a/medical-image-analysis_amd/csrc/conv_mma.hip
+++ b/medical-image-analysis_amd/csrc/conv_mma.hip
@@ -346,7 +346,6 @@
     if (a.split && wpack_split != nullptr) { a.wp = wpack_split; a.wsplit = 1; }
     rc = conv_mma_fast_launch(mode, dtype, a, mt, nt, grid_y, st);
   }
-#ifdef MIA_EXPERIMENTS
   else if (cr_y != nullptr) {
     if (!(mt == 4 && conv64_eligible(mode, dtype, a))) {
       mia_set_error("mia_conv_mma_cr: shape outside the column-reduce kernel's contract (ask mia_conv_cr_supported first)");
@@ -354,7 +353,6 @@
     }
     rc = conv64_launch(a, 0, opt.reserve_cus, st);
   }
-#endif
   else if (nl_scale != nullptr) {
     if (!(mt == 4 && conv64_eligible(mode, dtype, a))) {
       mia_set_error("mia_conv_mma_nl: shape outside the normalise-on-load kernel's contract (ask mia_conv_nl_supported first)");
@@ -406,10 +404,11 @@
                       hout, wout, stream, in_scale, in_shift, slope);
 }
 
-#ifdef MIA_EXPERIMENTS
+static bool conv_cr_contract(int mode, int dtype, int c1, int nout, int hout) {
+  return mode == MODE_G3S1 && dtype == MIA_BF16 && c1 == 64 && nout == 64 && hout > 8;
+}
 extern "C" int mia_conv_cr_supported(int mode, int dtype, int c1, int nout, int hout, int wout) {
-  (void)wout;
-  return (mode == MODE_G3S1 && dtype == MIA_BF16 && c1 == 64 && nout == 64 && hout > 8) ? 1 : 0;
+  return (conv_cr_contract(mode, dtype, c1, nout, hout) && (int64_t)hout * wout >= 64 * 64) ? 1 : 0;
 }
 
 extern "C" int mia_conv_mma_cr(int mode, int dtype, const void* in1, int c1, const void* wpack, int npad, int kpad, int flip_taps,
@@ -417,7 +416,7 @@
                                const float* xb, float slope, float* partials, int n, int hin, int win, int hout, int wout,
                                void* stream) {
   MIA_CHECK_ARG(y_prod && scale && shift && xa && xb && partials, "mia_conv_mma_cr: null pointer");
-  MIA_CHECK_ARG(mia_conv_cr_supported(mode, dtype, c1, nout, hout, wout), "mia_conv_mma_cr: unsupported shape (mode %d dtype %d %d -> %d)",
+  MIA_CHECK_ARG(conv_cr_contract(mode, dtype, c1, nout, hout), "mia_conv_mma_cr: unsupported shape (mode %d dtype %d %d -> %d)",
                 mode, dtype, c1, nout);
   MIA_CHECK_ARG((reinterpret_cast<uintptr_t>(y_prod) & 15) == 0 && (reinterpret_cast<uintptr_t>(scale) & 15) == 0 &&
                 (reinterpret_cast<uintptr_t>(shift) & 15) == 0 && (reinterpret_cast<uintptr_t>(xa) & 15) == 0 &&
@@ -427,8 +426,6 @@
                       win, hout, wout, stream, nullptr, nullptr, 0.f, y_prod, coef, slope);
 }
 
-#endif
-
 extern "C" int mia_conv_acc_supported(int mode, int dtype, int c1, int nout) {
   const int epu = dtype == MIA_BF16 ? 8 : 4;
   return ((mode == MODE_T3S2 || mode == MODE_G3S1) && (dtype == MIA_BF16 || dtype == MIA_F32) && c1 % (4 * epu) == 0 && nout % epu == 0) ? 1 : 0;
diff --git a/medical-image-analysis_amd/csrc/lds_dma.h b/medical-image-analysis_amd/csrc/lds_dma.h
--- a/medical-image-analysis_amd/csrc/lds_dma.h
+++ b/medical-image-analysis_amd/csrc/lds_dma.h
@@ -27,4 +27,9 @@
   asm volatile("s_mov_b32 m0, %2\n\ts_nop %3\n\tbuffer_load_dwordx4 %0, %1, 0 offen lds" : : "v"(voff), "s"(rsrc), "s"(lds_dst), "n"(NOP) : "memory", "m0");
 }
 
+template <int NOP>
+__device__ __forceinline__ void dma4(i32x4 rsrc, unsigned voff, unsigned lds_dst) {
+  asm volatile("s_mov_b32 m0, %2\n\ts_nop %3\n\tbuffer_load_dword %0, %1, 0 offen lds" : : "v"(voff), "s"(rsrc), "s"(lds_dst), "n"(NOP) : "memory", "m0");
+}
+
 template <int N> __device__ __forceinline__ void wait_vm() { asm volatile("s_waitcnt vmcnt(%0)" ::"n"(N) : "memory"); }
diff --git a/medical-image-analysis_amd/csrc/norm.hip b/medical-image-analysis_amd/csrc/norm.hip
--- a/medical-image-analysis_amd/csrc/norm.hip
+++ b/medical-image-analysis_amd/csrc/norm.hip
@@ -767,7 +767,6 @@
   return MIA_OK;
 }
 
-#ifdef MIA_EXPERIMENTS
 extern "C" int mia_norm_act_bwd_pre(const void* dz, const void* y, void* dy, int dtype, const float* scale, const float* shift,
                                     const float* xa, const float* xb, const float* ysum, int n, int64_t hw, int c, int mode,
                                     int fixed_stats, float slope, int parts, const float* partials, float* c1, float* c2,
@@ -781,8 +780,6 @@
   MIA_LAUNCH_CHECK();
   return MIA_OK;
 }
-
-#endif
 
 __global__ void bn_bwd_local_tot_kernel(int n_img, int c, int64_t hw, const float* __restrict__ c1, const float* __restrict__ c2,
                                         float* __restrict__ tot) {
diff --git a/medical-image-analysis_amd/mia_hip/__init__.py b/medical-image-analysis_amd/mia_hip/__init__.py
--- a/medical-image-analysis_amd/mia_hip/__init__.py
+++ b/medical-image-analysis_amd/mia_hip/__init__.py
@@ -76,13 +76,6 @@
             fn = getattr(l, name)
             fn.restype = ret
             fn.argtypes = args
-        exp = os.path.join(os.path.dirname(HEADER), "mia_hip_experiments.h")
-        if os.path.exists(exp):
-            for name, (ret, args) in parse_header(exp).items():
-                if hasattr(l, name):
-                    fn = getattr(l, name)
-                    fn.restype = ret
-                    fn.argtypes = args
         for item in filter(None, os.environ.get("MIA_OPTIONS", "").split(",")):
             key, _, val = item.partition("=")
             if l.mia_set_option(key.strip().encode(), int(val or 1)) != 0:
diff --git a/medical-image-analysis_amd/mia_hip/build.py b/medical-image-analysis_amd/mia_hip/build.py
--- a/medical-image-analysis_amd/mia_hip/build.py
+++ b/medical-image-analysis_amd/mia_hip/build.py
@@ -10,7 +10,7 @@
 LIB = os.path.join(HERE, "libmia_hip.so")
 OBJ = os.path.join(HERE, "_obj")
 FLAGS = ["--offload-arch=gfx950", "-O3", "-fPIC", "-std=c++17", "-fno-gpu-rdc"]
-COUNTED_VMCNT = {"conv_bt.hip": ("conv_bt_kernel",), "conv_pw.hip": ("conv_pw_kernel",), "conv64_dma.hip": ("conv64_dma_kernel",), "wgrad_ring.hip": ("wgrad_bf16_dma_kernel", "wgrad_bf16_dma96_kernel"), "wgrad_bt.hip": ("wgrad_bf16_bt_kernel", "wgrad_bf16_bt_s2_kernel", "wgrad_bf16_bt_t2_kernel")}
+COUNTED_VMCNT = {"conv_bt.hip": ("conv_bt_kernel",), "conv_pw.hip": ("conv_pw_kernel",), "conv64.hip": ("conv64_persist_kernel",), "conv64_dma.hip": ("conv64_dma_kernel",), "wgrad_ring.hip": ("wgrad_bf16_dma_kernel", "wgrad_bf16_dma96_kernel"), "wgrad_bt.hip": ("wgrad_bf16_bt_kernel", "wgrad_bf16_bt_s2_kernel", "wgrad_bf16_bt_t2_kernel")}
 
 
 def sources():
diff --git a/medical-image-analysis_amd/mia_hip/ops.py b/medical-image-analysis_amd/mia_hip/ops.py
--- a/medical-image-analysis_amd/mia_hip/ops.py
+++ b/medical-image-analysis_amd/mia_hip/ops.py
@@ -474,7 +474,7 @@
 
 
 _CR_HINT = {}
-FUSE_CR = __import__('os').environ.get('MIA_FUSE_CR', '0') != '0'
+FUSE_CR = __import__('os').environ.get('MIA_FUSE_CR', '1') != '0'
 
 
 def _hint_cr(dz: torch.Tensor, partials: torch.Tensor) -> None:
@@ -510,8 +510,7 @@
 
 
 def cr_supported(dtype, cin: int, cout: int, h: int, w: int) -> bool:
-    return (FUSE_CR and dtype == torch.bfloat16 and hasattr(lib(), "mia_conv_mma_cr")
-            and bool(lib().mia_conv_cr_supported(CONV_G3S1, BF16, cout, cin, h, w)))
+    return FUSE_CR and dtype == torch.bfloat16 and bool(lib().mia_conv_cr_supported(CONV_G3S1, BF16, cout, cin, h, w))
 
 
 _COL_SLABS = int(__import__('os').environ.get('MIA_COL_SLABS', '64'))
```
